# VachaLab/gorder

Measured on AMD Instinct MI355X. Metric: trajectory frames/sec, higher is better.
Workload: dtype f32

## Files before the change

gorder_amd/abi.py:

```python
from __future__ import annotations

import ctypes as C
import os
from dataclasses import dataclass, field
from typing import List, Optional, Sequence

import numpy as np

_HERE = os.path.dirname(os.path.abspath(__file__))
LIB_PATH = os.environ.get("GORDER_HIP_LIB") or os.path.join(_HERE, "libgorder_hip.so")

OK = 0
ERR_UNDEFINED_BOX = 1
ERR_NOT_ORTHOGONAL_BOX = 2
ERR_ZERO_BOX = 3
ERR_UNDEFINED_POSITION = 4
ERR_INVALID_GLOBAL_MEMBRANE_CENTER = 5
ERR_INVALID_LOCAL_MEMBRANE_CENTER = 6
ERR_DYNAMIC_NORMAL = 7
ERR_MANUAL_LEAFLET_FRAME = 8
ERR_MANUAL_NORMAL_FRAME = 9
ERR_INVALID_ARGUMENT = 100
ERR_DEVICE = 101
ERR_NO_DEVICE = 102
# ... 126 lines not shown
    flip: bool = False
    radius: float = 0.0
    membrane: Optional[np.ndarray] = None


@dataclass
class OrderMap:
    enabled: bool = False
    plane: int = 0
    span_x: Sequence[float] = (0.0, 0.0)
    span_y: Sequence[float] = (0.0, 0.0)
    bin: Sequence[float] = (0.1, 0.1)


GEOM_NONE, GEOM_CUBOID, GEOM_CYLINDER, GEOM_SPHERE = range(4)
GEOMREF_POINT, GEOMREF_BOX_CENTER, GEOMREF_GROUP = range(3)
_INF = float("inf")


@dataclass
class Geometry:
    kind: int = GEOM_NONE
    invert: bool = False
    reference: int = GEOMREF_POINT
    point: Sequence[float] = (0.0, 0.0, 0.0)
    group: Optional[np.ndarray] = None
    xdim: Sequence[float] = (-_INF, _INF)
    ydim: Sequence[float] = (-_INF, _INF)
    zdim: Sequence[float] = (-_INF, _INF)
    radius: float = 0.0
    span: Sequence[float] = (-_INF, _INF)
    orientation: int = 2
    structure_box: Sequence[float] = (0.0, 0.0, 0.0)


@dataclass
class DynamicNormal:
    enabled: bool = False
    radius: float = 2.0
    cloud: Optional[np.ndarray] = None


@dataclass
class Tables:
    n_atoms: int
    molecule_types: List[MolType]
    handle_pbc: bool = True
    normal: Sequence[float] = (0.0, 0.0, 1.0)
    leaflets: Leaflets = field(default_factory=Leaflets)
    ordermap: OrderMap = field(default_factory=OrderMap)
    timewise: bool = False
    device: int = 0
    flags: int = 0
    geometry: Geometry = field(default_factory=Geometry)
    dynamic_normal: DynamicNormal = field(default_factory=DynamicNormal)

    @property
    def n_acc(self) -> int:
        return sum(m.n_slots for m in self.molecule_types)

    @property
    def n_molecules_total(self) -> int:
        return sum(m.n_molecules for m in self.molecule_types)

    @property
    def n_samples_per_frame(self) -> int:
        return sum(m.n_slots * m.n_molecules for m in self.molecule_types)

    def as_ctypes(self):
        keep = []
        mts = (CMolType * max(1, len(self.molecule_types)))()
        for k, m in enumerate(self.molecule_types):
            c = mts[k]
            c.n_molecules = m.n_molecules
            b = _u32(m.bonds, (-1, m.n_molecules, 2)) if m.bonds is not None else None
            c.n_bond_types = 0 if b is None else b.shape[0]
            c.bonds = _ptr(b)
            ua = (CUaAtom * max(1, len(m.ua_atoms)))()
            for q, (kind, idx) in enumerate(m.ua_atoms):
                ia = _u32(idx, (m.n_molecules, 4))
                ua[q].kind = int(kind)
                ua[q].indices = _ptr(ia)
                keep.append(ia)
            c.n_ua_atoms = len(m.ua_atoms)
            c.ua_atoms = C.cast(ua, C.POINTER(CUaAtom))
            h = _u32(m.heads, (m.n_molecules,)) if m.heads is not None else None
            c.heads = _ptr(h)
            me = _u32(m.methyls, (m.n_molecules, -1)) if m.methyls is not None else None
            c.n_methyls = 0 if me is None else me.shape[1]
            c.methyls = _ptr(me)
            nh = _u32(m.normal_heads, (m.n_molecules,)) if m.normal_heads is not None else None
            c.normal_heads = _ptr(nh)
            keep += [b, ua, h, me, nh]
        t = CTables()
        t.n_atoms = self.n_atoms
        t.n_molecule_types = len(self.molecule_types)
        t.molecule_types = C.cast(mts, C.POINTER(CMolType))
        t.handle_pbc = 1 if self.handle_pbc else 0
        t.normal[:] = [float(x) for x in self.normal]
        lf = self.leaflets
        mem = _u32(lf.membrane) if lf.membrane is not None else None
        t.leaflets.method = lf.method
        t.leaflets.normal_dim = lf.normal_dim
        t.leaflets.frequency = lf.frequency
        t.leaflets.flip = 1 if lf.flip else 0
        t.leaflets.radius = lf.radius
        t.leaflets.n_membrane = 0 if mem is None else mem.size
        t.leaflets.membrane = _ptr(mem)
        om = self.ordermap
        t.ordermap.enabled = 1 if om.enabled else 0
        t.ordermap.plane = om.plane
        t.ordermap.span_x[:] = [float(x) for x in om.span_x]
        t.ordermap.span_y[:] = [float(x) for x in om.span_y]
        t.ordermap.bin[:] = [float(x) for x in om.bin]
        t.timewise = 1 if self.timewise else 0
        t.device = self.device
        t.flags = self.flags
        ge = self.geometry
        grp = _u32(ge.group) if ge.group is not None else None
        t.geometry.kind = ge.kind
        t.geometry.invert = 1 if ge.invert else 0
        t.geometry.reference = ge.reference
        t.geometry.point[:] = [float(x) for x in ge.point]
        t.geometry.n_group = 0 if grp is None else grp.size
        t.geometry.group = _ptr(grp)
        t.geometry.xdim[:] = [float(x) for x in ge.xdim]
        t.geometry.ydim[:] = [float(x) for x in ge.ydim]
        t.geometry.zdim[:] = [float(x) for x in ge.zdim]
        t.geometry.radius = ge.radius
        t.geometry.span[:] = [float(x) for x in ge.span]
        t.geometry.orientation = ge.orientation
        t.geometry.structure_box[:] = [float(x) for x in ge.structure_box]
        dn = self.dynamic_normal
        cloud = _u32(dn.cloud) if dn.cloud is not None else None
        t.dynamic_normal.enabled = 1 if dn.enabled else 0
        t.dynamic_normal.radius = dn.radius
        t.dynamic_normal.n_cloud = 0 if cloud is None else cloud.size
        t.dynamic_normal.cloud = _ptr(cloud)
        keep += [mts, mem, grp, cloud]
        return t, keep


_EXPORTS = [
    "gorder_hip_create", "gorder_hip_destroy", "gorder_hip_n_accumulators", "gorder_hip_ordermap_dims",
    "gorder_hip_set_stream", "gorder_hip_submit_device", "gorder_hip_submit_host",
    "gorder_hip_prime_leaflets", "gorder_hip_set_manual_leaflets", "gorder_hip_synchronize",
    "gorder_hip_finish", "gorder_hip_timewise", "gorder_hip_leaflets", "gorder_hip_leaflet_distances",
    "gorder_hip_normals", "gorder_hip_export_maps", "gorder_hip_set_normals",
    "gorder_hip_accumulators_device", "gorder_hip_bind_accumulators", "gorder_hip_last_error_index", "gorder_hip_last_error_frame", "gorder_hip_kernel_time_names",
    "gorder_hip_last_error_message", "gorder_hip_strerror", "gorder_hip_kernel_time", "gorder_hip_kernel_time_group", "gorder_hip_plan",
    "gorder_hip_plan_tables", "gorder_hip_selftest_arithmetic", "gorder_hip_selftest_trig", "gorder_hip_selftest_wave_ops", "gorder_hip_run_trajectory",
    "gorder_hip_comm_unique_id", "gorder_hip_comm_create", "gorder_hip_comm_destroy", "gorder_hip_allreduce",
    "gorder_hip_reset", "gorder_hip_xtc_decode", "gorder_hip_release_staging", "gorder_hip_speculation_stats", "gorder_hip_local_decide_stats",
    "gorder_hip_spherical_stats", "gorder_hip_clustering_stats",
    "gorder_hip_set_collect", "gorder_hip_collected_counts", "gorder_hip_collected_leaflets", "gorder_hip_collected_normals",
    "gorder_hip_set_manual_leaflet_table", "gorder_hip_set_manual_normal_table",
    "gorder_hip_timewise_chunk_frames", "gorder_hip_timewise_rows", "gorder_hip_timewise_blocks", "gorder_hip_error_estimate",
    "gorder_hip_convergence", "gorder_hip_ordermaps",
]

_lib = None


class GorderHipError(RuntimeError):
    def __init__(self, status: int, message: str = "", index: int = 0, frame: int = 0):
        self.status = status
        self.index = index
        self.frame = frame
        super().__init__(f"gorder_hip status {status}: {message}")


def load_library() -> C.CDLL:
    global _lib
    if _lib is not None:
        return _lib
    if not os.path.exists(LIB_PATH):
        raise GorderHipError(ERR_NO_DEVICE, f"{LIB_PATH} is missing: run `python -c 'import __graft_entry__ as g; "
                                            "g.build()'` (there is no CPU fallback)")
    try:
        import torch
        _rt = os.path.join(os.path.dirname(torch.__file__), "lib", "libamdhip64.so")
        if os.path.exists(_rt):
            C.CDLL(_rt, mode=C.RTLD_GLOBAL)
    except ImportError:
        pass
    lib = C.CDLL(LIB_PATH)
    vp, u32, u64, i32 = C.c_void_p, C.c_uint32, C.c_uint64, C.c_int
    lib.gorder_hip_create.argtypes = [C.POINTER(CTables), C.POINTER(vp)]
    lib.gorder_hip_destroy.argtypes = [vp]
    lib.gorder_hip_destroy.restype = None
    lib.gorder_hip_n_accumulators.argtypes = [vp]
    lib.gorder_hip_n_accumulators.restype = u32
    lib.gorder_hip_ordermap_dims.argtypes = [vp, C.POINTER(u32), C.POINTER(u32)]
    lib.gorder_hip_ordermap_dims.restype = u32
    lib.gorder_hip_set_stream.argtypes = [vp, vp]
    lib.gorder_hip_submit_device.argtypes = [vp, vp, vp, vp, u32]
    lib.gorder_hip_submit_host.argtypes = [vp, vp, vp, vp, u32]
    lib.gorder_hip_prime_leaflets.argtypes = [vp, vp, vp, u64]
    lib.gorder_hip_set_manual_leaflets.argtypes = [vp, vp, u64]
    lib.gorder_hip_synchronize.argtypes = [vp]
    lib.gorder_hip_finish.argtypes = [vp, vp, vp, vp, vp, C.POINTER(u64)]
    lib.gorder_hip_timewise.argtypes = [vp, vp, vp, u64]
    lib.gorder_hip_leaflets.argtypes = [vp, vp, C.POINTER(u64)]
    lib.gorder_hip_leaflet_distances.argtypes = [vp, vp]
    lib.gorder_hip_normals.argtypes = [vp, vp, vp]
    lib.gorder_hip_export_maps.argtypes = [vp, vp, vp, u64]
    lib.gorder_hip_set_normals.argtypes = [vp, vp, u32]
    lib.gorder_hip_accumulators_device.argtypes = [vp, C.POINTER(vp), C.POINTER(u64)]
    lib.gorder_hip_bind_accumulators.argtypes = [vp, vp, u64]
    lib.gorder_hip_last_error_index.argtypes = [vp]
    lib.gorder_hip_last_error_index.restype = u64
    lib.gorder_hip_kernel_time_names.argtypes = [vp]
    lib.gorder_hip_kernel_time_names.restype = C.c_char_p
    lib.gorder_hip_last_error_frame.argtypes = [vp]
    lib.gorder_hip_last_error_frame.restype = u64
    lib.gorder_hip_last_error_message.argtypes = [vp]
    lib.gorder_hip_last_error_message.restype = C.c_char_p
    lib.gorder_hip_strerror.argtypes = [i32]
    lib.gorder_hip_strerror.restype = C.c_char_p
    lib.gorder_hip_kernel_time.argtypes = [vp, C.POINTER(C.c_double), C.POINTER(u64), i32]
    lib.gorder_hip_kernel_time_group.argtypes = [vp, C.c_uint32, C.POINTER(C.c_char_p), C.POINTER(C.c_double), C.POINTER(u64)]
    lib.gorder_hip_plan.argtypes = [vp, C.POINTER(CPlan)]
    lib.gorder_hip_speculation_stats.argtypes = [vp, C.POINTER(C.c_uint64)]
    lib.gorder_hip_local_decide_stats.argtypes = [vp, C.POINTER(C.c_uint64)]
    lib.gorder_hip_spherical_stats.argtypes = [vp, C.POINTER(C.c_float)]
    lib.gorder_hip_clustering_stats.argtypes = [vp, C.POINTER(C.c_float)]
    lib.gorder_hip_plan_tables.argtypes = [C.POINTER(CTables), C.POINTER(CPlan), C.POINTER(i32)]
    lib.gorder_hip_selftest_arithmetic.argtypes = [i32, C.c_uint64, C.c_uint64, C.POINTER(C.c_uint64)]
    lib.gorder_hip_selftest_trig.argtypes = [i32, i32, C.c_uint32, C.c_uint32, C.c_uint32, C.c_void_p]
    lib.gorder_hip_selftest_wave_ops.argtypes = [i32, u32, vp, vp, vp, i32, vp, vp, vp, vp]
    lib.gorder_hip_run_trajectory.argtypes = [vp, C.POINTER(CTrajectory), C.POINTER(CTrajectoryStats)]
    lib.gorder_hip_comm_unique_id.argtypes = [vp]
    lib.gorder_hip_comm_create.argtypes = [vp, vp, i32, i32, C.POINTER(vp)]
    lib.gorder_hip_comm_destroy.argtypes = [vp]
    lib.gorder_hip_comm_destroy.restype = None
    lib.gorder_hip_allreduce.argtypes = [vp, vp]
    lib.gorder_hip_reset.argtypes = [vp]
    lib.gorder_hip_xtc_decode.argtypes = [vp, vp, u64, vp, u32, u32, vp, u32, vp, u32]
    lib.gorder_hip_release_staging.argtypes = [vp]
    lib.gorder_hip_release_staging.restype = None
    lib.gorder_hip_set_collect.argtypes = [vp, u32]
    lib.gorder_hip_collected_counts.argtypes = [vp, C.POINTER(u64), C.POINTER(u64)]
    lib.gorder_hip_collected_leaflets.argtypes = [vp, vp, vp, u64, C.POINTER(u64)]
    lib.gorder_hip_collected_normals.argtypes = [vp, vp, vp, u64, C.POINTER(u64)]
    lib.gorder_hip_set_manual_leaflet_table.argtypes = [vp, vp, u64, u64]
    lib.gorder_hip_set_manual_normal_table.argtypes = [vp, vp, u32, u64, u64]
    lib.gorder_hip_timewise_chunk_frames.argtypes = []
    lib.gorder_hip_timewise_chunk_frames.restype = u32
    lib.gorder_hip_timewise_rows.argtypes = [vp]
    lib.gorder_hip_timewise_rows.restype = u64
    lib.gorder_hip_timewise_blocks.argtypes = [vp, u32, u64, u64, vp, vp, C.POINTER(u64)]
    lib.gorder_hip_error_estimate.argtypes = [vp, u32, vp, vp, u32, vp, vp, vp]
    lib.gorder_hip_convergence.argtypes = [vp, vp, vp, u32, vp, vp, vp, vp, vp]
    lib.gorder_hip_ordermaps.argtypes = [vp, vp, vp, u32, u32, u32, vp, vp, u64, vp]
    _lib = lib
    return lib


def timewise_chunk_frames() -> int:
    return int(load_library().gorder_hip_timewise_chunk_frames())


def _pack_groups(groups):
    begin = np.zeros(len(groups) + 1, dtype=np.uint32)
    begin[1:] = np.cumsum([len(g) for g in groups])
    flat = [int(k) for g in groups for k in g]
    slots = np.array(flat if flat else [0], dtype=np.uint32)
    return begin, slots


def selftest_trig(fn: str, first_bits: int, stride: int, n: int, device: int = 0) -> np.ndarray:
    lib = load_library()
    out = np.empty(n, dtype=np.float32)
    st = lib.gorder_hip_selftest_trig(device, {"acos": 0, "acos_cores": 1, "cos": 2, "sin": 3}[fn], first_bits, stride, n, out.ctypes.data)
    if st != 0:
        raise GorderHipError(st, "gorder_hip_selftest_trig")
    return out


WAVE_OPS_ROWS = (10, 16, 9, 9)


def selftest_wave_ops(f64, f32, u32, finfo_empty: bool = False, device: int = 0):
    lib = load_library()
    f64 = np.ascontiguousarray(f64, dtype=np.float64)
    f32 = np.ascontiguousarray(f32, dtype=np.float32)
    u32 = np.ascontiguousarray(u32, dtype=np.uint32)
    n = len(f64)
    if len(f32) != n or len(u32) != n:
        raise ValueError("one value of each type per thread")
    o64 = np.empty((WAVE_OPS_ROWS[0], n), dtype=np.float64)
    o32 = np.empty((WAVE_OPS_ROWS[1], n), dtype=np.float32)
    ou = np.empty((WAVE_OPS_ROWS[2], n), dtype=np.uint32)
    fi = np.empty(WAVE_OPS_ROWS[3], dtype=np.uint32)
    st = lib.gorder_hip_selftest_wave_ops(device, n, f64.ctypes.data, f32.ctypes.data, u32.ctypes.data, int(finfo_empty),
                                          o64.ctypes.data, o32.ctypes.data, ou.ctypes.data, fi.ctypes.data)
    if st != 0:
        raise GorderHipError(st, lib.gorder_hip_strerror(st).decode())
    return o64, o32, ou, fi


def selftest_arithmetic(n: int = 1 << 26, seed: int = 1, device: int = 0):
    lib = load_library()
    out = (C.c_uint64 * 2)()
    st = lib.gorder_hip_selftest_arithmetic(device, n, seed, out)
    if st != 0:
        raise GorderHipError(st, lib.gorder_hip_strerror(st).decode())
    return int(out[0]), int(out[1])


def plan_tables(tables: Tables) -> dict:
    lib = load_library()
    ct, keep = tables.as_ctypes()
    plan, check = CPlan(), C.c_int(-1)
    st = lib.gorder_hip_plan_tables(C.byref(ct), C.byref(plan), C.byref(check))
    if st != OK:
        raise GorderHipError(st, lib.gorder_hip_strerror(st).decode())
    d = {name: getattr(plan, name) for name, _ in CPlan._fields_}
    d["selfcheck"] = check.value
    return d


@dataclass
class Results:
    sums: np.ndarray
    counts: np.ndarray
    n_frames: int
    map_sums: Optional[np.ndarray] = None
    map_counts: Optional[np.ndarray] = None

    def order_ticks(self, min_samples: int = 1) -> np.ndarray:
        n = self.counts.astype(np.int64)
        ok = n >= max(1, min_samples)
        q = np.full(self.sums.shape, np.iinfo(np.int64).min, dtype=np.int64)
        q[ok] = (np.abs(self.sums[ok]) // n[ok]) * np.sign(self.sums[ok])
        return q

    def order(self, min_samples: int = 1) -> np.ndarray:
        out = np.full(self.sums.shape, np.nan, dtype=np.float32)
        n = self.counts.astype(np.int64)
        ok = n >= max(1, min_samples)
        q = (np.abs(self.sums[ok]) // n[ok]) * np.sign(self.sums[ok])
        out[ok] = (q.astype(np.float64) / 1e6).astype(np.float32)
        return out


class HipEngine:

    def __init__(self, tables: Tables):
        self.lib = load_library()
        self.tables = tables
        ct, keep = tables.as_ctypes()
        self._h = C.c_void_p()
        st = self.lib.gorder_hip_create(C.byref(ct), C.byref(self._h))
        if st != OK:
            msg = self.lib.gorder_hip_strerror(st).decode()
            if self._h:
                msg += ": " + self.lib.gorder_hip_last_error_message(self._h).decode()
                self.lib.gorder_hip_destroy(self._h)
                self._h = C.c_void_p()
            raise GorderHipError(st, msg)
        self.n_acc = self.lib.gorder_hip_n_accumulators(self._h)
        self._keep = []

    def close(self):
        if getattr(self, "_h", None):
            self.lib.gorder_hip_destroy(self._h)
            self._h = C.c_void_p()

    def __del__(self):
        try:
            self.close()
        except Exception:
            pass

    def _check(self, st: int):
        if st != OK:
# ... 161 lines not shown
        self._check(self.lib.gorder_hip_timewise_blocks(self._h, n_blocks, total_frames, first_position, s.ctypes.data_as(C.c_void_p),
                                                        c.ctypes.data_as(C.c_void_p), C.byref(bs)))
        return s, c, int(bs.value)

    def error_estimate(self, groups, n_blocks: int = 5, blocks=None) -> np.ndarray:
        begin, slots = _pack_groups(groups)
        out = np.zeros((len(groups), 3), dtype=np.float32)
        bs = bc = None
        if blocks is not None:
            bs = np.ascontiguousarray(blocks[0], dtype=np.int64)
            bc = np.ascontiguousarray(blocks[1], dtype=np.uint64)
            assert bs.shape == bc.shape == (n_blocks, 3, self.n_acc)
        self._check(self.lib.gorder_hip_error_estimate(self._h, n_blocks, begin.ctypes.data_as(C.c_void_p), slots.ctypes.data_as(C.c_void_p),
                                                       len(groups), None if bs is None else bs.ctypes.data_as(C.c_void_p),
                                                       None if bc is None else bc.ctypes.data_as(C.c_void_p), out.ctypes.data_as(C.c_void_p)))
        return out

    def convergence(self, groups, carry=None):
        begin, slots = _pack_groups(groups)
        n = len(groups)
        prefix = np.zeros((self.timewise_rows(), 3, n), dtype=np.float32)
        es, ec = np.zeros((3, n), dtype=np.int64), np.zeros((3, n), dtype=np.uint64)
        cs = cc = None
        if carry is not None:
            cs = np.ascontiguousarray(carry[0], dtype=np.int64)
            cc = np.ascontiguousarray(carry[1], dtype=np.uint64)
            assert cs.shape == cc.shape == (3, n)
        self._check(self.lib.gorder_hip_convergence(self._h, begin.ctypes.data_as(C.c_void_p), slots.ctypes.data_as(C.c_void_p), n,
                                                    None if cs is None else cs.ctypes.data_as(C.c_void_p),
                                                    None if cc is None else cc.ctypes.data_as(C.c_void_p),
                                                    prefix.ctypes.data_as(C.c_void_p), es.ctypes.data_as(C.c_void_p),
                                                    ec.ctypes.data_as(C.c_void_p)))
        return prefix, (es, ec)

    def ordermaps(self, groups, min_samples: int = 1, negate: bool = True, device_maps=None) -> np.ndarray:
        begin, slots = _pack_groups(groups)
        nx, ny = self.ordermap_dims()
        out = np.zeros((len(groups), 3, nx, ny), dtype=np.float32)
        buf = out if out.size else np.zeros(1, dtype=np.float32)
        ds = dc = None
        n_u64 = 0
        if device_maps is not None:
            import torch
            ds, dc = device_maps
            for t in (ds, dc):
                assert t.is_cuda and t.is_contiguous() and t.element_size() == 8
            assert ds.numel() == dc.numel()
            n_u64 = ds.numel()
            torch.cuda.synchronize(ds.device)
        self._check(self.lib.gorder_hip_ordermaps(self._h, begin.ctypes.data_as(C.c_void_p), slots.ctypes.data_as(C.c_void_p), len(groups),
                                                  int(min_samples), 1 if negate else 0,
                                                  None if ds is None else C.c_void_p(ds.data_ptr()),
                                                  None if dc is None else C.c_void_p(dc.data_ptr()), n_u64,
                                                  buf.ctypes.data_as(C.c_void_p)))
        return out

    def leaflets(self):
        flags = np.zeros(self.tables.n_molecules_total, dtype=np.uint8)
        fr = C.c_uint64()
        self._check(self.lib.gorder_hip_leaflets(self._h, flags.ctypes.data_as(C.c_void_p), C.byref(fr)))
        return flags, int(fr.value)

    def set_collect(self, what: int):
        self._check(self.lib.gorder_hip_set_collect(self._h, what))

    def collected_counts(self):
        a, b = C.c_uint64(), C.c_uint64()
        self._check(self.lib.gorder_hip_collected_counts(self._h, C.byref(a), C.byref(b)))
        return int(a.value), int(b.value)

    def collected_leaflets(self):
        rows = self.collected_counts()[0]
        flags = np.zeros((rows, self.tables.n_molecules_total), dtype=np.uint8)
        frames = np.zeros(rows, dtype=np.uint64)
        n = C.c_uint64()
        self._check(self.lib.gorder_hip_collected_leaflets(self._h, flags.ctypes.data_as(C.c_void_p),
                                                           frames.ctypes.data_as(C.c_void_p), rows, C.byref(n)))
        assert n.value == rows
        return flags, frames

    def collected_normals(self):
        rows = self.collected_counts()[1]
        normals = np.zeros((rows, self.tables.n_molecules_total, 3), dtype=np.float32)
        frames = np.zeros(rows, dtype=np.uint64)
        n = C.c_uint64()
        self._check(self.lib.gorder_hip_collected_normals(self._h, normals.ctypes.data_as(C.c_void_p),
                                                          frames.ctypes.data_as(C.c_void_p), rows, C.byref(n)))
        assert n.value == rows
        return normals, frames

    def leaflet_distances(self) -> np.ndarray:
        d = np.zeros(self.tables.n_molecules_total, dtype=np.float32)
        self._check(self.lib.gorder_hip_leaflet_distances(self._h, d.ctypes.data_as(C.c_void_p)))
        return d

    def set_normals(self, normals: np.ndarray):
        n = np.ascontiguousarray(normals, dtype=np.float32)
        assert n.ndim == 3 and n.shape[1:] == (self.tables.n_molecules_total, 3)
        self._check(self.lib.gorder_hip_set_normals(self._h, n.ctypes.data_as(C.c_void_p), n.shape[0]))

    def normals(self):
        n = np.zeros((self.tables.n_molecules_total, 3), dtype=np.float32)
        k = np.zeros(self.tables.n_molecules_total, dtype=np.uint32)
        self._check(self.lib.gorder_hip_normals(self._h, n.ctypes.data_as(C.c_void_p), k.ctypes.data_as(C.c_void_p)))
        return n, k

    def accumulator_words(self) -> int:
        p, n = C.c_void_p(), C.c_uint64()
        self._check(self.lib.gorder_hip_accumulators_device(self._h, C.byref(p), C.byref(n)))
        return int(n.value)

    def flush(self):
        self.accumulator_words()

    def bind_accumulators(self, tensor):
        assert tensor.is_cuda and tensor.is_contiguous() and tensor.element_size() == 8
        self._keep.append(tensor)
        self._check(self.lib.gorder_hip_bind_accumulators(self._h, C.c_void_p(tensor.data_ptr()), tensor.numel()))

    def export_maps(self, sums, counts):
        for t in (sums, counts):
            assert t.is_cuda and t.is_contiguous() and t.element_size() == 8
        assert sums.numel() == counts.numel()
        self._check(self.lib.gorder_hip_export_maps(self._h, C.c_void_p(sums.data_ptr()), C.c_void_p(counts.data_ptr()),
                                                     sums.numel()))

    def kernel_time(self, reset: bool = False):
        ms, n = C.c_double(), C.c_uint64()
        self._check(self.lib.gorder_hip_kernel_time(self._h, C.byref(ms), C.byref(n), 1 if reset else 0))
        return ms.value, int(n.value)

    def kernel_names(self) -> str:
        return self.lib.gorder_hip_kernel_time_names(self._h).decode()

    def kernel_groups(self):
        out, k = [], 0
        while True:
            name, ms, n = C.c_char_p(), C.c_double(), C.c_uint64()
            if self.lib.gorder_hip_kernel_time_group(self._h, k, C.byref(name), C.byref(ms), C.byref(n)) != 0:
                return out
            out.append((name.value.decode(), ms.value, int(n.value)))
            k += 1

    def speculation_stats(self) -> dict:
        out = (C.c_uint64 * 4)()
        self._check(self.lib.gorder_hip_speculation_stats(self._h, out))
        return {"batches": int(out[0]), "moved": int(out[1]), "exact_frames": int(out[2]), "enabled": bool(out[3])}

    def local_decide_stats(self) -> dict:
        out = (C.c_uint64 * 4)()
        self._check(self.lib.gorder_hip_local_decide_stats(self._h, out))
        return {"submits": int(out[0]), "paused": int(out[1]), "open_frames": int(out[2]), "frames": int(out[3])}

    def spherical_stats(self) -> dict:
        out = (C.c_float * 12)()
        self._check(self.lib.gorder_hip_spherical_stats(self._h, out))
        v = np.array(out[:], dtype=np.float32)
        return {"centre": v[0:3].copy(), "weight_a": v[3], "mean_a": v[4], "var_a": v[5], "mean_b": v[6], "var_b": v[7],
                "avg_log_likelihood": v[8], "iterations": int(v[9]), "n_outer": int(v[10])}

    def clustering_stats(self) -> dict:
        out = (C.c_float * 12)()
        self._check(self.lib.gorder_hip_clustering_stats(self._h, out))
        v = np.array(out[:], dtype=np.float32)
        return {"eigenvalues": v[0:3].copy(), "steps": int(v[3]), "rounds": int(v[4]), "n_cluster": (int(v[5]), int(v[6])),
                "n_upper": int(v[7]), "n_lower": int(v[8]), "o_up": v[9], "o_lo": v[10]}

    def plan(self) -> dict:
        p = CPlan()
        self._check(self.lib.gorder_hip_plan(self._h, C.byref(p)))
        return {name: getattr(p, name) for name, _ in CPlan._fields_}
```

gorder_amd/csrc/gorder_hip.hip:

```cpp
#include <hip/hip_runtime.h>

#include <dlfcn.h>

#include <cmath>
#include <cstdio>
#include <cstdlib>
#include <cstring>
#include <mutex>
#include <new>
#include <string>
#include <deque>
#include <vector>

#include "../../include/gorder_hip.h"
#include "gm_math.h"
#include "plan.h"
#include "collect_store.h"
#include "replay_rows.h"
#include "timewise_blocks.h"
#include "ordermap_final.h"

#pragma clang fp contract(off)

using gorder::DirectItem;
using gorder::Item;
using gorder::kBlock;
using gorder::Plan;
using gorder::Tile;

#include "kernels_common.h"
#include "kernels_bonds.h"
#include "kernels_extras.h"
#include "kernels_leaflets.h"
#include "kernels_cluster.h"
#include "kernels_cluster_cutoff.h"
#include "kernels_normals.h"
#include "kernels_xtc.h"
#include "kernels_trr.h"
#include "kernels_collect.h"
#include "kernels_replay.h"
#include "kernels_timewise.h"
#include "kernels_ordermap.h"


struct gorder_hip_handle {
    void *traj_cache = nullptr;
    void (*traj_cache_free)(gorder_hip_handle *) = nullptr;
    Plan plan;
    gorder_tables_t tables{};
    int device = 0;
    hipStream_t own_stream = nullptr;
    hipStream_t stream = nullptr;
    Tile *d_tiles = nullptr;
    Item *d_items = nullptr;
    uint32_t *d_tile_slots = nullptr;
    DirectItem *d_direct = nullptr;
    Tile *d_ua_tiles = nullptr;
    gorder::UaItem *d_ua_items = nullptr;
    uint32_t *d_ua_tile_slots = nullptr;
    uint32_t map_nx = 0, map_ny = 0;
    unsigned long long *d_map_sums = nullptr, *d_map_cnts = nullptr;
    unsigned long long *d_map_packed = nullptr;
    unsigned long long *d_map_rec = nullptr;
    size_t map_rec_cap = 0;
    gorder::MapRun *d_ua_runs = nullptr, *d_runs = nullptr;
    uint32_t *d_ua_run_begin = nullptr, *d_run_begin = nullptr;
    Item *d_items_by_slot = nullptr;
    uint32_t *d_ua_item_run = nullptr, *d_item_run = nullptr;
    uint4 *d_lgrid = nullptr;
    LocalRowPre *d_lrowpre = nullptr;
    LocalEdge *d_ledge = nullptr;
    float4 *d_lfinfo = nullptr;
    static constexpr uint32_t kDecidePause = 16;
    uint32_t *d_lsummary = nullptr, *h_lsummary = nullptr;
    hipEvent_t lsummary_written = nullptr;
    bool lsummary_pending = false;
    uint32_t decide_pause = 0;
    uint64_t decide_submits = 0, decide_paused_submits = 0;
    uint32_t *d_lneed = nullptr;
    uint2 *d_ltodo = nullptr;
    size_t map_lds_bytes = 0;
    bool map_staged = false;
    uint64_t map_pending = 0;
    uint64_t map_fold_limit = kMapFoldLimit;
    uint32_t map_max_mol = 1;
    unsigned long long *d_tw_sums = nullptr, *d_tw_cnts = nullptr;
    uint64_t tw_cap = 0;
    unsigned long long *d_twx_blocks = nullptr, *d_twx_rows = nullptr, *d_twx_totals = nullptr, *d_twx_edge = nullptr;
    uint32_t *d_twx_groups = nullptr;
    float *d_twx_out = nullptr;
    size_t twx_blocks_cap = 0, twx_rows_cap = 0, twx_totals_cap = 0, twx_edge_cap = 0, twx_groups_cap = 0, twx_out_cap = 0;
    uint32_t *d_omx_groups = nullptr;
    float *d_omx_out = nullptr;
    size_t omx_groups_cap = 0, omx_out_cap = 0;
    ExtraArgs extra{};
    uint32_t *d_geom_group = nullptr;
    float *d_shapes = nullptr;
    float *d_inv_box = nullptr;
    size_t inv_box_cap = 0;
    uint32_t dyn_slab = 4, local_slab = 4;
    bool local_halo = false;
    size_t local_rec_stride = 0;
    XtcCheckpoint *d_xtc_cp = nullptr;
    size_t xtc_cp_cap = 0;
    bool dyn = false;
    uint32_t *d_dyn_cloud = nullptr, *d_dyn_heads = nullptr;
    uint32_t *d_dyn_cell_of = nullptr, *d_dyn_count = nullptr;
    float *d_dyn_rec = nullptr;
    float4 *d_dyn_normals = nullptr;
    DynCov *d_dyn_cov = nullptr;
    size_t dyn_normals_cap = 0;
    std::vector<float> last_normals;
    std::vector<float> manual_normals;
    uint32_t manual_frames = 0;
    bool manual_active = false;
    size_t shapes_cap = 0;
    uint32_t *d_err = nullptr;
    unsigned long long *d_acc = nullptr;
    unsigned long long *d_rep = nullptr;
    uint32_t n_rep = 32;
    bool rep_dirty = false;
    bool acc_external = false;
    size_t acc_words = 0;
    uint32_t *d_heads = nullptr, *d_membrane = nullptr, *d_methyl_begin = nullptr, *d_methyl_atoms = nullptr;
    uint8_t *d_aflags = nullptr;
    size_t aflags_rows = 0;
    float *d_adist = nullptr;
    float *d_sph_spill = nullptr, *d_sph_stats = nullptr;
    uint32_t sph_spill = 0, sph_slab = 1u << 20, sph_threads = 1024;
    void *d_cl_scratch = nullptr;
    uint32_t *d_cl_head_slot = nullptr;
    uint8_t *d_cl_carry = nullptr, *d_cl_is0 = nullptr;
    float *d_cl_stats = nullptr;
    uint32_t cl_slab = 1, cl_m_max = 0;
    bool cl_stored_w = false;
    bool cl_have_carry = false;
    bool cl_cut = false;
    uint32_t cl_tiles = 0, cl_sort = 0;
    std::vector<uint8_t> cl_is0;
    uint32_t *d_lcell_of = nullptr, *d_lcell_count = nullptr, *d_lcell_fill = nullptr;
    float *d_ltrig = nullptr;
    uint32_t *d_arow = nullptr, *d_aframes = nullptr;
    std::vector<uint32_t> up_arow, up_aframes;
    const uint32_t *up_arow_at = nullptr, *up_aframes_at = nullptr;
    size_t arow_cap = 0, aframes_cap = 0;
    bool have_assignment = false;
    uint64_t assignment_frame = 0;
    bool spec_enabled = false;
    bool spec_now = false;
    uint2 *d_own = nullptr;
    float4 *d_mom = nullptr;
    size_t mom_cap = 0;
    float *d_head_z = nullptr;
    size_t head_z_cap = 0;
    uint32_t *d_own_head_begin = nullptr;
    uint2 *d_own_heads = nullptr;
    float *d_spec_center = nullptr;
    uint8_t *d_spec_ok = nullptr;
    size_t spec_frames_cap = 0;
    uint32_t *d_spec_counters = nullptr;
    static constexpr uint32_t kSpecRing = 8;
    uint32_t *h_spec_counters = nullptr;
    hipEvent_t spec_counters_copied[kSpecRing] = {};
    uint64_t spec_ring_frames[kSpecRing] = {};
    uint32_t *d_spec_mol_begin = nullptr;
    SpecSample *d_spec_samples = nullptr;
    uint64_t spec_batches = 0, spec_fixed = 0, spec_exact_frames = 0;
    float *d_stage_xyz[2] = {nullptr, nullptr}, *d_stage_box[2] = {nullptr, nullptr};
    size_t stage_xyz_cap[2] = {0, 0}, stage_box_cap[2] = {0, 0};
    hipEvent_t stage_copied[2] = {nullptr, nullptr}, stage_computed[2] = {nullptr, nullptr};
    bool stage_used[2] = {false, false};
    int stage_next = 0;
    hipStream_t copy_stream = nullptr;
    float n2 = 1.0f, n2sq = 1.0f;
    int axis = -1;
    int frames_per_stage = kFramesPerStage;
    bool membrane_is_frame = false;
    bool use_gather = false;
    uint32_t wg_capacity = 256u * 6u;
    uint32_t wg_target = 0;
    uint32_t lw = 0;
    size_t lds_bytes = 0;
    uint64_t n_frames = 0;
    uint64_t err_index = 0;
    std::string err_msg;
    static constexpr uint32_t kTimingEvents = 1024;
    struct TimingSeg { uint32_t label, ev_a, ev_b; };
    bool timing_on = false;
    hipEvent_t timing_ev[kTimingEvents] = {};
    uint32_t timing_next_ev = 0;
    int timing_open_label = -1;
    uint32_t timing_open_ev = 0;
    std::deque<TimingSeg> timing_pending;
    std::vector<std::string> timing_labels;
    std::vector<double> timing_label_ms;
    std::vector<uint64_t> timing_label_n;
    uint64_t timing_launches = 0;
    std::string timed_kernels;
    std::vector<uint32_t> host_heads, host_dyn_heads;
    uint32_t *d_mol_slot0 = nullptr;
    uint64_t err_frame = 0;
    struct BatchLog { uint64_t ordinal, first, stride; std::vector<uint64_t> list; };
    static constexpr size_t kBatchLog = 4096;
    std::deque<BatchLog> batch_log;
    uint64_t n_submits = 0;
    const unsigned long long *decoder_key = nullptr;
    uint32_t collect = 0;
    bool collect_locked = false;
    gorder::CollectStore collect_flags;
    gorder::CollectStore collect_normals;
    unsigned long long *d_collect_words = nullptr;
    CollectVec3 *d_collect_vec = nullptr;
    uint8_t *d_touched = nullptr;
    size_t collect_words_cap = 0, collect_vec_cap = 0, touched_cap = 0;
    unsigned long long *d_ltable = nullptr;
    gorder::ReplayWindow ltable_win;
    bool replay_have_carry = false;
    uint64_t replay_carry_index = 0;
    ReplayVec3 *d_ntable = nullptr;
    gorder::ReplayWindow ntable_win;
    uint32_t ntable_step = 1;
    uint32_t *d_nrow = nullptr;
    size_t nrow_cap = 0;
};

namespace {

int fail(gorder_hip_handle *h, int status, const std::string &msg) {
    if (h) h->err_msg = msg;
    return status;
}

#define HIP_TRY(h, expr)                                                                    \
    do {                                                                                    \
        hipError_t e_ = (expr);                                                             \
        if (e_ != hipSuccess)                                                               \
            return fail(h, GORDER_ERR_DEVICE, std::string(#expr) + ": " + hipGetErrorString(e_)); \
    } while (0)

template <typename T>
int upload(gorder_hip_handle *h, T **dst, const std::vector<T> &src) {
    *dst = nullptr;
    if (src.empty()) return GORDER_OK;
    HIP_TRY(h, hipMalloc((void **)dst, src.size() * sizeof(T)));
    HIP_TRY(h, hipMemcpy(*dst, src.data(), src.size() * sizeof(T), hipMemcpyHostToDevice));
    return GORDER_OK;
}

template <typename T>
int ensure(gorder_hip_handle *h, T **buf, size_t *cap, size_t need) {
    if (need <= *cap) return GORDER_OK;
    if (*buf) HIP_TRY(h, hipFree(*buf));
    *buf = nullptr;
    *cap = 0;
// ... 10 lines not shown
uint32_t sample_atom(const Plan &p, uint32_t slot, uint32_t mol, uint32_t which) {
    for (const Tile &t : p.tiles)
        for (uint32_t q = 0; q < t.n_items; q++) {
            const Item &it = p.items[t.item0 + q];
            if (it.mol == mol && p.tile_slots[t.slot0 + it.lslot] == slot) return t.atom0 + (which ? it.lj : it.li);
        }
    for (const DirectItem &d : p.direct)
        if (d.mol == mol && d.slot == slot) return which ? d.j : d.i;
    for (const Tile &t : p.ua_tiles)
        for (uint32_t q = 0; q < t.n_items; q++) {
            const gorder::UaItem &it = p.ua_items[t.item0 + q];
            if (it.mol == mol && p.ua_tile_slots[t.slot0 + it.lslot0] == slot) return t.atom0 + it.l[which & 3u];
        }
    return 0;
}

int check_device_error(gorder_hip_handle *h) {
    unsigned long long rec[3] = {kErrNone, kErrNone, 0};
    HIP_TRY(h, hipMemcpy(rec, h->d_err, sizeof(rec), hipMemcpyDeviceToHost));
    const bool latched = rec[1] != kErrNone;
    const unsigned long long key = latched ? rec[1] : rec[0];
    if (key == kErrNone) { h->batch_log.clear(); return GORDER_OK; }
    const uint32_t code = (uint32_t)(key & 15u), detail = (uint32_t)(key >> 4) & 3u, mol = (uint32_t)(key >> 6) & 0x1ffffu;
    const uint32_t sample = (uint32_t)(key >> 23) & 1u, slot = (uint32_t)(key >> 24) & 0x3fffu;
    const uint32_t stage = (uint32_t)(key >> 38) & 3u, frame = (uint32_t)(key >> 40) & 0x7fffffu;
    const int status = code == 8u ? (int)GORDER_ERR_BOX_RANGE : (code == 9u ? (int)GORDER_ERR_TRAJECTORY_FORMAT :
                       (code == 10u ? (int)GORDER_ERR_CLUSTERING : (code == 11u ? (int)GORDER_ERR_CLUSTER_MATCH : (int)code)));
    h->err_frame = frame;
    char where[96];
    snprintf(where, sizeof(where), "frame %u of a batch", frame);
    if (latched)
        for (const auto &b : h->batch_log)
            if (b.ordinal == rec[2]) {
                if (b.list.empty()) h->err_frame = b.first + (uint64_t)frame * b.stride;
                else if (frame < b.list.size()) h->err_frame = b.list[frame];
                snprintf(where, sizeof(where), "frame %llu of the trajectory (frame %u of batch %llu)",
                         (unsigned long long)h->err_frame, frame, (unsigned long long)rec[2]);
                break;
            }
    h->err_index = 0;
    if (status == GORDER_ERR_UNDEFINED_POSITION) {
        if (stage == kStageTypes && sample) h->err_index = sample_atom(h->plan, slot, mol, detail);
        else if (mol < h->host_dyn_heads.size()) h->err_index = h->host_dyn_heads[mol];
    } else if (status == GORDER_ERR_INVALID_LOCAL_MEMBRANE_CENTER) {
        if (mol < h->host_heads.size()) h->err_index = h->host_heads[mol];
    } else if (status == GORDER_ERR_DYNAMIC_NORMAL) {
        h->err_index = detail;
    } else if (status == GORDER_ERR_CLUSTERING || status == GORDER_ERR_CLUSTER_MATCH) {
        h->err_index = h->err_frame;
    }
    char buf[200];
    snprintf(buf, sizeof(buf), "device raised %s (payload %llu) in %s", gorder_hip_strerror(status),
             (unsigned long long)h->err_index, where);
    h->err_msg = buf;
    return status;
}

int timing_drain_oldest(gorder_hip_handle *h) {
    const gorder_hip_handle::TimingSeg sg = h->timing_pending.front();
    float t = 0.0f;
    HIP_TRY(h, hipEventSynchronize(h->timing_ev[sg.ev_b]));
    HIP_TRY(h, hipEventElapsedTime(&t, h->timing_ev[sg.ev_a], h->timing_ev[sg.ev_b]));
    h->timing_label_ms[sg.label] += t;
    h->timing_label_n[sg.label] += 1;
    h->timing_pending.pop_front();
    return GORDER_OK;
}
int timing_mark(gorder_hip_handle *h, const char *label) {
    if (!h->timing_on) return GORDER_OK;
    if (!label && h->timing_open_label < 0) return GORDER_OK;
    while (h->timing_pending.size() >= gorder_hip_handle::kTimingEvents / 2u - 2u) {
        const int st = timing_drain_oldest(h);
        if (st != GORDER_OK) return st;
    }
    const uint32_t ev = h->timing_next_ev;
    h->timing_next_ev = (ev + 1u) % gorder_hip_handle::kTimingEvents;
    if (!h->timing_ev[ev]) HIP_TRY(h, hipEventCreate(&h->timing_ev[ev]));
    HIP_TRY(h, hipEventRecord(h->timing_ev[ev], h->stream));
    if (h->timing_open_label >= 0) h->timing_pending.push_back({(uint32_t)h->timing_open_label, h->timing_open_ev, ev});
    h->timing_open_label = -1;
    if (label) {
        size_t k = 0;
        while (k < h->timing_labels.size() && h->timing_labels[k] != label) k++;
        if (k == h->timing_labels.size()) {
            h->timing_labels.push_back(label);
            h->timing_label_ms.push_back(0.0);
            h->timing_label_n.push_back(0);
            if (!h->timed_kernels.empty()) h->timed_kernels += " + ";
            h->timed_kernels += label;
        }
        h->timing_open_label = (int)k;
        h->timing_open_ev = ev;
    }
    return GORDER_OK;
}
#define TIMING_MARK(h, label)                                   \
    do {                                                        \
        const int tm_ = timing_mark(h, label);                  \
        if (tm_ != GORDER_OK) return tm_;                       \
    } while (0)

bool env_flag(const char *name) {
    const char *v = getenv(name);
    return v && *v && strcmp(v, "0") != 0;
}

int fold_replicas(gorder_hip_handle *h) {
    if (!h->rep_dirty || !h->d_rep) return GORDER_OK;
    const uint32_t n = 4u * h->plan.n_acc;
    hipLaunchKernelGGL(k_fold_replicas, dim3((n + 255) / 256), dim3(256), 0, h->stream, h->d_acc, h->d_rep, h->n_rep, n);
    HIP_TRY(h, hipGetLastError());
    h->rep_dirty = false;
    return GORDER_OK;
}

int fold_maps(gorder_hip_handle *h) {
    if (!h->extra.maps || !h->map_pending) return GORDER_OK;
    const size_t n = (size_t)h->plan.n_acc * h->map_nx * h->map_ny;
    const uint32_t blocks = (uint32_t)std::min<size_t>((n + 255) / 256, 256 * 16);
    hipLaunchKernelGGL(k_fold_maps, dim3(blocks), dim3(256), 0, h->stream, h->d_map_packed, h->d_map_sums, h->d_map_cnts,
                       n, h->tables.leaflets.method != GORDER_LEAFLETS_NONE ? 1 : 0);
    HIP_TRY(h, hipGetLastError());
    h->map_pending = 0;
    return GORDER_OK;
}

int launch_cell_list(gorder_hip_handle *h, const LocalArgs &lo, uint32_t ns, uint32_t n_list, void *counts, size_t count_bytes) {
    const bool three = env_flag("GORDER_HIP_LOCAL_THREE_KERNELS");
    TIMING_MARK(h, n_list <= kLocalBuildMax && !three ? "k_local_build" : "k_local_bin + k_local_scan + k_local_scatter");
    if (n_list <= kLocalBuildMax && !three) {
        if (n_list <= 2u * 8192u) hipLaunchKernelGGL(k_local_build<2>, dim3(ns), dim3(1024), kLocalBuildLds, h->stream, lo);
        else if (n_list <= 5u * 8192u) hipLaunchKernelGGL(k_local_build<5>, dim3(ns), dim3(1024), kLocalBuildLds, h->stream, lo);
        else hipLaunchKernelGGL(k_local_build<kLocalBuildTrips>, dim3(ns), dim3(1024), kLocalBuildLds, h->stream, lo);
        return GORDER_OK;
    }
    HIP_TRY(h, hipMemsetAsync(counts, 0, count_bytes, h->stream));
    const dim3 ga((n_list + 255) / 256, ns);
    hipLaunchKernelGGL(k_local_bin, ga, dim3(256), 0, h->stream, lo);
    hipLaunchKernelGGL(k_local_scan, dim3(ns), dim3(1024), 0, h->stream, lo);
    hipLaunchKernelGGL(k_local_scatter, ga, dim3(256), 0, h->stream, lo);
    return GORDER_OK;
}

int run_dynamic_normals(gorder_hip_handle *h, const FrameArgs &a) {
    int st;
    const uint32_t n_mol = h->plan.n_mol_total;
    if ((st = ensure(h, &h->d_dyn_normals, &h->dyn_normals_cap, (size_t)a.n_frames * n_mol)) != GORDER_OK) return st;
    const gorder_dynamic_normal_t &dn = h->tables.dynamic_normal;
    const size_t ncell = (size_t)kLocalMaxCells1D * kLocalMaxCells1D;
    LocalArgs lo{};
    lo.xyz = a.xyz; lo.box9 = a.box9; lo.n_atoms = a.n_atoms;
    lo.n_mol_total = n_mol; lo.heads = h->d_dyn_heads; lo.membrane = h->d_dyn_cloud; lo.n_membrane = dn.n_cloud;
    lo.dim = 2; lo.pbc = a.pbc; lo.radius = dn.radius; lo.radius_thr = local_radius_threshold(dn.radius);
    lo.halo = 0; lo.rec_stride = dn.n_cloud;
    lo.cell_of = h->d_dyn_cell_of; lo.trig = h->d_dyn_rec;
    lo.cell_count = h->d_dyn_count; lo.cell_fill = h->d_dyn_count + h->dyn_slab * (ncell + 1);
    lo.err = h->d_err; lo.aframes = nullptr; lo.write_dist_frame = -1;
    for (uint32_t done = 0; done < a.n_frames; done += h->dyn_slab) {
        const uint32_t ns = std::min(a.n_frames - done, h->dyn_slab);
        lo.frame0 = done;
        lo.n_slab = ns;
        if ((st = launch_cell_list(h, lo, ns, dn.n_cloud, h->d_dyn_count,
                                   (size_t)h->dyn_slab * (2 * ncell + 1) * sizeof(uint32_t))) != GORDER_OK) return st;
        TIMING_MARK(h, "k_dyn_cov + k_dyn_eigen");
        hipLaunchKernelGGL(k_dyn_cov, dim3((n_mol + 15) / 16, ns), dim3(256), 0, h->stream, lo, h->d_dyn_cov);
        hipLaunchKernelGGL(k_dyn_eigen, dim3((uint32_t)(((size_t)ns * n_mol + 255) / 256)), dim3(256), 0, h->stream, lo, h->d_dyn_cov,
                           h->d_dyn_normals);
    }
    HIP_TRY(h, hipGetLastError());
    h->last_normals.resize(4 * (size_t)n_mol);
    HIP_TRY(h, hipMemcpyAsync(h->last_normals.data(), h->d_dyn_normals + (size_t)(a.n_frames - 1) * n_mol,
                              4 * sizeof(float) * (size_t)n_mol, hipMemcpyDeviceToHost, h->stream));
    return GORDER_OK;
}

int launch_orders(gorder_hip_handle *h, FrameArgs &a) {
    const Plan &p = h->plan;
    const uint32_t n_tiles = (uint32_t)p.tiles.size();
    const bool extras = h->extra.maps || h->extra.tw || h->extra.geom_kind || h->dyn || h->manual_active;
#define name(k) TIMING_MARK(h, k)
    if (h->dyn && !h->manual_active) {
        const int st2 = run_dynamic_normals(h, a);
        if (st2 != GORDER_OK) return st2;
    }
    if (h->extra.geom_kind) {
        int st2;
        if ((st2 = ensure(h, &h->d_shapes, &h->shapes_cap, (size_t)a.n_frames * 8)) != GORDER_OK) return st2;
        const gorder_geometry_t &ge = h->tables.geometry;
        GeomArgs ga{};
        ga.xyz = a.xyz; ga.box9 = a.box9; ga.n_atoms = a.n_atoms; ga.pbc = a.pbc;
        ga.kind = ge.kind; ga.reference = ge.reference; ga.orientation = ge.orientation;
        for (int d = 0; d < 3; d++) { ga.point[d] = ge.point[d]; ga.structure_box[d] = ge.structure_box[d]; }
        for (int d = 0; d < 2; d++) { ga.xdim[d] = ge.xdim[d]; ga.ydim[d] = ge.ydim[d]; ga.zdim[d] = ge.zdim[d]; ga.span[d] = ge.span[d]; }
        ga.radius = ge.radius; ga.group = h->d_geom_group; ga.n_group = ge.n_group;
        ga.shapes = h->d_shapes; ga.err = h->d_err;
        name("k_geom_shapes");
        hipLaunchKernelGGL(k_geom_shapes, dim3(a.n_frames), dim3(256), 0, h->stream, ga);
        HIP_TRY(h, hipGetLastError());
    }
    if (n_tiles && !extras) {
        const uint32_t G = (uint32_t)h->frames_per_stage;
        const uint32_t n_stages = (a.n_frames + G - 1) / G;
        uint32_t target = h->wg_target ? h->wg_target : h->wg_capacity;
        if (!h->wg_target) target = 12u * h->wg_capacity;
        uint32_t n_chunks = std::max(1u, target / n_tiles);
        n_chunks = std::min(n_chunks, std::max(1u, n_stages / 4u));
        uint32_t fpc = ((n_stages + n_chunks - 1) / n_chunks) * G;
        n_chunks = (a.n_frames + fpc - 1) / fpc;
        a.frames_per_chunk = fpc;
        const uint64_t grid = (uint64_t)n_tiles * n_chunks;
        if (grid > 0x7fffffffull) return fail(h, GORDER_ERR_INVALID_ARGUMENT, "batch too large");
        const bool ac = (h->tables.flags & GORDER_FLAG_TRIG_ACOS_COS) != 0;
        const dim3 g((uint32_t)grid), b(kBlock);
#define GORDER_LAUNCH_TILED_A(G_, NPF_, AC_, PBC_, LF_, AX_)                                               \
        do {                                                                                                \
            if (LF_ && h->spec_now)                                                                         \
                hipLaunchKernelGGL((k_bonds_tiled<G_, NPF_, AC_, PBC_, LF_, AX_, LF_>), g, b, h->lds_bytes, h->stream, a, \
                                   a.xyz, a.box9, a.aflags, a.arow, h->d_tiles, h->d_items, h->d_tile_slots, n_tiles, h->lw); \
            else                                                                                            \
                hipLaunchKernelGGL((k_bonds_tiled<G_, NPF_, AC_, PBC_, LF_, AX_>), g, b, h->lds_bytes, h->stream, a,     \
                                   a.xyz, a.box9, a.aflags, a.arow, h->d_tiles, h->d_items, h->d_tile_slots, n_tiles,   \
                                   h->lw);                                                                  \
        } while (0)
#define GORDER_LAUNCH_TILED_V(G_, NPF_, AC_, PBC_, LF_)                                                    \
        do {                                                                                                \
            if (h->axis == 2) GORDER_LAUNCH_TILED_A(G_, NPF_, AC_, PBC_, LF_, 2);                           \
            else if (h->axis == 1) GORDER_LAUNCH_TILED_A(G_, NPF_, AC_, PBC_, LF_, 1);                      \
            else if (h->axis == 0) GORDER_LAUNCH_TILED_A(G_, NPF_, AC_, PBC_, LF_, 0);                      \
            else GORDER_LAUNCH_TILED_A(G_, NPF_, AC_, PBC_, LF_, -1);                                       \
        } while (0)
#define GORDER_LAUNCH_TILED(G_, NPF_)                                                                       \
        do {                                                                                                \
            const int v_ = (ac ? 4 : 0) | (a.pbc ? 2 : 0) | (a.leaflets ? 1 : 0);                           \
            switch (v_) {                                                                                   \
                case 0: GORDER_LAUNCH_TILED_V(G_, NPF_, false, false, false); break;                        \
                case 1: GORDER_LAUNCH_TILED_V(G_, NPF_, false, false, true); break;                         \
                case 2: GORDER_LAUNCH_TILED_V(G_, NPF_, false, true, false); break;                         \
                case 3: GORDER_LAUNCH_TILED_V(G_, NPF_, false, true, true); break;                          \
                case 4: GORDER_LAUNCH_TILED_V(G_, NPF_, true, false, false); break;                         \
                case 5: GORDER_LAUNCH_TILED_V(G_, NPF_, true, false, true); break;                          \
                case 6: GORDER_LAUNCH_TILED_V(G_, NPF_, true, true, false); break;                          \
                default: GORDER_LAUNCH_TILED_V(G_, NPF_, true, true, true); break;                          \
            }                                                                                               \
        } while (0)
#define GORDER_LAUNCH_GATHER_V(G_, AC_, PBC_, LF_)                                                         \
        hipLaunchKernelGGL((k_bonds_gather<G_, AC_, PBC_, LF_>), g, b, 0, h->stream, a, a.xyz, a.box9, a.aflags, \
                           a.arow, h->d_tiles, h->d_items, h->d_tile_slots, n_tiles)
#define GORDER_LAUNCH_GATHER(G_)                                                                            \
        do {                                                                                                \
            const int v_ = (ac ? 4 : 0) | (a.pbc ? 2 : 0) | (a.leaflets ? 1 : 0);                           \
            switch (v_) {                                                                                   \
                case 0: GORDER_LAUNCH_GATHER_V(G_, false, false, false); break;                             \
                case 1: GORDER_LAUNCH_GATHER_V(G_, false, false, true); break;                              \
                case 2: GORDER_LAUNCH_GATHER_V(G_, false, true, false); break;                              \
                case 3: GORDER_LAUNCH_GATHER_V(G_, false, true, true); break;                               \
                case 4: GORDER_LAUNCH_GATHER_V(G_, true, false, false); break;                              \
                case 5: GORDER_LAUNCH_GATHER_V(G_, true, false, true); break;                               \
                case 6: GORDER_LAUNCH_GATHER_V(G_, true, true, false); break;                               \
                default: GORDER_LAUNCH_GATHER_V(G_, true, true, true); break;                               \
            }                                                                                               \
        } while (0)
        name(h->use_gather ? "k_bonds_gather" : "k_bonds_tiled");
        if (h->use_gather) {
            GORDER_LAUNCH_GATHER(4);
        } else {
            if ((3u * p.max_window + 6u) / 4u <= 4u * 64u && !env_flag("GORDER_HIP_NPF5")) GORDER_LAUNCH_TILED(4, 4);
            else GORDER_LAUNCH_TILED(4, 5);
        }
#undef GORDER_LAUNCH_GATHER
#undef GORDER_LAUNCH_GATHER_V
#undef GORDER_LAUNCH_TILED_A
#undef GORDER_LAUNCH_TILED_V
#undef GORDER_LAUNCH_TILED
        HIP_TRY(h, hipGetLastError());
    }
    if (extras || !p.ua_tiles.empty()) {
        ExtraArgs e = h->extra;
        e.tw_sums = h->d_tw_sums; e.tw_cnts = h->d_tw_cnts; e.tw_row0 = h->n_frames;
        e.shapes = h->d_shapes;
        const bool ua_fast = (h->tables.flags & GORDER_FLAG_UA_FAST_NORMALISE) != 0 && !p.ua_tiles.empty();
        e.inv_box = nullptr;
        if (ua_fast && a.pbc) {
            int st3;
            if ((st3 = ensure(h, &h->d_inv_box, &h->inv_box_cap, (size_t)a.n_frames * 8)) != GORDER_OK) return st3;
            hipLaunchKernelGGL(k_inv_box, dim3((4u * a.n_frames + 255u) / 256u), dim3(256), 0, h->stream, a.box9, a.n_frames, h->d_inv_box);
            e.inv_box = h->d_inv_box;
        }
        e.dyn = (h->dyn || h->manual_active) ? h->d_dyn_normals : nullptr;
        const bool ac = (h->tables.flags & GORDER_FLAG_TRIG_ACOS_COS) != 0;
        uint32_t sub = e.maps ? (uint32_t)std::max<uint64_t>(1, (h->map_fold_limit - 1) / h->map_max_mol) : a.n_frames;
        const bool staged = e.maps && h->map_staged;
        const size_t rec_per_frame = std::max(p.ua_tiles.size() * 3u, extras ? p.tiles.size() : (size_t)0) * kBlock;
        if (staged) {
            sub = std::min<uint32_t>(sub, (uint32_t)std::max<size_t>(1, ((size_t)1 << 27) / rec_per_frame));
            sub = std::min(sub, a.n_frames);
            const int st2 = ensure(h, &h->d_map_rec, &h->map_rec_cap, rec_per_frame * (((size_t)sub + 15) / 16 * 16));
            if (st2 != GORDER_OK) return st2;
        }
        for (uint32_t lo = 0; lo < a.n_frames; lo += sub) {
            const uint32_t hi = std::min(a.n_frames, lo + sub), nf = hi - lo;
            if (e.maps) {
                const uint64_t cost = (uint64_t)nf * h->map_max_mol;
                if (h->map_pending + cost >= h->map_fold_limit) {
                    const int st = fold_maps(h);
                    if (st != GORDER_OK) return st;
                }
                h->map_pending += cost;
// ... 646 lines not shown
            if (!mt.normal_heads) return fail(h, GORDER_ERR_INVALID_ARGUMENT, "dynamic normals need normal_heads[] per molecule type");
            for (uint32_t k = 0; k < mt.n_molecules; k++) {
                if (mt.normal_heads[k] >= t->n_atoms) return fail(h, GORDER_ERR_INVALID_ARGUMENT, "normal head index out of range");
                nheads.push_back(mt.normal_heads[k]);
            }
        }
        if ((st = upload(h, &h->d_dyn_cloud, cloud)) != GORDER_OK) return st;
        if ((st = upload(h, &h->d_dyn_heads, nheads)) != GORDER_OK) return st;
        h->host_dyn_heads = nheads;
        const size_t nm = dn.n_cloud, ncell = (size_t)kLocalMaxCells1D * kLocalMaxCells1D;
        const size_t sl = h->dyn_slab = local_slab_frames(nm);
        for (const void *fn : {reinterpret_cast<const void *>(k_local_build<2>), reinterpret_cast<const void *>(k_local_build<5>),
                               reinterpret_cast<const void *>(k_local_build<kLocalBuildTrips>)})
            HIP_TRY(h, hipFuncSetAttribute(fn, hipFuncAttributeMaxDynamicSharedMemorySize, (int)kLocalBuildLds));
        HIP_TRY(h, hipMalloc((void **)&h->d_dyn_cell_of, sl * nm * sizeof(uint32_t)));
        HIP_TRY(h, hipMalloc((void **)&h->d_dyn_rec, sl * nm * 4 * sizeof(float)));
        HIP_TRY(h, hipMalloc((void **)&h->d_dyn_count, sl * (2 * ncell + 1) * sizeof(uint32_t)));
        HIP_TRY(h, hipMalloc((void **)&h->d_dyn_cov, sl * (size_t)(p.n_mol_total ? p.n_mol_total : 1) * sizeof(DynCov)));
        h->dyn = true;
    }

    const gorder_leaflets_t &lf = t->leaflets;
    if (lf.method != GORDER_LEAFLETS_NONE) {
        if (lf.method > GORDER_LEAFLETS_CLUSTERING) return fail(h, GORDER_ERR_INVALID_ARGUMENT, "leaflets.method");
        if (lf.method != GORDER_LEAFLETS_SPHERICAL && lf.method != GORDER_LEAFLETS_CLUSTERING && lf.normal_dim > 2) return fail(h, GORDER_ERR_INVALID_ARGUMENT, "leaflets.normal_dim");
        std::vector<uint32_t> heads, mb(1, 0), ma;
        for (uint32_t m = 0; m < t->n_molecule_types; m++) {
            const gorder_moltype_t &mt = t->molecule_types[m];
            if (lf.method != GORDER_LEAFLETS_MANUAL && !mt.heads)
                return fail(h, GORDER_ERR_INVALID_ARGUMENT, "leaflets need heads[] per molecule type");
            if (lf.method == GORDER_LEAFLETS_INDIVIDUAL && (!mt.methyls || mt.n_methyls == 0))
                return fail(h, GORDER_ERR_INVALID_ARGUMENT, "individual leaflets need methyls[]");
            for (uint32_t k = 0; k < mt.n_molecules; k++) {
                const uint32_t hd = mt.heads ? mt.heads[k] : 0;
                if (hd >= t->n_atoms) return fail(h, GORDER_ERR_INVALID_ARGUMENT, "head index out of range");
                heads.push_back(hd);
                if (lf.method == GORDER_LEAFLETS_INDIVIDUAL)
                    for (uint32_t q = 0; q < mt.n_methyls; q++) {
                        const uint32_t a = mt.methyls[(size_t)k * mt.n_methyls + q];
                        if (a >= t->n_atoms) return fail(h, GORDER_ERR_INVALID_ARGUMENT, "methyl index out of range");
                        ma.push_back(a);
                    }
                mb.push_back((uint32_t)ma.size());
            }
        }
        if ((st = upload(h, &h->d_heads, heads)) != GORDER_OK) return st;
        h->host_heads = heads;
        if (lf.method == GORDER_LEAFLETS_LOCAL) {
            std::vector<uint32_t> ms;
            for (uint32_t m = 0; m < t->n_molecule_types; m++) ms.insert(ms.end(), t->molecule_types[m].n_molecules, p.slot0[m]);
            if ((st = upload(h, &h->d_mol_slot0, ms)) != GORDER_OK) return st;
        }
        if ((st = upload(h, &h->d_methyl_begin, mb)) != GORDER_OK) return st;
        if ((st = upload(h, &h->d_methyl_atoms, ma)) != GORDER_OK) return st;
        if (lf.method == GORDER_LEAFLETS_LOCAL && !(lf.radius > 0.0f))
            return fail(h, GORDER_ERR_INVALID_ARGUMENT, "local leaflets need a positive radius");
        if (lf.method == GORDER_LEAFLETS_GLOBAL || lf.method == GORDER_LEAFLETS_LOCAL) {
            if (!lf.membrane || lf.n_membrane == 0)
                return fail(h, GORDER_ERR_INVALID_ARGUMENT, "global/local leaflets need the membrane group");
            std::vector<uint32_t> mem(lf.membrane, lf.membrane + lf.n_membrane);
            for (uint32_t a : mem)
                if (a >= t->n_atoms) return fail(h, GORDER_ERR_INVALID_ARGUMENT, "membrane index out of range");
            if ((st = upload(h, &h->d_membrane, mem)) != GORDER_OK) return st;
            h->membrane_is_frame = lf.n_membrane == t->n_atoms && !env_flag("GORDER_HIP_LEAFLETS_GENERIC");
            for (uint32_t i = 0; i < lf.n_membrane && h->membrane_is_frame; i++) h->membrane_is_frame = mem[i] == i;
        }
        if (lf.method == GORDER_LEAFLETS_SPHERICAL) {
            if (!lf.membrane || lf.n_membrane < 2)
                return fail(h, GORDER_ERR_INVALID_ARGUMENT, "leaflets.n_membrane: spherical clustering needs at least two group atoms");
            std::vector<uint32_t> grp(lf.membrane, lf.membrane + lf.n_membrane);
            std::vector<int32_t> slot_of(t->n_atoms, -1);
            for (uint32_t i = 0; i < lf.n_membrane; i++) {
                if (grp[i] >= t->n_atoms) return fail(h, GORDER_ERR_INVALID_ARGUMENT, "leaflets.membrane: index out of range");
                if (slot_of[grp[i]] < 0) slot_of[grp[i]] = (int32_t)i;
            }
            for (uint32_t hd : heads)
                if (slot_of[hd] < 0)
                    return fail(h, GORDER_ERR_INVALID_ARGUMENT, "molecule_types[].heads: a head is not a member of leaflets.membrane");
            if ((st = upload(h, &h->d_membrane, grp)) != GORDER_OK) return st;
            h->sph_threads = lf.n_membrane <= 256u * (uint32_t)kSphKeep ? 256u : 1024u;
            const uint32_t resident = h->sph_threads * (uint32_t)kSphKeep;
            h->sph_spill = lf.n_membrane > resident ? lf.n_membrane - resident : 0u;
            if (h->sph_spill) {
                h->sph_slab = (uint32_t)std::min<size_t>(std::max<size_t>(((size_t)64 << 20) / (h->sph_spill * sizeof(float)), 1), 4096);
                HIP_TRY(h, hipMalloc((void **)&h->d_sph_spill, (size_t)h->sph_slab * h->sph_spill * sizeof(float)));
            }
            HIP_TRY(h, hipMalloc((void **)&h->d_sph_stats, 12 * sizeof(float)));
            HIP_TRY(h, hipMemset(h->d_sph_stats, 0, 12 * sizeof(float)));
        }
        if (lf.method == GORDER_LEAFLETS_CLUSTERING) {
            if (!lf.membrane || lf.n_membrane < kClMinGroup)
                return fail(h, GORDER_ERR_INVALID_ARGUMENT, "leaflets.n_membrane: clustering needs at least two group atoms");
            h->cl_cut = (t->flags & GORDER_FLAG_CLUSTER_CUTOFF) != 0;
            if (!h->cl_cut && lf.n_membrane > kClMaxGroup)
                return fail(h, GORDER_ERR_INVALID_ARGUMENT, "leaflets.n_membrane: clustering takes at most 8192 group atoms");
            if (h->cl_cut && lf.n_membrane > kClCutMaxGroup)
                return fail(h, GORDER_ERR_INVALID_ARGUMENT, "leaflets.n_membrane: clustering with GORDER_FLAG_CLUSTER_CUTOFF takes at most 131072 group atoms");
            std::vector<uint32_t> grp(lf.membrane, lf.membrane + lf.n_membrane);
            std::vector<int32_t> slot_of(t->n_atoms, -1);
            for (uint32_t i = 0; i < lf.n_membrane; i++) {
                if (grp[i] >= t->n_atoms) return fail(h, GORDER_ERR_INVALID_ARGUMENT, "leaflets.membrane: index out of range");
                if (i && grp[i] <= grp[i - 1]) return fail(h, GORDER_ERR_INVALID_ARGUMENT, "leaflets.membrane: clustering needs ascending, distinct atoms");
                slot_of[grp[i]] = (int32_t)i;
            }
            std::vector<uint32_t> head_slot;
            for (uint32_t hd : heads) {
                if (slot_of[hd] < 0)
                    return fail(h, GORDER_ERR_INVALID_ARGUMENT, "molecule_types[].heads: a head is not a member of leaflets.membrane");
                head_slot.push_back((uint32_t)slot_of[hd]);
            }
            if ((st = upload(h, &h->d_membrane, grp)) != GORDER_OK) return st;
            if ((st = upload(h, &h->d_cl_head_slot, head_slot)) != GORDER_OK) return st;
            const uint32_t n = lf.n_membrane;
            h->cl_m_max = std::min<uint32_t>(n - 1u, (uint32_t)kClMaxSteps);
            h->cl_stored_w = env_flag("GORDER_HIP_CLUSTER_STORED_W");
            h->cl_tiles = (n + kClCutTile - 1u) / kClCutTile;
            h->cl_sort = (n + kClCutSort - 1u) / kClCutSort;
            const size_t per_frame = h->cl_cut ? clcut_frame_bytes(n, h->cl_m_max)
                                               : cl_frame_bytes(n, h->cl_m_max) + (h->cl_stored_w ? (size_t)n * n * 4 : 0);
            h->cl_slab = (uint32_t)std::min<size_t>(std::max<size_t>(((size_t)512 << 20) / per_frame, 1), 1024);
            HIP_TRY(h, hipMalloc(&h->d_cl_scratch, (size_t)h->cl_slab * per_frame));
            HIP_TRY(h, hipMalloc((void **)&h->d_cl_carry, n));
            HIP_TRY(h, hipMalloc((void **)&h->d_cl_is0, h->cl_slab));
            HIP_TRY(h, hipMalloc((void **)&h->d_cl_stats, 12 * sizeof(float)));
            HIP_TRY(h, hipMemset(h->d_cl_stats, 0, 12 * sizeof(float)));
        }
        if (lf.method == GORDER_LEAFLETS_GLOBAL && p.spec_ok && !env_flag("GORDER_HIP_NO_SPECULATE")) {
            std::vector<uint2> own(p.tiles.size());
            for (size_t i = 0; i < own.size(); i++) own[i] = make_uint2(p.own[2 * i], p.own[2 * i + 1]);
            if ((st = upload(h, &h->d_own, own)) != GORDER_OK) return st;
            std::vector<std::vector<SpecSample>> per_mol(p.n_mol_total);
            for (const Tile &tile : p.tiles)
                for (uint32_t q = 0; q < tile.n_items; q++) {
                    const Item &it = p.items[tile.item0 + q];
                    per_mol[it.mol].push_back({tile.atom0 + it.li, tile.atom0 + it.lj, p.tile_slots[tile.slot0 + it.lslot]});
                }
            std::vector<uint32_t> mbeg(1, 0);
            std::vector<SpecSample> all;
            for (const auto &v : per_mol) { all.insert(all.end(), v.begin(), v.end()); mbeg.push_back((uint32_t)all.size()); }
            if ((st = upload(h, &h->d_spec_mol_begin, mbeg)) != GORDER_OK) return st;
            if ((st = upload(h, &h->d_spec_samples, all)) != GORDER_OK) return st;
            std::vector<uint2> oh(p.own_heads.size() / 2);
            for (size_t i = 0; i < oh.size(); i++) oh[i] = make_uint2(p.own_heads[2 * i], p.own_heads[2 * i + 1]);
            if ((st = upload(h, &h->d_own_head_begin, p.own_head_begin)) != GORDER_OK) return st;
            if ((st = upload(h, &h->d_own_heads, oh)) != GORDER_OK) return st;
            HIP_TRY(h, hipMalloc((void **)&h->d_spec_counters, 4 * sizeof(uint32_t)));
            HIP_TRY(h, hipMemset(h->d_spec_counters, 0, 4 * sizeof(uint32_t)));
            HIP_TRY(h, hipHostMalloc((void **)&h->h_spec_counters, 2 * gorder_hip_handle::kSpecRing * sizeof(uint32_t)));
            for (hipEvent_t &ev : h->spec_counters_copied) HIP_TRY(h, hipEventCreateWithFlags(&ev, hipEventDisableTiming));
            h->spec_enabled = true;
        }
        if (lf.method == GORDER_LEAFLETS_LOCAL) {
            const size_t nm = lf.n_membrane, ncell = (size_t)kLocalMaxCells1D * kLocalMaxCells1D;
            const size_t sl = h->local_slab = local_slab_frames(nm);
            for (const void *fn : {reinterpret_cast<const void *>(k_local_build<2>), reinterpret_cast<const void *>(k_local_build<5>),
                                   reinterpret_cast<const void *>(k_local_build<kLocalBuildTrips>)})
                HIP_TRY(h, hipFuncSetAttribute(fn, hipFuncAttributeMaxDynamicSharedMemorySize, (int)kLocalBuildLds));
            h->local_halo = t->handle_pbc && !env_flag("GORDER_HIP_LOCAL_ATOMS_ONLY");
            h->local_rec_stride = (h->local_halo ? 2u : 1u) * nm;
            HIP_TRY(h, hipMalloc((void **)&h->d_lcell_of, sl * nm * sizeof(uint32_t)));
            HIP_TRY(h, hipMalloc((void **)&h->d_ltrig, sl * h->local_rec_stride * sizeof(LocalRec)));
            HIP_TRY(h, hipMalloc((void **)&h->d_lcell_count, sl * (ncell + 1) * sizeof(uint32_t)));
            HIP_TRY(h, hipMalloc((void **)&h->d_lcell_fill, sl * ncell * sizeof(uint32_t)));
            HIP_TRY(h, hipMalloc((void **)&h->d_lgrid, sl * sizeof(uint4)));
            if (h->local_halo) {
                HIP_TRY(h, hipMalloc((void **)&h->d_lrowpre, sl * (size_t)kLocalMaxCells1D * (kLocalMaxCells1D + 1u) * sizeof(LocalRowPre)));
                HIP_TRY(h, hipMalloc((void **)&h->d_ledge, sl * (size_t)kLocalMaxCells1D * (kLocalMaxCells1D + 1u) * sizeof(LocalEdge)));
                HIP_TRY(h, hipMalloc((void **)&h->d_lfinfo, sl * sizeof(float4)));
                HIP_TRY(h, hipMalloc((void **)&h->d_lneed, (sl + 1) * sizeof(uint32_t)));
                HIP_TRY(h, hipMalloc((void **)&h->d_lsummary, 2 * sizeof(uint32_t)));
                HIP_TRY(h, hipMemset(h->d_lsummary, 0, 2 * sizeof(uint32_t)));
                HIP_TRY(h, hipHostMalloc((void **)&h->h_lsummary, 2 * sizeof(uint32_t)));
                h->h_lsummary[0] = h->h_lsummary[1] = 0u;
                HIP_TRY(h, hipEventCreateWithFlags(&h->lsummary_written, hipEventDisableTiming));
                HIP_TRY(h, hipFuncSetAttribute(reinterpret_cast<const void *>(k_local_decide), hipFuncAttributeMaxDynamicSharedMemorySize,
                                               (int)kDecideLds));
                HIP_TRY(h, hipFuncSetAttribute(reinterpret_cast<const void *>(k_local_sums), hipFuncAttributeMaxDynamicSharedMemorySize,
                                               (int)kSumsLds));
                HIP_TRY(h, hipMalloc((void **)&h->d_ltodo, (1 + sl * (size_t)(p.n_mol_total ? p.n_mol_total : 1)) * sizeof(uint2)));
            }
        }
        HIP_TRY(h, hipMalloc((void **)&h->d_adist, sizeof(float) * (p.n_mol_total ? p.n_mol_total : 1)));
    }
    HIP_TRY(h, hipDeviceSynchronize());
    return GORDER_OK;
}

void gorder_hip_destroy(gorder_hip_handle *h) {
    if (!h) return;
    (void)hipSetDevice(h->device);
    if (h->stream) (void)hipStreamSynchronize(h->stream);
    if (h->traj_cache_free) h->traj_cache_free(h);
    for (hipEvent_t ev : h->timing_ev)
        if (ev) (void)hipEventDestroy(ev);
    (void)hipFree(h->d_mol_slot0);
    (void)hipFree(h->d_tiles); (void)hipFree(h->d_items); (void)hipFree(h->d_tile_slots);
    (void)hipFree(h->d_direct); (void)hipFree(h->d_err); (void)hipFree(h->d_xtc_cp);
    (void)hipFree(h->d_ua_tiles); (void)hipFree(h->d_ua_items); (void)hipFree(h->d_ua_tile_slots);
    (void)hipFree(h->d_map_sums); (void)hipFree(h->d_map_cnts); (void)hipFree(h->d_map_packed); (void)hipFree(h->d_tw_sums); (void)hipFree(h->d_tw_cnts);
    (void)hipFree(h->d_twx_blocks); (void)hipFree(h->d_twx_rows); (void)hipFree(h->d_twx_totals); (void)hipFree(h->d_twx_edge); (void)hipFree(h->d_twx_groups); (void)hipFree(h->d_twx_out);
    (void)hipFree(h->d_omx_groups); (void)hipFree(h->d_omx_out);
    (void)hipFree(h->d_geom_group); (void)hipFree(h->d_shapes); (void)hipFree(h->d_inv_box);
    (void)hipFree(h->d_map_rec); (void)hipFree(h->d_ua_runs); (void)hipFree(h->d_ua_run_begin);
    (void)hipFree(h->d_runs); (void)hipFree(h->d_run_begin); (void)hipFree(h->d_items_by_slot);
    (void)hipFree(h->d_ua_item_run); (void)hipFree(h->d_item_run); (void)hipFree(h->d_lgrid); (void)hipFree(h->d_lrowpre); (void)hipFree(h->d_ledge);
    (void)hipFree(h->d_own); (void)hipFree(h->d_mom); (void)hipFree(h->d_head_z); (void)hipFree(h->d_own_head_begin); (void)hipFree(h->d_own_heads); (void)hipFree(h->d_spec_center); (void)hipFree(h->d_spec_ok);
    (void)hipFree(h->d_spec_counters); (void)hipFree(h->d_spec_mol_begin); (void)hipFree(h->d_spec_samples);
    if (h->h_spec_counters) (void)hipHostFree(h->h_spec_counters);
    for (hipEvent_t ev : h->spec_counters_copied) if (ev) (void)hipEventDestroy(ev); (void)hipFree(h->d_lfinfo); (void)hipFree(h->d_ltodo); (void)hipFree(h->d_lneed);
    (void)hipFree(h->d_lsummary); if (h->h_lsummary) (void)hipHostFree(h->h_lsummary); if (h->lsummary_written) (void)hipEventDestroy(h->lsummary_written);
    (void)hipFree(h->d_dyn_cloud); (void)hipFree(h->d_dyn_heads); (void)hipFree(h->d_dyn_cell_of); (void)hipFree(h->d_dyn_count);
    (void)hipFree(h->d_dyn_rec); (void)hipFree(h->d_dyn_normals); (void)hipFree(h->d_dyn_cov);
    if (!h->acc_external) (void)hipFree(h->d_acc);
    (void)hipFree(h->d_rep);
    (void)hipFree(h->d_heads); (void)hipFree(h->d_membrane); (void)hipFree(h->d_methyl_begin);
    (void)hipFree(h->d_methyl_atoms); (void)hipFree(h->d_aflags); (void)hipFree(h->d_adist);
    (void)hipFree(h->d_sph_spill); (void)hipFree(h->d_sph_stats);
    (void)hipFree(h->d_cl_scratch); (void)hipFree(h->d_cl_head_slot); (void)hipFree(h->d_cl_carry); (void)hipFree(h->d_cl_is0);
    (void)hipFree(h->d_cl_stats);
    (void)hipFree(h->d_arow); (void)hipFree(h->d_aframes);
    (void)hipFree(h->d_collect_words); (void)hipFree(h->d_collect_vec); (void)hipFree(h->d_touched);
    (void)hipFree(h->d_ltable); (void)hipFree(h->d_ntable); (void)hipFree(h->d_nrow);
    h->collect_flags.release(); h->collect_normals.release();
    (void)hipFree(h->d_lcell_of); (void)hipFree(h->d_lcell_count); (void)hipFree(h->d_lcell_fill);
    (void)hipFree(h->d_ltrig);
    for (int k = 0; k < 2; k++) {
        (void)hipFree(h->d_stage_xyz[k]); (void)hipFree(h->d_stage_box[k]);
        if (h->stage_copied[k]) (void)hipEventDestroy(h->stage_copied[k]);
        if (h->stage_computed[k]) (void)hipEventDestroy(h->stage_computed[k]);
    }
    if (h->copy_stream) (void)hipStreamDestroy(h->copy_stream);
    if (h->own_stream) (void)hipStreamDestroy(h->own_stream);
    delete h;
}

uint32_t gorder_hip_n_accumulators(const gorder_hip_handle *h) { return h ? h->plan.n_acc : 0; }
uint32_t gorder_hip_ordermap_dims(const gorder_hip_handle *h, uint32_t *nx, uint32_t *ny) {
    if (nx) *nx = h ? h->map_nx : 0;
    if (ny) *ny = h ? h->map_ny : 0;
    return h ? h->map_nx * h->map_ny : 0;
}

int gorder_hip_set_stream(gorder_hip_handle *h, void *hip_stream) {
    if (!h) return GORDER_ERR_INVALID_ARGUMENT;
    HIP_TRY(h, hipSetDevice(h->device));
    HIP_TRY(h, hipStreamSynchronize(h->stream));
    h->stream = hip_stream ? (hipStream_t)hip_stream : h->own_stream;
    return GORDER_OK;
}

static void spec_poll(gorder_hip_handle *h, bool wait);
int gorder_hip_speculation_stats(gorder_hip_handle *h, uint64_t out[4]) {
    if (!h || !out) return GORDER_ERR_INVALID_ARGUMENT;
    HIP_TRY(h, hipSetDevice(h->device));
    HIP_TRY(h, hipStreamSynchronize(h->stream));
    spec_poll(h, true);
    out[0] = h->spec_batches; out[1] = h->spec_fixed; out[2] = h->spec_exact_frames; out[3] = h->spec_enabled ? 1 : 0;
    return GORDER_OK;
}

int gorder_hip_local_decide_stats(gorder_hip_handle *h, uint64_t out[4]) {
    if (!h || !out) return GORDER_ERR_INVALID_ARGUMENT;
    HIP_TRY(h, hipSetDevice(h->device));
    HIP_TRY(h, hipStreamSynchronize(h->stream));
    out[0] = h->decide_submits; out[1] = h->decide_paused_submits;
    out[2] = h->h_lsummary ? h->h_lsummary[0] : 0; out[3] = h->h_lsummary ? h->h_lsummary[1] : 0;
    return GORDER_OK;
}

int gorder_hip_plan(const gorder_hip_handle *h, gorder_hip_plan_t *plan) {
    if (!h || !plan) return GORDER_ERR_INVALID_ARGUMENT;
    plan->n_tiles = (uint32_t)h->plan.tiles.size();
    plan->block_threads = kBlock;
    plan->max_window_atoms = h->plan.max_window;
    plan->n_direct_items = (uint32_t)h->plan.direct.size();
    plan->frames_per_stage = (uint32_t)h->frames_per_stage;
    plan->lds_bytes = (uint32_t)h->lds_bytes;
    plan->map_staged = h->map_staged ? 1u : 0u;
    plan->map_lds_bytes = (uint32_t)h->map_lds_bytes;
    plan->leaflets_one_read = h->plan.spec_ok ? 1u : 0u;
    return GORDER_OK;
}

static void spec_poll(gorder_hip_handle *h, bool wait) {
    for (uint32_t i = 0; i < gorder_hip_handle::kSpecRing; i++) {
        if (!h->spec_ring_frames[i]) continue;
        if (wait) (void)hipEventSynchronize(h->spec_counters_copied[i]);
        else if (hipEventQuery(h->spec_counters_copied[i]) != hipSuccess) continue;
        const uint32_t moved = h->h_spec_counters[2 * i], exact = h->h_spec_counters[2 * i + 1];
        h->spec_fixed += moved;
        h->spec_exact_frames += exact;
        if ((uint64_t)exact * 8u > h->spec_ring_frames[i] ||
            (uint64_t)moved * 16u > h->spec_ring_frames[i] * h->plan.n_mol_total)
            h->spec_enabled = false;
        h->spec_ring_frames[i] = 0;
    }
}

static size_t cl_round(size_t b) { return (b + 15u) & ~(size_t)15u; }
static size_t cl_frame_bytes(uint32_t n, uint32_t m_max) {
    return cl_round(3 * (size_t)n * 4) + 3 * cl_round((size_t)n * 4) + cl_round((size_t)(m_max + 1u) * n * 4) +
           cl_round(kClSol * 8) + cl_round(n) + cl_round(kClMeta * 4) + 16;
}
static void clcut_sizes(uint32_t n, uint32_t m_max, size_t (&b)[22]) {
    const size_t tiles = (n + kClCutTile - 1u) / kClCutTile, sort = (n + kClCutSort - 1u) / kClCutSort, nf = cl_round((size_t)n * 4);
    const size_t v[22] = {cl_round(kClSol * 8), cl_round((size_t)tiles * kClLd * 8), cl_round(kClLd * 8), cl_round(2 * kClLd * 8),
                          cl_round(kClCutScal * 8), cl_round(sizeof(ClCutGrid)), cl_round(sort * kClCutMaxCells * 4),
                          cl_round((kClCutMaxCells + 1u) * 4), nf , nf , cl_round(3 * (size_t)n * 4), nf ,
                          nf , nf , nf , nf , cl_round((size_t)(m_max + 1u) * n * 4),
                          cl_round(kClMeta * 4), 16 , 16 , cl_round(n) , 0};
    for (int k = 0; k < 22; k++) b[k] = v[k];
}
static size_t clcut_frame_bytes(uint32_t n, uint32_t m_max) {
    size_t b[22], sum = 0;
    clcut_sizes(n, m_max, b);
    for (size_t v : b) sum += v;
    return sum;
}
static int run_clustering_cutoff(gorder_hip_handle *h, const float *d_xyz, const float *d_box, size_t n_assign, uint32_t row0) {
    const gorder_leaflets_t &lf = h->tables.leaflets;
    const uint32_t n = lf.n_membrane, slab = h->cl_slab, tiles = h->cl_tiles, sort = h->cl_sort;
    size_t bytes[22];
    clcut_sizes(n, h->cl_m_max, bytes);
    ClCutArgs ca{};
    ca.c.xyz = d_xyz; ca.c.box9 = d_box; ca.c.n_atoms = h->plan.n_atoms; ca.c.group = h->d_membrane; ca.c.n = n;
    ca.c.pbc = h->tables.handle_pbc ? 1 : 0; ca.c.m_max = h->cl_m_max; ca.c.err = h->d_err; ca.c.W = nullptr;
    ca.n_tiles = tiles; ca.n_sort = sort;
    char *base = (char *)h->d_cl_scratch;
    int at = 0;
    auto carve = [&]() { char *p = base; base += bytes[at++] * slab; return p; };
    ca.c.sol = (double *)carve(); ca.part = (double *)carve(); ca.coef = (double *)carve(); ca.albe = (double *)carve();
    ca.scal = (double *)carve(); ca.grid = (ClCutGrid *)carve(); ca.cnt = (uint32_t *)carve(); ca.cell_start = (uint32_t *)carve();
    ca.cell_of = (uint32_t *)carve(); ca.perm = (uint32_t *)carve(); ca.c.pos = (float *)carve(); ca.c.s = (float *)carve();
    ca.c.q = (float *)carve(); ca.c.emb = (float *)carve(); ca.e0 = (float *)carve(); ca.e1 = (float *)carve();
    ca.c.V = (float *)carve(); ca.c.meta = (float *)carve(); ca.c.fail = (uint32_t *)carve(); ca.done = (uint32_t *)carve();
    ca.c.lab = (uint8_t *)carve();
    ClOrientArgs oa{};
    oa.n = n; oa.lab = ca.c.lab; oa.emb = ca.c.emb; oa.meta = ca.c.meta; oa.fail = ca.c.fail; oa.carry = h->d_cl_carry;
    oa.aflags = h->d_aflags; oa.n_mol_total = h->plan.n_mol_total; oa.head_slot = h->d_cl_head_slot;
    oa.flip = lf.flip ? 1 : 0; oa.err = h->d_err; oa.is_frame0 = h->d_cl_is0;
    for (size_t done = 0; done < n_assign; done += slab) {
        const uint32_t ns = (uint32_t)std::min<size_t>(n_assign - done, slab);
        const bool last = done + ns == n_assign;
        ca.c.aframes = h->d_aframes + done; ca.c.n_assign = ns;
        oa.aframes = ca.c.aframes; oa.n_assign = ns; oa.row0 = row0 + (uint32_t)done;
        oa.adist = last ? h->d_adist : nullptr;
        oa.stats = last ? h->d_cl_stats : nullptr;
        const dim3 rows(tiles, ns), blocks(sort, ns);
        HIP_TRY(h, hipMemsetAsync(ca.c.fail, 0, (size_t)ns * sizeof(uint32_t), h->stream));
        HIP_TRY(h, hipMemsetAsync(ca.done, 0, (size_t)ns * sizeof(uint32_t), h->stream));
        HIP_TRY(h, hipMemcpyAsync(h->d_cl_is0, h->cl_is0.data() + done, ns, hipMemcpyHostToDevice, h->stream));
        TIMING_MARK(h, "k_clcut_cells");
        hipLaunchKernelGGL(k_clcut_grid, dim3(ns), dim3(256), 0, h->stream, ca);
        hipLaunchKernelGGL(k_clcut_count, blocks, dim3(1024), 0, h->stream, ca);
        hipLaunchKernelGGL(k_clcut_scan, dim3(ns), dim3(1024), 0, h->stream, ca);
        hipLaunchKernelGGL(k_clcut_scatter, blocks, dim3(1024), 0, h->stream, ca);
        TIMING_MARK(h, "k_clcut_lanczos");
        hipLaunchKernelGGL(k_clcut_degrees, rows, dim3(kClCutTile), 0, h->stream, ca);
        hipLaunchKernelGGL(k_clcut_start, dim3(ns), dim3(1024), 0, h->stream, ca);
        for (int j = 0; j < (int)h->cl_m_max; j++) {
            hipLaunchKernelGGL(k_clcut_spmv, rows, dim3(kClCutTile), 0, h->stream, ca, j);
            hipLaunchKernelGGL(k_clcut_coef, dim3(ns), dim3(512), 0, h->stream, ca, j, 0);
            hipLaunchKernelGGL(k_clcut_update, rows, dim3(kClCutTile), 0, h->stream, ca, j, 0);
            hipLaunchKernelGGL(k_clcut_dots, rows, dim3(kClCutTile), 0, h->stream, ca, j);
            hipLaunchKernelGGL(k_clcut_coef, dim3(ns), dim3(512), 0, h->stream, ca, j, 1);
            hipLaunchKernelGGL(k_clcut_update, rows, dim3(kClCutTile), 0, h->stream, ca, j, 1);
            hipLaunchKernelGGL(k_clcut_small, dim3(ns), dim3(1024), 0, h->stream, ca, j);
            hipLaunchKernelGGL(k_clcut_scale, rows, dim3(kClCutTile), 0, h->stream, ca, j);
        }
        TIMING_MARK(h, "k_clcut_embed");
        hipLaunchKernelGGL(k_clcut_ritz, rows, dim3(kClCutTile), 0, h->stream, ca);
        hipLaunchKernelGGL(k_clcut_embed, dim3(ns), dim3(1024), 0, h->stream, ca);
        TIMING_MARK(h, "k_cluster_orient");
        hipLaunchKernelGGL(k_cluster_orient, dim3(1), dim3(1024), 0, h->stream, oa);
        HIP_TRY(h, hipGetLastError());
    }
    h->cl_have_carry = true;
    return GORDER_OK;
}

static int run_clustering(gorder_hip_handle *h, const float *d_xyz, const float *d_box, size_t n_assign, uint32_t row0) {
    if (h->cl_cut) return run_clustering_cutoff(h, d_xyz, d_box, n_assign, row0);
    const gorder_leaflets_t &lf = h->tables.leaflets;
    const uint32_t n = lf.n_membrane, slab = h->cl_slab;
    ClArgs ca{};
    ca.xyz = d_xyz; ca.box9 = d_box; ca.n_atoms = h->plan.n_atoms; ca.group = h->d_membrane; ca.n = n;
    ca.pbc = h->tables.handle_pbc ? 1 : 0; ca.m_max = h->cl_m_max; ca.err = h->d_err;
    char *base = (char *)h->d_cl_scratch;
    auto carve = [&](size_t per_frame) { char *at = base; base += per_frame * slab; return at; };
    ca.sol = (double *)carve(cl_round(kClSol * 8));
    ca.pos = (float *)carve(cl_round(3 * (size_t)n * 4));
    ca.s = (float *)carve(cl_round((size_t)n * 4));
    ca.q = (float *)carve(cl_round((size_t)n * 4));
    ca.emb = (float *)carve(cl_round((size_t)n * 4));
    ca.V = (float *)carve(cl_round((size_t)(h->cl_m_max + 1u) * n * 4));
    ca.meta = (float *)carve(cl_round(kClMeta * 4));
    ca.fail = (uint32_t *)carve(16);
    ca.lab = (uint8_t *)carve(cl_round(n));
    ca.W = h->cl_stored_w ? (float *)carve((size_t)n * n * 4) : nullptr;
    ClOrientArgs oa{};
    oa.n = n; oa.lab = ca.lab; oa.emb = ca.emb; oa.meta = ca.meta; oa.fail = ca.fail; oa.carry = h->d_cl_carry;
    oa.aflags = h->d_aflags; oa.n_mol_total = h->plan.n_mol_total; oa.head_slot = h->d_cl_head_slot;
    oa.flip = lf.flip ? 1 : 0; oa.err = h->d_err; oa.is_frame0 = h->d_cl_is0;
    for (size_t done = 0; done < n_assign; done += slab) {
        const uint32_t ns = (uint32_t)std::min<size_t>(n_assign - done, slab);
        const bool last = done + ns == n_assign;
        ca.aframes = h->d_aframes + done; ca.n_assign = ns;
        oa.aframes = ca.aframes; oa.n_assign = ns; oa.row0 = row0 + (uint32_t)done;
        oa.adist = last ? h->d_adist : nullptr;
        oa.stats = last ? h->d_cl_stats : nullptr;
        HIP_TRY(h, hipMemsetAsync(ca.fail, 0, (size_t)ns * sizeof(uint32_t), h->stream));
        HIP_TRY(h, hipMemcpyAsync(h->d_cl_is0, h->cl_is0.data() + done, ns, hipMemcpyHostToDevice, h->stream));
        TIMING_MARK(h, "k_cluster_degrees");
        hipLaunchKernelGGL(k_cluster_degrees, dim3((n + 255u) / 256u, ns), dim3(256), 0, h->stream, ca);
        TIMING_MARK(h, "k_cluster_lanczos");
        hipLaunchKernelGGL(k_cluster_lanczos, dim3(ns), dim3(1024), 0, h->stream, ca);
        TIMING_MARK(h, "k_cluster_embed");
        hipLaunchKernelGGL(k_cluster_embed, dim3(ns), dim3(1024), 0, h->stream, ca);
        TIMING_MARK(h, "k_cluster_orient");
        hipLaunchKernelGGL(k_cluster_orient, dim3(1), dim3(1024), 0, h->stream, oa);
    }
    h->cl_have_carry = true;
    return GORDER_OK;
}

static int run_leaflets(gorder_hip_handle *h, const float *d_xyz, const float *d_box,
                        const std::vector<uint32_t> &aframes, uint32_t row0, const uint8_t *skip = nullptr) {
    if (aframes.empty()) return GORDER_OK;
    int st;
    const size_t cap_before = h->aframes_cap;
    if ((st = ensure(h, &h->d_aframes, &h->aframes_cap, aframes.size())) != GORDER_OK) return st;
    if (h->aframes_cap != cap_before) h->up_aframes_at = nullptr;
    if (h->up_aframes_at != h->d_aframes || h->up_aframes != aframes) {
        HIP_TRY(h, hipMemcpyAsync(h->d_aframes, aframes.data(), aframes.size() * sizeof(uint32_t),
                                  hipMemcpyHostToDevice, h->stream));
        h->up_aframes = aframes;
        h->up_aframes_at = h->d_aframes;
    }
    const gorder_leaflets_t &lf = h->tables.leaflets;
    LeafletArgs la{};
    la.xyz = d_xyz; la.box9 = d_box; la.n_atoms = h->plan.n_atoms;
    la.aframes = h->d_aframes; la.row0 = row0; la.aflags = h->d_aflags; la.adist = h->d_adist;
    la.n_mol_total = h->plan.n_mol_total; la.heads = h->d_heads;
    la.membrane = h->d_membrane; la.n_membrane = lf.n_membrane;
    la.methyl_begin = h->d_methyl_begin; la.methyl_atoms = h->d_methyl_atoms;
    la.dim = lf.normal_dim; la.flip = lf.flip ? 1 : 0; la.pbc = h->tables.handle_pbc ? 1 : 0;
    la.err = h->d_err;
    la.skip = skip;
    la.n_assign = (uint32_t)aframes.size();
    if (lf.method == GORDER_LEAFLETS_GLOBAL) {
        const dim3 g(skip ? std::min<uint32_t>((uint32_t)aframes.size(), 512u) : (uint32_t)aframes.size()), b(1024);
        TIMING_MARK(h, h->membrane_is_frame ? "k_leaflets_global_contig" : "k_leaflets_global");
        if (h->membrane_is_frame) {
            if (skip) hipLaunchKernelGGL(k_leaflets_global_contig<true>, g, dim3(256), 0, h->stream, la);
            else hipLaunchKernelGGL(k_leaflets_global_contig<false>, g, dim3(256), 0, h->stream, la);
        } else {
            if (skip) hipLaunchKernelGGL(k_leaflets_global<true>, g, b, 0, h->stream, la);
            else hipLaunchKernelGGL(k_leaflets_global<false>, g, b, 0, h->stream, la);
        }
    } else if (lf.method == GORDER_LEAFLETS_INDIVIDUAL) {
        TIMING_MARK(h, "k_leaflets_individual");
        size_t done = 0;
        while (done < aframes.size()) {
            const uint32_t ny = (uint32_t)std::min<size_t>(aframes.size() - done, 65535);
            LeafletArgs lb = la;
            lb.aframes = h->d_aframes + done;
            lb.row0 = row0 + (uint32_t)done;
            if (done + ny < aframes.size()) lb.adist = nullptr;
            hipLaunchKernelGGL(k_leaflets_individual, dim3((la.n_mol_total + 255) / 256, ny), dim3(256), 0,
                               h->stream, lb);
            done += ny;
        }
    } else if (lf.method == GORDER_LEAFLETS_SPHERICAL) {
        TIMING_MARK(h, "k_leaflets_spherical");
        SphArgs sa{};
        sa.xyz = d_xyz; sa.box9 = d_box; sa.n_atoms = h->plan.n_atoms;
        sa.aflags = h->d_aflags; sa.n_mol_total = h->plan.n_mol_total; sa.heads = h->d_heads;
        sa.group = h->d_membrane; sa.n_group = lf.n_membrane;
        sa.flip = lf.flip ? 1 : 0; sa.pbc = h->tables.handle_pbc ? 1 : 0;
        sa.spill = h->d_sph_spill; sa.n_spill = h->sph_spill; sa.err = h->d_err;
        for (size_t done = 0; done < aframes.size(); done += h->sph_slab) {
            const uint32_t ns = (uint32_t)std::min<size_t>(aframes.size() - done, h->sph_slab);
            const bool last = done + ns == aframes.size();
            sa.aframes = h->d_aframes + done;
            sa.row0 = row0 + (uint32_t)done;
            sa.n_assign = ns;
            sa.adist = last ? h->d_adist : nullptr;
            sa.stats = last ? h->d_sph_stats : nullptr;
            if (h->sph_threads == 256u) hipLaunchKernelGGL(k_leaflets_spherical<256>, dim3(ns), dim3(256), 0, h->stream, sa);
            else hipLaunchKernelGGL(k_leaflets_spherical<1024>, dim3(ns), dim3(1024), 0, h->stream, sa);
        }
    } else if (lf.method == GORDER_LEAFLETS_CLUSTERING) {
        if ((st = run_clustering(h, d_xyz, d_box, aframes.size(), row0)) != GORDER_OK) return st;
    } else if (lf.method == GORDER_LEAFLETS_LOCAL) {
        const size_t ncell = (size_t)kLocalMaxCells1D * kLocalMaxCells1D;
        LocalArgs lo{};
        lo.xyz = d_xyz; lo.box9 = d_box; lo.n_atoms = h->plan.n_atoms;
        lo.aflags = h->d_aflags; lo.adist = h->d_adist; lo.n_mol_total = h->plan.n_mol_total;
        lo.heads = h->d_heads; lo.mol_slot0 = h->d_mol_slot0; lo.n_membrane = lf.n_membrane;
        lo.membrane = h->membrane_is_frame ? nullptr : h->d_membrane;
        lo.dim = lf.normal_dim; lo.flip = lf.flip ? 1 : 0; lo.pbc = h->tables.handle_pbc ? 1 : 0;
        lo.radius = lf.radius;
        lo.radius_thr = local_radius_threshold(lf.radius);
        lo.cell_of = h->d_lcell_of; lo.trig = h->d_ltrig; lo.cell_count = h->d_lcell_count;
        lo.cell_fill = h->d_lcell_fill; lo.err = h->d_err;
        lo.grid = h->d_lgrid;
        lo.halo = h->local_halo ? 1 : 0;
        lo.prune = env_flag("GORDER_HIP_LOCAL_NO_PRUNE") ? 0 : (env_flag("GORDER_HIP_LOCAL_DECIDE_NOTHING") ? 2 : 1);
        lo.rec_stride = (uint32_t)h->local_rec_stride;
        lo.rowpre = h->d_lrowpre;
        lo.edge = h->d_ledge;
        lo.finfo = h->d_lfinfo;
        lo.todo = h->d_ltodo;
        bool decide = lo.halo && lo.prune && lo.n_mol_total && !env_flag("GORDER_HIP_LOCAL_NO_DECIDE");
        if (decide) {
            if (h->lsummary_pending) {
                if (hipEventQuery(h->lsummary_written) == hipSuccess) {
                    h->lsummary_pending = false;
                    if (2u * h->h_lsummary[0] > h->h_lsummary[1]) h->decide_pause = gorder_hip_handle::kDecidePause;
                } else {
                    (void)hipGetLastError();
                }
            }
            if (h->decide_pause) { h->decide_pause--; h->decide_paused_submits++; decide = false; }
            else h->decide_submits++;
        }
        lo.need = decide ? h->d_lneed : nullptr;
        lo.sums = decide && lf.n_membrane <= kLocalBuildMax && !env_flag("GORDER_HIP_LOCAL_THREE_KERNELS") &&
                  !env_flag("GORDER_HIP_LOCAL_NO_SUMS") ? 1 : 0;
        const bool report = decide && !h->lsummary_pending;
        lo.summary = report ? h->d_lsummary : nullptr;
        for (size_t done = 0; done < aframes.size(); done += h->local_slab) {
            const uint32_t ns = (uint32_t)std::min<size_t>(aframes.size() - done, h->local_slab);
            lo.aframes = h->d_aframes + done;
            lo.n_slab = ns;
            lo.row0 = row0 + (uint32_t)done;
            lo.write_dist_frame = (done + ns == aframes.size()) ? (int)ns - 1 : -1;
            lo.summary_host = report && done + ns == aframes.size() ? h->h_lsummary : nullptr;
            if (lf.n_membrane > kLocalBuildMax || env_flag("GORDER_HIP_LOCAL_THREE_KERNELS"))
                HIP_TRY(h, hipMemsetAsync(h->d_lcell_fill, 0, ns * ncell * sizeof(uint32_t), h->stream));
            if (lo.sums) {
                HIP_TRY(h, hipMemsetAsync(h->d_lneed, 0, (ns + 1) * sizeof(uint32_t), h->stream));
                TIMING_MARK(h, "k_local_sums");
                hipLaunchKernelGGL(k_local_sums, dim3(ns), dim3(1024), kSumsLds, h->stream, lo);
                TIMING_MARK(h, "k_local_decide");
                hipLaunchKernelGGL(k_local_decide, dim3(ns), dim3(1024), kDecideLds, h->stream, lo);
            }
            const int cst = launch_cell_list(h, lo, ns, lf.n_membrane, h->d_lcell_count, ns * (ncell + 1) * sizeof(uint32_t));
            if (cst != GORDER_OK) return cst;
            if (lo.halo) {
                TIMING_MARK(h, "k_local_rowprefix");
                hipLaunchKernelGGL(k_local_rowprefix, dim3(kLocalMaxCells1D / 4u, ns), dim3(256), 0, h->stream, lo);
                lo.rows_groups = (lo.n_mol_total + 15u) / 16u;
                if (lo.need && !lo.sums) {
                    TIMING_MARK(h, "k_local_decide");
                    hipLaunchKernelGGL(k_local_decide, dim3(ns), dim3(1024), kDecideLds, h->stream, lo);
                }
                TIMING_MARK(h, "k_local_flags_rows");
                if (lo.need) hipLaunchKernelGGL(k_local_flags_rows_open, dim3(lo.rows_groups * 8u * kRowsSlots), dim3(256), 0, h->stream, lo);
                else hipLaunchKernelGGL(k_local_flags_rows, dim3(lo.rows_groups * ((ns + 7u) / 8u * 8u)), dim3(256), 0, h->stream, lo);
                TIMING_MARK(h, "k_local_flags_todo");
                hipLaunchKernelGGL(k_local_flags_todo, dim3(512), dim3(256), 0, h->stream, lo);
            } else {
                TIMING_MARK(h, "k_local_flags");
                hipLaunchKernelGGL(k_local_flags, dim3((lo.n_mol_total + 3) / 4, ns), dim3(256), 0, h->stream, lo);
            }
        }
        if (report && !aframes.empty()) {
            HIP_TRY(h, hipEventRecord(h->lsummary_written, h->stream));
            h->lsummary_pending = true;
        }
    }
    HIP_TRY(h, hipGetLastError());
    return GORDER_OK;
}

int gorder_hip_submit_device(gorder_hip_handle *h, const float *d_xyz, const float *d_box,
                             const uint64_t *frame_index, uint32_t n_frames) {
    if (!h || !d_xyz || !frame_index) return GORDER_ERR_INVALID_ARGUMENT;
    const bool pbc = h->tables.handle_pbc != 0;
    if (pbc && !d_box) return fail(h, GORDER_ERR_INVALID_ARGUMENT, "box required when handle_pbc = 1");
    if (((uintptr_t)d_xyz & 15u) != 0) return fail(h, GORDER_ERR_INVALID_ARGUMENT, "d_xyz must be 16-byte aligned");
    if (n_frames == 0) return GORDER_OK;
    HIP_TRY(h, hipSetDevice(h->device));
    h->collect_locked = true;
    const Plan &p = h->plan;
    const gorder_leaflets_t &lf = h->tables.leaflets;
    int st;
    if ((h->n_frames + n_frames) > (uint64_t)(9223372036854775807ll / 1000000ll) / h->map_max_mol)
        return fail(h, GORDER_ERR_OVERFLOW, "order accumulators could overflow i64 (frames x molecules >= 2^63 / 1e6)");

    const bool leaflets = lf.method != GORDER_LEAFLETS_NONE;
    size_t n_new_rows = 0;
    bool spec = false;
    std::vector<uint32_t> spec_aframes;
    std::vector<uint64_t> collect_frames;
    if (h->manual_frames) {
        if (h->manual_frames != n_frames) return fail(h, GORDER_ERR_INVALID_ARGUMENT, "gorder_hip_set_normals: frame count differs from the batch");
        if (!p.direct.empty()) return fail(h, GORDER_ERR_INVALID_ARGUMENT, "manual normals: a bond spans more than the LDS window");
    }
    const bool ltable = lf.method == GORDER_LEAFLETS_MANUAL && h->d_ltable;
    gorder::ReplayLeafletBatch replay;
    std::vector<uint32_t> normal_rows;
    if (ltable) {
        uint64_t bad = 0;
        if (gorder::replay_plan_leaflets(lf.frequency, h->ltable_win, h->replay_have_carry, h->replay_carry_index, frame_index, n_frames,
                                         replay, &bad) != gorder::kReplayOk) {
            h->err_frame = bad;
            return fail(h, GORDER_ERR_MANUAL_LEAFLET_FRAME, "manual leaflet table: no row for frame " + std::to_string(bad));
        }
    }
    if (h->d_ntable) {
        uint64_t bad = 0;
        const gorder::ReplayStatus rs = gorder::replay_plan_normals(h->ntable_step, h->ntable_win, frame_index, n_frames, normal_rows, &bad);
        if (rs != gorder::kReplayOk) {
            h->err_frame = bad;
            if (rs == gorder::kReplayBadStep)
                return fail(h, GORDER_ERR_INVALID_ARGUMENT, "manual normal table: frame " + std::to_string(bad) + " is no multiple of the step");
            return fail(h, GORDER_ERR_MANUAL_NORMAL_FRAME, "manual normal table: no row for frame " + std::to_string(bad));
        }
    }
    auto abort_batch = [&](int status) {
        hipLaunchKernelGGL(k_batch_abort, dim3(1), dim3(1), 0, h->stream, h->d_err);
        (void)hipGetLastError();
        (void)timing_mark(h, nullptr);
        return status;
    };
    if (leaflets) {
        std::vector<uint32_t> arow(n_frames), aframes;
        uint32_t cur = 0;
        bool have = h->have_assignment;
        uint64_t last_assign_frame = h->assignment_frame;
        if (ltable) {
            arow = replay.arow;
            last_assign_frame = replay.carry_index * lf.frequency;
        } else for (uint32_t f = 0; f < n_frames; f++) {
            if (lf.method != GORDER_LEAFLETS_MANUAL && should_assign(lf.frequency, frame_index[f])) {
                if (lf.method == GORDER_LEAFLETS_CLUSTERING) {
                    if (aframes.empty()) h->cl_is0.clear();
                    if (aframes.empty() && frame_index[f] != 0 && !h->cl_have_carry)
                        return fail(h, GORDER_ERR_LEAFLETS_NOT_PRIMED, "clustering: no clusters of an earlier assignment frame to match against");
                    h->cl_is0.push_back(frame_index[f] == 0 ? 1 : 0);
                }
                aframes.push_back(f);
                cur = (uint32_t)aframes.size();
                have = true;
                last_assign_frame = frame_index[f];
            }
            if (!have) return fail(h, GORDER_ERR_LEAFLETS_NOT_PRIMED, "no leaflet assignment for the first frame");
            arow[f] = cur;
        }
        const bool tw_tiled = h->extra.tw && !(h->tables.flags & GORDER_FLAG_TRIG_ACOS_COS) && h->d_item_run &&
                              h->frames_per_stage == (int)kRecFrames && !env_flag("GORDER_HIP_TW_GATHER");
        spec = h->spec_enabled && lf.method == GORDER_LEAFLETS_GLOBAL && h->have_assignment && aframes.size() == n_frames &&
               !h->extra.maps && (!h->extra.tw || tw_tiled) && !h->extra.geom_kind && !h->dyn && !h->manual_frames && !h->d_ntable &&
               !h->use_gather && !p.tiles.empty();
        if (spec) {
            spec_poll(h, false);
            const uint32_t slot = (uint32_t)(h->spec_batches % gorder_hip_handle::kSpecRing);
            if (h->spec_ring_frames[slot]) (void)hipEventSynchronize(h->spec_counters_copied[slot]), spec_poll(h, false);
            spec = h->spec_enabled;
        }
        if (spec) std::fill(arow.begin(), arow.end(), 0u);
        const size_t rows = (ltable ? replay.expand.size() : aframes.size()) + 1;
        if (rows > h->aflags_rows) {
            uint8_t *nb = nullptr;
            const size_t nrows = rows + rows / 4;
            HIP_TRY(h, hipMalloc((void **)&nb, nrows * (size_t)p.n_mol_total));
            if (h->d_aflags) {
                HIP_TRY(h, hipMemcpyAsync(nb, h->d_aflags, p.n_mol_total, hipMemcpyDeviceToDevice, h->stream));
                HIP_TRY(h, hipStreamSynchronize(h->stream));
                HIP_TRY(h, hipFree(h->d_aflags));
            }
            h->d_aflags = nb;
            h->aflags_rows = nrows;
        }
        const size_t cap_before = h->arow_cap;
        if ((st = ensure(h, &h->d_arow, &h->arow_cap, n_frames)) != GORDER_OK) return st;
        if (h->arow_cap != cap_before) h->up_arow_at = nullptr;
        if (h->up_arow_at != h->d_arow || h->up_arow != arow) {
            HIP_TRY(h, hipMemcpyAsync(h->d_arow, arow.data(), n_frames * sizeof(uint32_t), hipMemcpyHostToDevice,
                                      h->stream));
            h->up_arow = arow;
            h->up_arow_at = h->d_arow;
        }
        if (h->collect & GORDER_COLLECT_LEAFLETS)
            for (uint32_t f : aframes) collect_frames.push_back(frame_index[f]);
        if (spec) spec_aframes = aframes;
        else if (ltable) { if ((st = replay_flag_rows(h, replay)) != GORDER_OK) return abort_batch(st); }
        else if ((st = run_leaflets(h, d_xyz, d_box, aframes, 1)) != GORDER_OK) return abort_batch(st);
        h->have_assignment = true;
        h->assignment_frame = last_assign_frame;
        n_new_rows = spec ? 0 : (ltable ? replay.expand.size() : aframes.size());
    }
    if (h->extra.tw && h->n_frames + n_frames > h->tw_cap) {
        const size_t row = 3 * (size_t)p.n_acc;
        const uint64_t ncap = (h->n_frames + n_frames) * 2;
        unsigned long long *ns = nullptr, *nc = nullptr;
        HIP_TRY(h, hipMalloc((void **)&ns, ncap * row * sizeof(unsigned long long)));
        HIP_TRY(h, hipMalloc((void **)&nc, ncap * row * sizeof(unsigned long long)));
        HIP_TRY(h, hipMemsetAsync(ns, 0, ncap * row * sizeof(unsigned long long), h->stream));
        HIP_TRY(h, hipMemsetAsync(nc, 0, ncap * row * sizeof(unsigned long long), h->stream));
        if (h->d_tw_sums) {
            HIP_TRY(h, hipMemcpyAsync(ns, h->d_tw_sums, h->n_frames * row * sizeof(unsigned long long), hipMemcpyDeviceToDevice, h->stream));
            HIP_TRY(h, hipMemcpyAsync(nc, h->d_tw_cnts, h->n_frames * row * sizeof(unsigned long long), hipMemcpyDeviceToDevice, h->stream));
            HIP_TRY(h, hipStreamSynchronize(h->stream));
            HIP_TRY(h, hipFree(h->d_tw_sums));
            HIP_TRY(h, hipFree(h->d_tw_cnts));
        }
// ... 898 lines not shown
```

gorder_amd/csrc/kernels_leaflets.h:

```cpp
#pragma once

namespace {

struct LeafletArgs {
    const float *xyz;
    const float *box9;
    uint32_t n_atoms;
    const uint32_t *aframes;
    uint32_t row0;
    uint8_t *aflags;
    float *adist;
    uint32_t n_mol_total;
    const uint32_t *heads;
    const uint32_t *membrane;
    uint32_t n_membrane;
    const uint32_t *methyl_begin;
    const uint32_t *methyl_atoms;
    uint32_t dim;
    int flip, pbc;
    uint32_t *err;
    const uint8_t *skip;
    uint32_t n_assign;
};

// ... 344 lines not shown
        __syncthreads();
    }
}

struct SpecArgs {
    const float *xyz;
    const float *box9;
    uint32_t n_atoms, n_frames, n_tiles, n_mol_total, n_membrane;
    uint32_t dim;
    int flip, pbc;
    const float4 *mom;
    const float *head_z;
    float *center;
    uint8_t *ok;
    uint8_t *aflags;
    float *adist;
    uint32_t *counters;
    uint32_t *counters_next;
    uint32_t *host_counters;
    uint32_t *err;
};
__global__ __launch_bounds__(256) void k_spec_check(SpecArgs a) {
    __shared__ float s_center;
    __shared__ int s_ok;
    for (uint32_t f = blockIdx.x; f < a.n_frames; f += gridDim.x) {
        const float L = a.pbc ? a.box9[9 * (size_t)f + 4 * a.dim] : 0.0f;
        if (threadIdx.x < 64u) {
            double S = 0.0, Q = 0.0;
            float mn = 3.0e38f, mx = -3.0e38f;
            for (uint32_t t = threadIdx.x; t < a.n_tiles; t += 64u) {
                const float4 m = a.mom[(size_t)f * a.n_tiles + t];
                S += (double)m.x; Q += (double)m.y;
                mn = fminf(mn, m.z); mx = fmaxf(mx, m.w);
            }
            wave_sum2_minmax_bfly(S, Q, mn, mx);
            if (threadIdx.x == 0u) {
                const double n = (double)a.n_membrane, c = S / n;
                bool ok = (S - S == 0.0) && (Q - Q == 0.0) && mn <= mx;
                if (ok && a.pbc) {
                    const double k = 6.283185307179586 / (double)L;
                    const double var = fmax(Q - S * S / n, 0.0) + 1e-4 * Q + 1e-6 * n;
                    const double dmax = k * fmax((double)mx - c, c - (double)mn), S2 = k * k * var, den = n - 0.5 * S2;
                    ok = den > 0.0 && L > 0.0f;
                    if (ok) {
                        const double dist = (dmax * S2 / 6.0 / den) / k;
                        const double room = 0.5 * (double)L - 1e-4 * (double)L - dist;
                        ok = (double)mx - c < room && c - (double)mn < room;
                    }
                }
                a.center[f] = (float)c;
                a.ok[f] = ok ? 1 : 0;
                s_center = (float)c;
                s_ok = ok ? 1 : 0;
                if (!ok) atomicAdd(&a.counters[1], 1u);
            }
        }
        __syncthreads();
        if (s_ok) {
            const float c = s_center;
            const bool last = f + 1 == a.n_frames;
            int bad = 0;
            for (uint32_t m = threadIdx.x; m < a.n_mol_total; m += blockDim.x) {
                float d = a.head_z[(size_t)f * a.n_mol_total + m] - c;
                if (a.pbc) d = gm_min_image(d, L, bad);
                a.aflags[(size_t)(1u + f) * a.n_mol_total + m] = (uint8_t)((d >= 0.0f ? 0 : 1) ^ (a.flip ? 1 : 0));
                if (last && a.adist) a.adist[m] = d;
            }
            if (bad) raise_box_range(a.err, f);
        }
        __syncthreads();
    }
}
struct SpecSample { uint32_t i, j, slot; };
template <bool ACOS_COS, bool TW>
__global__ __launch_bounds__(64) void k_spec_fixup(FrameArgs a, SpecArgs sa, const uint32_t *__restrict__ mol_begin,
                                                   const SpecSample *__restrict__ samples, unsigned long long *tw_sums,
                                                   unsigned long long *tw_cnts, uint64_t tw_row0) {
    const uint64_t n_pairs = (uint64_t)sa.n_frames * sa.n_mol_total;
    uint32_t moved = 0;
    for (uint64_t p0 = (uint64_t)blockIdx.x * 64u; p0 < n_pairs; p0 += (uint64_t)gridDim.x * 64u) {
        const uint64_t pi = p0 + threadIdx.x;
        bool differs = false;
        uint32_t exact_l = 0;
        if (pi < n_pairs) {
            exact_l = sa.aflags[(size_t)sa.n_mol_total + pi];
            differs = exact_l != sa.aflags[pi % sa.n_mol_total];
        }
        unsigned long long todo = __ballot(differs);
        moved += (uint32_t)__popcll(todo);
        while (todo) {
            const int l = __ffsll((long long)todo) - 1;
            todo &= todo - 1ull;
            const uint64_t pj = p0 + (uint64_t)l;
            const uint32_t f = (uint32_t)(pj / sa.n_mol_total), m = (uint32_t)(pj - (uint64_t)f * sa.n_mol_total);
            const uint32_t exact = (uint32_t)__shfl((int)exact_l, l, 64);
            const float *x = a.xyz + (size_t)f * a.n_atoms * 3u;
            for (uint32_t q = mol_begin[m] + threadIdx.x; q < mol_begin[m + 1]; q += 64u) {
                const SpecSample sm = samples[q];
                SampleAcc acc;
                int bad = 0;
                const float *p1 = x + 3u * (size_t)sm.i, *p2 = x + 3u * (size_t)sm.j;
                bond_sample<ACOS_COS>(a, f, p1[0], p1[1], p1[2], p2[0], p2[1], p2[2], m, acc, bad);
                unsigned long long *rep = a.rep;
                if (exact == 0u) {
                    atomicAdd(&rep[(size_t)a.n_acc + sm.slot], (unsigned long long)acc.s_tot);
                    atomicAdd(&rep[3u * (size_t)a.n_acc + sm.slot], 1ull);
                } else {
                    atomicAdd(&rep[(size_t)a.n_acc + sm.slot], (unsigned long long)(-acc.s_tot));
                    atomicAdd(&rep[3u * (size_t)a.n_acc + sm.slot], ~0ull);
                }
                if (TW) {
                    const size_t up = (size_t)(tw_row0 + f) * 3u * a.n_acc + (size_t)a.n_acc + sm.slot;
                    atomicAdd(&tw_sums[up], (unsigned long long)(exact == 0u ? acc.s_tot : -acc.s_tot));
                    atomicAdd(&tw_cnts[up], exact == 0u ? 1ull : ~0ull);
                }
            }
        }
    }
    if (threadIdx.x == 0u && moved) atomicAdd(&sa.counters[0], moved);
}
__global__ __launch_bounds__(256) void k_spec_finish(SpecArgs sa) {
    for (uint32_t m = threadIdx.x; m < sa.n_mol_total; m += blockDim.x)
        sa.aflags[m] = sa.aflags[(size_t)sa.n_frames * sa.n_mol_total + m];
    if (threadIdx.x == 0u) {
        sa.host_counters[0] = sa.counters[0];
        sa.host_counters[1] = sa.counters[1];
        sa.counters_next[0] = 0u;
        sa.counters_next[1] = 0u;
    }
}

__global__ __launch_bounds__(256) void k_leaflets_individual(LeafletArgs a) {
    const uint32_t m = blockIdx.x * blockDim.x + threadIdx.x;
    if (m >= a.n_mol_total) return;
    const uint32_t f = a.aframes[blockIdx.y];
    const float *x = a.xyz + (size_t)f * a.n_atoms * 3u;
    float L = 1.0f;
    if (a.pbc) L = a.box9[9 * (size_t)f + 4 * a.dim];
    int bad = 0;
    const float hp = x[3u * (size_t)a.heads[m] + a.dim];
    float total = 0.0f;
    for (uint32_t k = a.methyl_begin[m]; k < a.methyl_begin[m + 1]; k++) {
        const float mp = x[3u * (size_t)a.methyl_atoms[k] + a.dim];
        const float d = hp - mp;
        total += a.pbc ? gm_min_image(d, L, bad) : d;
    }
    a.aflags[(size_t)(a.row0 + blockIdx.y) * a.n_mol_total + m] =
        (uint8_t)((total >= 0.0f ? 0 : 1) ^ (a.flip ? 1 : 0));
    if (blockIdx.y + 1 == gridDim.y && a.adist) a.adist[m] = total;
    if (bad) raise_box_range(a.err, f);
}

constexpr uint32_t kLocalMaxCells1D = 128;
constexpr uint32_t kLocalSlabMax = 2048;
inline uint32_t local_slab_frames(size_t n_membrane) {
    const size_t per_frame = n_membrane * (2u * 12u + 4u) + (size_t)(2 * 4u + 16u + 16u) * kLocalMaxCells1D * (kLocalMaxCells1D + 1u) + 32u;
    const size_t n = ((size_t)4096 << 20) / per_frame;
    uint32_t cap = kLocalSlabMax;
    if (const char *ev = getenv("GORDER_HIP_LOCAL_SLAB")) cap = (uint32_t)std::max(4, atoi(ev));
    return (uint32_t)(n < 4 ? 4 : (n > cap ? cap : n));
}

struct LocalRowPre { float sc, ss; double sz; };
struct alignas(16) LocalEdge { uint32_t q; float zm, sq; uint32_t cs; };
constexpr uint32_t kEdgeSpanMax = 2000;
__device__ __forceinline__ uint32_t local_edge_trig(float sc, float ss) {
    return ((uint32_t)(int)__builtin_rintf(sc * 16.0f) & 0xffffu) | ((uint32_t)(int)__builtin_rintf(ss * 16.0f) << 16);
}
__device__ __forceinline__ void local_edge_trig_diff(uint32_t hi, uint32_t lo, float &dc, float &ds) {
    dc = (float)(int16_t)((hi & 0xffffu) - (lo & 0xffffu)) * 0.0625f;
    ds = (float)(int16_t)((hi >> 16) - (lo >> 16)) * 0.0625f;
}
struct LocalRec { float x, y, z; };

struct LocalArgs {
    const float *xyz;
    const float *box9;
    uint32_t n_atoms;
    const uint32_t *aframes;
    uint32_t frame0;
    uint32_t n_slab;
    uint32_t row0;
    uint8_t *aflags;
    float *adist;
    int write_dist_frame;
    uint32_t n_mol_total;
    const uint32_t *heads;
    const uint32_t *mol_slot0;
    const uint32_t *membrane;
    uint32_t n_membrane;
    uint4 *grid;
    uint32_t dim;
    int flip, pbc;
    float radius;
    float radius_thr;
    uint32_t *cell_of;
    float *trig;
    uint32_t *cell_count;
    uint32_t *cell_fill;
    int halo;
    int prune;
    uint32_t rows_groups;
    uint32_t rec_stride;
    LocalEdge *edge;
    LocalRowPre *rowpre;
    float4 *finfo;
    uint2 *todo;
    int sums;
    uint32_t *summary;
    uint32_t *summary_host;
    uint32_t *need;
    uint32_t *err;
};

constexpr uint32_t kLocalFine = 4;
constexpr uint32_t kLocalFineRows = 7;
__device__ __forceinline__ void local_axis(float L, float radius, uint32_t &nc, uint32_t &k, uint32_t k_max = kLocalFine,
                                           uint32_t nc_max = kLocalMaxCells1D) {
    nc = 1; k = 0;
    for (uint32_t kk = k_max; kk >= 1u; kk--) {
        const float fine = floorf(L / (radius / (float)kk) * 0.9999f);
        if (fine >= (float)(2u * kk + 1u) && fine <= (float)nc_max) { nc = (uint32_t)fine; k = kk; return; }
    }
}
__device__ __forceinline__ void local_grid(const LocalArgs &a, const float *box, uint32_t &nca, uint32_t &ncb,
                                           int &da, int &db, uint32_t &ka, uint32_t &kb) {
    da = (int)((a.dim + 1u) % 3u);
    db = (int)((a.dim + 2u) % 3u);
    nca = ncb = 1;
    ka = kb = 0;
    if (a.pbc) {
        const uint32_t k_max = a.halo ? kLocalFineRows : kLocalFine;
        local_axis(box[da], a.radius, nca, ka, k_max);
        local_axis(box[db], a.radius, ncb, kb, k_max, a.halo ? kLocalMaxCells1D - 2u * kLocalFineRows : kLocalMaxCells1D);
    }
}
__device__ __forceinline__ uint32_t local_row_stride(const LocalArgs &a, uint32_t ncb, uint32_t kb) {
    return a.halo ? ncb + 2u * kb : ncb;
}
__device__ __forceinline__ void local_grid(const LocalArgs &a, const float *box, uint32_t &nca, uint32_t &ncb,
                                           int &da, int &db) {
    uint32_t ka, kb;
    local_grid(a, box, nca, ncb, da, db, ka, kb);
}

__device__ __forceinline__ void local_finfo_init(const LocalArgs &a, uint32_t s) {
    if (a.finfo) reinterpret_cast<uint4 *>(a.finfo)[s] = make_uint4(0xffffffffu, 0u, 0u, 0u);
}
__device__ __forceinline__ void frame_box(const LocalArgs &a, uint32_t f, float *box) {
    box[0] = box[1] = box[2] = 1.0f;
    if (a.pbc) {
        const float *b = a.box9 + 9 * (size_t)f;
        box[0] = b[0]; box[1] = b[4]; box[2] = b[8];
    }
}

__device__ __forceinline__ uint32_t local_cell_of(const LocalArgs &a, uint32_t s, uint32_t f, uint32_t i,
                                                  const float *box, uint32_t nca, uint32_t ncb, uint32_t ncs, int da, int db) {
    const float *p = a.xyz + ((size_t)f * a.n_atoms + (a.membrane ? a.membrane[i] : i)) * 3u;
    int bad = 0;
    uint32_t ca = 0, cb = 0;
    if (a.pbc) {
        const float wa = gm_wrap(p[da], box[da], bad), wb = gm_wrap(p[db], box[db], bad);
        ca = (uint32_t)fminf(fmaxf(floorf(wa / box[da] * (float)nca), 0.0f), (float)(nca - 1u));
        cb = (uint32_t)fminf(fmaxf(floorf(wb / box[db] * (float)ncb), 0.0f), (float)(ncb - 1u));
    }
    const uint32_t c = ca * ncs + cb;
    a.cell_of[(size_t)s * a.n_membrane + i] = c;
    if (bad) raise_box_range(a.err, f);
    return c;
}

constexpr uint32_t kLocalLdsCells = 4096;

__global__ __launch_bounds__(256) void k_local_bin(LocalArgs a) {
    __shared__ uint32_t hist[kLocalLdsCells];
    const uint32_t i = blockIdx.x * blockDim.x + threadIdx.x;
    const uint32_t s = blockIdx.y;
    const uint32_t f = a.aframes ? a.aframes[s] : a.frame0 + s;
    float box[3];
    frame_box(a, f, box);
    uint32_t nca, ncb, ka, kb;
    int da, db;
    local_grid(a, box, nca, ncb, da, db, ka, kb);
    const uint32_t ncs = local_row_stride(a, ncb, kb), ncell = nca * ncs;
    uint32_t *count = a.cell_count + (size_t)s * (kLocalMaxCells1D * kLocalMaxCells1D + 1u);
    const bool lds = ncell <= kLocalLdsCells;
    if (lds) {
        for (uint32_t k = threadIdx.x; k < ncell; k += blockDim.x) hist[k] = 0;
        __syncthreads();
    }
    if (i < a.n_membrane) {
        const uint32_t c = local_cell_of(a, s, f, i, box, nca, ncb, ncs, da, db);
        if (lds) atomicAdd(&hist[c], 1u);
        else atomicAdd(&count[c], 1u);
        if (a.halo && c % ncs < 2u * kb) {
            if (lds) atomicAdd(&hist[c + ncb], 1u);
            else atomicAdd(&count[c + ncb], 1u);
        }
    }
    if (lds) {
        __syncthreads();
        for (uint32_t k = threadIdx.x; k < ncell; k += blockDim.x)
            if (hist[k]) atomicAdd(&count[k], hist[k]);
    }
}

__global__ __launch_bounds__(1024) void k_local_scan(LocalArgs a) {
    __shared__ uint32_t part[1024];
    const uint32_t s = blockIdx.x;
    uint32_t *cnt = a.cell_count + (size_t)s * (kLocalMaxCells1D * kLocalMaxCells1D + 1u);
    constexpr uint32_t N = kLocalMaxCells1D * kLocalMaxCells1D, PER = N / 1024u;
    uint32_t local[PER];
    uint32_t sum = 0;
    for (uint32_t k = 0; k < PER; k++) {
        local[k] = cnt[threadIdx.x * PER + k];
        sum += local[k];
    }
    part[threadIdx.x] = sum;
    __syncthreads();
    for (uint32_t off = 1; off < 1024; off <<= 1) {
        uint32_t v = threadIdx.x >= off ? part[threadIdx.x - off] : 0;
        __syncthreads();
        part[threadIdx.x] += v;
        __syncthreads();
    }
    uint32_t run = part[threadIdx.x] - sum;
    for (uint32_t k = 0; k < PER; k++) {
        cnt[threadIdx.x * PER + k] = run;
        run += local[k];
    }
    if (threadIdx.x == 1023) cnt[N] = run;
    if (threadIdx.x == 0 && a.grid) {
        float box[3];
        frame_box(a, a.aframes ? a.aframes[s] : a.frame0 + s, box);
        uint32_t nca, ncb, ka, kb;
        int da, db;
        local_grid(a, box, nca, ncb, da, db, ka, kb);
        a.grid[s] = make_uint4(nca, ncb, ka, kb);
        local_finfo_init(a, s);
    }
}

__global__ __launch_bounds__(256) void k_local_scatter(LocalArgs a) {
    __shared__ uint32_t hist[kLocalLdsCells];
    const uint32_t i = blockIdx.x * blockDim.x + threadIdx.x;
    const uint32_t s = blockIdx.y;
    const uint32_t f = a.aframes ? a.aframes[s] : a.frame0 + s;
    float box[3];
    frame_box(a, f, box);
    uint32_t nca, ncb, ka, kb;
    int da, db;
    local_grid(a, box, nca, ncb, da, db, ka, kb);
    const uint32_t ncs = local_row_stride(a, ncb, kb), ncell = nca * ncs;
    const int dn = (int)a.dim;
    const bool lds = ncell <= kLocalLdsCells;
    uint32_t *fill = a.cell_fill + (size_t)s * (kLocalMaxCells1D * kLocalMaxCells1D);
    const bool valid = i < a.n_membrane;
    uint32_t c = 0, rank = 0;
    if (valid) c = a.cell_of[(size_t)s * a.n_membrane + i];
    if (lds) {
        for (uint32_t k = threadIdx.x; k < ncell; k += blockDim.x) hist[k] = 0;
        __syncthreads();
        if (valid) rank = atomicAdd(&hist[c], 1u);
        __syncthreads();
        for (uint32_t k = threadIdx.x; k < ncell; k += blockDim.x)
            if (hist[k]) hist[k] = atomicAdd(&fill[k], hist[k]);
        __syncthreads();
        if (valid) rank += hist[c];
    } else if (valid) {
        rank = atomicAdd(&fill[c], 1u);
    }
    if (!valid) return;
    const uint32_t start = a.cell_count[(size_t)s * (kLocalMaxCells1D * kLocalMaxCells1D + 1u) + c];
    const float *p = a.xyz + ((size_t)f * a.n_atoms + (a.membrane ? a.membrane[i] : i)) * 3u;
    const size_t q = (size_t)s * a.rec_stride + start + rank;
    reinterpret_cast<LocalRec *>(a.trig)[q] = LocalRec{p[da], p[db], p[dn]};
    if (a.halo && c % ncs < 2u * kb) {
        const uint32_t c2 = c + ncb;
        const size_t q2 = (size_t)s * a.rec_stride + a.cell_count[(size_t)s * (kLocalMaxCells1D * kLocalMaxCells1D + 1u) + c2] +
                          atomicAdd(&fill[c2], 1u);
        reinterpret_cast<LocalRec *>(a.trig)[q2] = LocalRec{p[da], p[db], p[dn]};
    }
}

template <uint32_t PIECE>
__device__ __forceinline__ void local_row_prefix(const uint32_t *__restrict__ cstart, const LocalRec *__restrict__ rec,
                                                 LocalRowPre *__restrict__ out, LocalEdge *__restrict__ out_edge, uint32_t ra,
                                                 uint32_t ncs, float inv_Ln,
                                                 float z_mid, float *pc, float *ps, double *pz, float *pq, float &zlo, float &zhi,
                                                 uint32_t &nf) {
    const uint32_t lane = threadIdx.x & 63u;
    constexpr uint32_t CQ = kLocalMaxCells1D / 64u + 1u;
    uint32_t cq[CQ];
#pragma unroll
    for (uint32_t i = 0; i < CQ; i++) cq[i] = lane + 64u * i <= ncs ? cstart[ra * ncs + lane + 64u * i] : 0xffffffffu;
    const uint32_t qa = (uint32_t)__builtin_amdgcn_readfirstlane((int)cq[0]);
    uint32_t qb = 0;
#pragma unroll
    for (uint32_t i = 0; i < CQ; i++)
        if ((ncs >> 6) == i) qb = (uint32_t)__builtin_amdgcn_readlane((int)cq[i], (int)(ncs & 63u));
    float carry_c = 0.0f, carry_s = 0.0f, carry_q = 0.0f;
    double carry_z = 0.0;
    static_assert(PIECE == 256u, "a lane takes four consecutive records of a piece");
    for (uint32_t base = qa; base < qb || base == qa; base += PIECE) {
        const uint32_t n_here = min(PIECE, qb - base);
        LocalRec r[4];
#pragma unroll
        for (uint32_t k = 0; k < 4u; k++) {
            const uint32_t q = base + 4u * lane + k;
            r[k] = rec[q < qb ? q : (qb ? qb - 1u : 0u)];
        }
        float vc[4], vs[4], vq[4];
        double vz[4];
#pragma unroll
        for (uint32_t k = 0; k < 4u; k++) {
            const bool valid = base + 4u * lane + k < qb;
            float sn_t, cs_t;
            local_trig(r[k].z, inv_Ln, &sn_t, &cs_t);
            vc[k] = valid ? cs_t : 0.0f;
            vs[k] = valid ? sn_t : 0.0f;
            vz[k] = valid ? (double)r[k].z : 0.0;
            const float dq = r[k].z - z_mid;
            vq[k] = valid ? dq * dq : 0.0f;
            if (valid) {
                zlo = fminf(zlo, r[k].z);
                zhi = fmaxf(zhi, r[k].z);
                nf |= ((r[k].x - r[k].x) + (r[k].y - r[k].y)) + (r[k].z - r[k].z) == 0.0f ? 0u : 1u;
            }
        }
        const float c1 = vc[0], c2 = c1 + vc[1], c3 = c2 + vc[2], tc = c3 + vc[3];
        const float s1 = vs[0], s2 = s1 + vs[1], s3 = s2 + vs[2], ts = s3 + vs[3];
        const float q1 = vq[0], q2 = q1 + vq[1], q3 = q2 + vq[2], tq = q3 + vq[3];
        const double z1 = vz[0], z2 = z1 + vz[1], z3 = z2 + vz[2], tz = z3 + vz[3];
        float ic = tc, is = ts, iq = tq;
        double iz = tz;
        row_sums(ic, is, iz, iq);
        float bc = 0.0f, bs = 0.0f, bq = 0.0f;
        double bz = 0.0;
#pragma unroll
        for (int r4 = 0; r4 < 3; r4++) {
            const float rc = lane_value(ic, 16 * r4 + 15), rs = lane_value(is, 16 * r4 + 15), rq = lane_value(iq, 16 * r4 + 15);
            const double rz = lane_value(iz, 16 * r4 + 15);
            if ((int)(lane >> 4) > r4) { bc += rc; bs += rs; bz += rz; bq += rq; }
        }
        ic += bc; is += bs; iz += bz; iq += bq;
        const float ec = carry_c + (ic - tc), es = carry_s + (is - ts), eq = carry_q + (iq - tq);
        const double ez = carry_z + (iz - tz);
        *reinterpret_cast<float4 *>(pc + 4u * lane) = make_float4(ec, ec + c1, ec + c2, ec + c3);
        *reinterpret_cast<float4 *>(ps + 4u * lane) = make_float4(es, es + s1, es + s2, es + s3);
        *reinterpret_cast<float4 *>(pq + 4u * lane) = make_float4(eq, eq + q1, eq + q2, eq + q3);
        *reinterpret_cast<double2 *>(pz + 4u * lane) = make_double2(ez, ez + z1);
        *reinterpret_cast<double2 *>(pz + 4u * lane + 2u) = make_double2(ez + z2, ez + z3);
        carry_c += lane_value(ic, 63);
        carry_s += lane_value(is, 63);
        carry_z += lane_value(iz, 63);
        carry_q += lane_value(iq, 63);
        if (lane == 0u) { pc[n_here] = carry_c; ps[n_here] = carry_s; pz[n_here] = carry_z; pq[n_here] = carry_q; }
        __builtin_amdgcn_fence(__ATOMIC_RELEASE, "wavefront");
        __builtin_amdgcn_wave_barrier();
        __builtin_amdgcn_fence(__ATOMIC_ACQUIRE, "wavefront");
        const bool last = base + n_here >= qb;
#pragma unroll
        for (uint32_t i = 0; i < CQ; i++) {
            const uint32_t j = lane + 64u * i, q0 = cq[i];
            if (j <= ncs && q0 >= base && (q0 < base + n_here || (last && q0 == qb))) {
                LocalRowPre o;
                o.sc = pc[q0 - base]; o.ss = ps[q0 - base]; o.sz = pz[q0 - base];
                out[j] = o;
                LocalEdge e;
                e.q = q0;
                e.zm = (float)(o.sz - (double)(q0 - qa) * (double)z_mid);
                e.sq = pq[q0 - base];
                e.cs = local_edge_trig(o.sc, o.ss);
                out_edge[j] = e;
            }
        }
        __builtin_amdgcn_fence(__ATOMIC_RELEASE, "wavefront");
        __builtin_amdgcn_wave_barrier();
        if (qb == qa) break;
    }
}
__device__ __forceinline__ void local_finfo_merge(const LocalArgs &a, uint32_t s, float zlo, float zhi, uint32_t nf) {
    wave_minmax_or_bfly(zlo, zhi, nf);
    if ((threadIdx.x & 63u) == 0u) {
        uint32_t *fi = reinterpret_cast<uint32_t *>(a.finfo + s);
        if (zlo <= zhi) {
            atomicMin(fi, local_float_key(zlo));
            atomicMax(fi + 1, local_float_key(zhi));
        }
        if (nf) atomicOr(fi + 2, 1u);
    }
}
constexpr uint32_t kRowPrefixPiece = 256;
__global__ __launch_bounds__(256) void k_local_rowprefix(LocalArgs a) {
    __shared__ alignas(16) float l_c[4][kRowPrefixPiece + 4], l_s[4][kRowPrefixPiece + 4], l_q[4][kRowPrefixPiece + 4];
    __shared__ alignas(16) double l_z[4][kRowPrefixPiece + 2];
    const uint32_t s = blockIdx.y, wave = threadIdx.x >> 6, ra = blockIdx.x * 4u + wave;
    const uint4 g = a.grid[s];
    const uint32_t nca = g.x, ncs = local_row_stride(a, g.y, g.w);
// ... 515 lines not shown
        const float B = __builtin_fmaxf((r_q - 2.0f * hm * r_z) + fr * hm * hm, 0.0f) * 1.02f + 1e-3f * fr;
        const float mid = T - 0.5f * A, rad = 0.5005f * __builtin_amdgcn_sqrtf(fr * B);
        const float slack = 0.1f + fn * (1e-3f + 1e-6f * fn * Ln);
        const float r_c = __builtin_amdgcn_sqrtf(c_c * c_c + c_s * c_s);
        const float est_c = (local_atan2_fast(-c_s, -c_c) + 3.1415927f) * (Ln * 0.15915494f);
        const float shift_c = gm_min_image(hn_pos - est_c, Ln, bad);
        const float xr = (fr + 1.0f) * __builtin_amdgcn_rcpf(r_c);
        const float emargin = 1e-4f * Ln + (xr + 0.5708f * xr * xr * xr) * (0.15916f * Ln);
        const bool same_image = fr + 1.0f < r_c && ulo_g + shift_c > -halfn + emargin && uhi_g + shift_c < halfn - emargin;
        const bool head_near = __builtin_fabsf(mid) + rad < (halfn - 1e-3f * Ln) * fi;
        const uint64_t wide = __ballot(!span_ok);
        const bool spans_ok = ((wide >> (16u * row)) & 0xffffull) == 0ull;
        const bool decided = !fail && !redo && spans_ok && c_n > r_n && same_image && head_near && (int)s != a.write_dist_frame &&
                             __builtin_fabsf(mid) > rad + slack;
        const uint64_t dm = __ballot(sub != 15u || decided || !head_ok);
        if (dm == ~0ull) {
            if (sub == 15u && head_ok)
                a.aflags[(size_t)(a.row0 + s) * a.n_mol_total + m] = (uint8_t)((mid > 0.0f ? 1 : 0) ^ (a.flip ? 1 : 0));
            if (bad) raise_box_range(a.err, f);
            return;
        }
    }
    if (try_prune && !fail && sub < n_rows && j_lo != j_hi) {
        const LocalRowPre p_lo = pre[row_e0 + j_lo], p_hi = pre[row_e0 + j_hi];
        sc += p_hi.sc - p_lo.sc;
        ss += p_hi.ss - p_lo.ss;
        inner_z = p_hi.sz - p_lo.sz;
    }
    {
        const uint32_t n_a = run_q1[0] - run_q0[0], n_b = run_q1[1] - run_q0[1];
        const uint32_t p_a = (n_a + 7u) >> 3, p_b = (n_b + 7u) >> 3, mine = p_a + p_b;
        const uint32_t incl = row_sum(mine);
        const uint32_t t0 = lane_value(incl, 15), t1 = lane_value(incl, 31), t2 = lane_value(incl, 47), t3 = lane_value(incl, 63);
        n_ring = row == 0u ? t0 : (row == 1u ? t1 : (row == 2u ? t2 : t3));
        constexpr uint32_t kRec = (uint32_t)sizeof(LocalRec);
        const uint32_t pos = incl - mine;
        const uint32_t a_from = run_q0[0] * kRec, a_to = run_q1[0] * kRec, b_from = run_q0[1] * kRec, b_to = run_q1[1] * kRec;
        for (uint32_t k = 0; k < mine; k++) {
            const bool second = k >= p_a;
            const uint32_t from = (second ? b_from - p_a * (8u * kRec) : a_from) + k * (8u * kRec), to = second ? b_to : a_to;
            if (pos + k < kRowRing) ring[pos + k] = make_uint2(from, min(to, from + 8u * kRec));
        }
    }
    redo |= n_ring > kRowRing;
    uint32_t n_max = max(max((uint32_t)__builtin_amdgcn_readlane((int)n_ring, 0), (uint32_t)__builtin_amdgcn_readlane((int)n_ring, 16)),
                         max((uint32_t)__builtin_amdgcn_readlane((int)n_ring, 32), (uint32_t)__builtin_amdgcn_readlane((int)n_ring, 48)));
    n_max = min(n_max, kRowRing);
    const uint32_t n_mine = min(n_ring, kRowRing), half = sub >> 3, lane_off = (sub & 7u) * (uint32_t)sizeof(LocalRec);
    const uint32_t n_end = (n_max + 2u * kRowFlight - 1u) / (2u * kRowFlight) * (2u * kRowFlight);
    for (uint32_t e = n_mine + sub; e < n_end; e += 16u) ring[e] = make_uint2(0u, 0u);
    __builtin_amdgcn_wave_barrier();
    const __amdgpu_buffer_rsrc_t rec_rsrc = __builtin_amdgcn_make_buffer_rsrc(const_cast<LocalRec *>(rec), 0, a.rec_stride * (uint32_t)sizeof(LocalRec), 0x00020000);
    typedef uint32_t u3 __attribute__((ext_vector_type(3)));
    typedef float f3 __attribute__((ext_vector_type(3)));
    float t_min = 0.0f;
    for (uint32_t t = 0; !fail && t < n_max; t += 2u * kRowFlight) {
        f3 r[kRowFlight];
        uint2 run[kRowFlight];
        bool v[kRowFlight];
#pragma unroll
        for (uint32_t u = 0; u < kRowFlight; u++) run[u] = ring[t + 2u * u + half];
#pragma unroll
        for (uint32_t u = 0; u < kRowFlight; u++) {
            const uint32_t q = run[u].x + lane_off;
            v[u] = q < run[u].y;
            r[u] = __builtin_bit_cast(f3, (u3)__builtin_amdgcn_raw_buffer_load_b96(rec_rsrc, (int)q, 0, 0));
        }
#pragma unroll
        for (uint32_t u = 0; u < kRowFlight; u++) {
            const float ea = __builtin_fabsf(r[u].x - ha_pos), eb = __builtin_fabsf(r[u].y - hb_pos);
            const float ta = La - ea, tb = Lb - eb;
            const float ma = __builtin_fminf(ea, ta), mb = __builtin_fminf(eb, tb);
            const bool in = v[u] & (ma * ma + mb * mb < thr);
            t_min = __builtin_fminf(t_min, __builtin_fminf(ta, tb));
            cnt += in ? 1u : 0u;
            su += in ? r[u].z : 0.0f;
        }
    }
    redo |= t_min < 0.0f;
    double tu = (double)su + inner_z;
    tu = row_sum(tu);
    row_sums(sc, ss, cnt, n_inner);
    const uint64_t redo_mask = __ballot(redo);
    const bool row_redo = ((redo_mask >> (16u * row)) & 0xffffull) != 0ull;
    bool general = fail || row_redo;
    if (sub == 15u && head_ok && !general) {
        if (cnt == 0u) {
            raise_error(a.err, GORDER_ERR_INVALID_LOCAL_MEMBRANE_CENTER, f, kStageTypes, a.mol_slot0 ? a.mol_slot0[m] : 0u, 0, m);
        } else {
            const float r_inner = __builtin_amdgcn_sqrtf(sc * sc + ss * ss), e_ring = (float)(cnt - n_inner) + 1.0f;
            const float est = (local_atan2_fast(-ss, -sc) + 3.1415927f) * (Ln * 0.15915494f);
            const float shift = gm_min_image(hn_pos - est, Ln, bad);
            const float margin = 1e-4f * Ln + e_ring * __builtin_amdgcn_rcpf(r_inner) * (0.2501f * Ln);
            if (e_ring < r_inner && ulo_g + shift > -halfn + margin && uhi_g + shift < halfn - margin) {
                const double dc = (double)cnt;
                double rc = __builtin_amdgcn_rcp(dc);
                rc = __builtin_fma(__builtin_fma(-dc, rc, 1.0), rc, rc);
                rc = __builtin_fma(__builtin_fma(-dc, rc, 1.0), rc, rc);
                const float center = gm_wrap((float)(tu * rc), Ln, bad);
                if (center != center) {
                    raise_error(a.err, GORDER_ERR_INVALID_LOCAL_MEMBRANE_CENTER, f, kStageTypes, a.mol_slot0 ? a.mol_slot0[m] : 0u, 0, m);
                } else {
                    const float d = gm_min_image(hn_pos - center, Ln, bad);
                    a.aflags[(size_t)(a.row0 + s) * a.n_mol_total + m] = (uint8_t)((d >= 0.0f ? 0 : 1) ^ (a.flip ? 1 : 0));
                    if ((int)s == a.write_dist_frame && a.adist) a.adist[m] = d;
                }
            } else {
                general = true;
            }
        }
    }
    if (bad) raise_box_range(a.err, f);
    if (general && head_ok && sub == 15u) {
        const uint32_t at = atomicAdd(&a.todo[0].x, 1u);
        a.todo[1u + at] = make_uint2(s, m);
    }
}
constexpr uint32_t kRowsSlots = 1;
__global__ __launch_bounds__(256) void k_local_flags_rows(LocalArgs a) {
    __shared__ LocalRingLists l_ring[16];
    const uint32_t n_groups = a.rows_groups, linear = blockIdx.x;
    const uint32_t xcd = linear & 7u, k = linear >> 3;
    const uint32_t s = (k / n_groups) * 8u + xcd, bx = k - (k / n_groups) * n_groups;
    if (s < a.n_slab) local_rows_group(a, s, bx, l_ring);
}
__global__ __launch_bounds__(256) void k_local_flags_rows_open(LocalArgs a) {
    __shared__ LocalRingLists l_ring[16];
    const uint32_t n_groups = a.rows_groups, linear = blockIdx.x;
    const uint32_t xcd = linear & 7u, k = linear >> 3;
    if (a.need[a.n_slab] == 0u) return;
    const uint32_t slot = k / n_groups, bx = k - slot * n_groups, lane = threadIdx.x & 63u;
    uint32_t seen = 0;
    for (uint32_t base = xcd; base < a.n_slab; base += 8u * 64u) {
        const uint32_t sl = base + 8u * lane;
        uint64_t open = __ballot(sl < a.n_slab && a.need[sl] != 0u);
        while (open != 0ull) {
            const uint32_t bit = (uint32_t)__builtin_ctzll(open);
            open &= open - 1ull;
            if (seen++ % kRowsSlots == slot) local_rows_group(a, (uint32_t)__builtin_amdgcn_readfirstlane((int)(base + 8u * bit)), bx, l_ring);
        }
    }
}

constexpr uint32_t kSumsCells = 9000;
constexpr uint32_t kSumsLds = kSumsCells * 2u * (uint32_t)sizeof(unsigned long long);
struct LocalWrapped { float a, b; int bad; };
__device__ __attribute__((noinline)) LocalWrapped local_wrap_far(float xa, float xb, float La, float Lb) {
    LocalWrapped w;
    w.bad = 0;
    w.a = gm_wrap(xa, La, w.bad);
    w.b = gm_wrap(xb, Lb, w.bad);
    return w;
}
__global__ __launch_bounds__(1024) void k_local_sums(LocalArgs a) {
    extern __shared__ unsigned long long l_sums[];
    __shared__ float l_zlo[16], l_zhi[16];
    __shared__ uint32_t l_flag[16];
    const uint32_t s = blockIdx.x, tid = threadIdx.x, lane = tid & 63u, wave = tid >> 6;
    const uint32_t f = a.aframes ? a.aframes[s] : a.frame0 + s;
    float box[3];
    frame_box(a, f, box);
    uint32_t nca, ncb, ka, kb;
    int da, db;
    local_grid(a, box, nca, ncb, da, db, ka, kb);
    const uint32_t ncs = local_row_stride(a, ncb, kb), n_base = nca * ncb;
    const int dn = (int)a.dim;
    if (tid == 0u) a.grid[s] = make_uint4(nca, ncb, ka, kb);
    if (!(a.pbc && ka >= 1u && kb >= 1u && n_base <= kSumsCells)) {
        if (tid == 0u) { local_finfo_init(a, s); a.need[s] = 1u; a.need[a.n_slab] = 1u; }
        return;
    }
    unsigned long long *l_a = l_sums, *l_b = l_sums + n_base;
    for (uint32_t k = tid; k < 2u * n_base; k += 1024u) l_sums[k] = 0ull;
    __syncthreads();
    const float *x = a.xyz + (size_t)f * a.n_atoms * 3u;
    const float La = box[da], Lb = box[db], Ln = box[dn];
    const float inv_a = (float)nca / La, inv_b = (float)ncb / Lb, inv_Ln = 1.0f / Ln, z_mid = 0.5f * Ln;
    int bad = 0;
    float zlo = 3.0e38f, zhi = -3.0e38f;
    uint32_t flag = 0;
    constexpr uint32_t U = 8;
    for (uint32_t i0 = tid; i0 < a.n_membrane; i0 += U * 1024u) {
        uint32_t at[U];
        float pa[U], pb[U], pn[U];
#pragma unroll
        for (uint32_t u = 0; u < U; u++) { const uint32_t i = min(i0 + u * 1024u, a.n_membrane - 1u); at[u] = a.membrane ? a.membrane[i] : i; }
#pragma unroll
        for (uint32_t u = 0; u < U; u++) {
            pa[u] = x[3u * (size_t)at[u] + da]; pb[u] = x[3u * (size_t)at[u] + db]; pn[u] = x[3u * (size_t)at[u] + dn];
        }
#pragma unroll
        for (uint32_t u = 0; u < U; u++) {
            if (i0 + u * 1024u >= a.n_membrane) continue;
            float wa = pa[u] > La ? pa[u] - La : pa[u], wb = pb[u] > Lb ? pb[u] - Lb : pb[u];
            wa = wa < 0.0f ? wa + La : wa;
            wb = wb < 0.0f ? wb + Lb : wb;
            if (__builtin_expect(!(wa >= 0.0f && wa <= La && wb >= 0.0f && wb <= Lb), 0)) {
                const LocalWrapped w = local_wrap_far(pa[u], pb[u], La, Lb);
                wa = w.a; wb = w.b; bad |= w.bad;
            }
            const uint32_t ca = (uint32_t)fminf(fmaxf(floorf(wa * inv_a), 0.0f), (float)(nca - 1u));
            const uint32_t cb = (uint32_t)fminf(fmaxf(floorf(wb * inv_b), 0.0f), (float)(ncb - 1u));
            const float z = pn[u], zm = z - z_mid;
            float sn, cs;
            local_trig(z, inv_Ln, &sn, &cs);
            const bool finite = ((pa[u] - pa[u]) + (pb[u] - pb[u])) + (z - z) == 0.0f;
            const bool room = zm > -8.0f && zm < 8.0f;
            flag |= (finite ? 0u : 1u) | (room ? 0u : 2u);
            zlo = fminf(zlo, z);
            zhi = fmaxf(zhi, z);
            if (finite && room) {
                const unsigned long long wa64 = ((unsigned long long)(uint32_t)__builtin_rintf((zm + 8.0f) * 32768.0f) << 32) |
                                                (unsigned long long)(uint32_t)__builtin_rintf(zm * zm * 8192.0f);
                const unsigned long long wb64 = (1ull << 42) | ((unsigned long long)(uint32_t)__builtin_rintf((cs + 1.0f) * 256.0f) << 21) |
                                                (unsigned long long)(uint32_t)__builtin_rintf((sn + 1.0f) * 256.0f);
                atomicAdd(&l_a[ca * ncb + cb], wa64);
                atomicAdd(&l_b[ca * ncb + cb], wb64);
            }
        }
    }
    if (bad) raise_box_range(a.err, f);
    __syncthreads();
    LocalEdge *out = a.edge + (size_t)s * (kLocalMaxCells1D * (kLocalMaxCells1D + 1u));
    for (uint32_t ra = wave; ra < nca; ra += 16u) {
        uint32_t c_n = 0, c_c = 0, c_s = 0;
        double c_z = 0.0, c_q = 0.0;
        for (uint32_t j0 = 0; j0 <= ncs; j0 += 64u) {
            const uint32_t j = j0 + lane, jb = j < ncb ? j : j - ncb;
            unsigned long long va = 0ull, vb = 0ull;
            if (j < ncs) { va = l_a[ra * ncb + jb]; vb = l_b[ra * ncb + jb]; }
            const uint32_t n = (uint32_t)(vb >> 42), ci = (uint32_t)(vb >> 21) & 0x1fffffu, si = (uint32_t)vb & 0x1fffffu;
            const double zi = (double)(uint32_t)(va >> 32), qi = (double)(uint32_t)va;
            flag |= n > 4095u ? 2u : 0u;
            const uint32_t i_n = wave_scan_rows(n, lane), i_c = wave_scan_rows(ci, lane), i_s = wave_scan_rows(si, lane);
            const double i_z = wave_scan_rows(zi, lane), i_q = wave_scan_rows(qi, lane);
            if (j <= ncs) {
                const uint32_t e_n = c_n + (i_n - n);
                const double e_z = c_z + (i_z - zi), e_q = c_q + (i_q - qi);
                const float e_c = (float)(c_c + (i_c - ci)) * (1.0f / 256.0f) - (float)e_n;
                const float e_s = (float)(c_s + (i_s - si)) * (1.0f / 256.0f) - (float)e_n;
                LocalEdge e;
                e.q = e_n;
                e.zm = (float)(e_z * (1.0 / 32768.0) - 8.0 * (double)e_n);
                e.sq = (float)(e_q * (1.0 / 8192.0));
                e.cs = local_edge_trig(e_c, e_s);
                out[(size_t)ra * (ncs + 1u) + j] = e;
            }
            c_n += lane_value(i_n, 63);
            c_c += lane_value(i_c, 63);
            c_s += lane_value(i_s, 63);
            c_z += lane_value(i_z, 63);
            c_q += lane_value(i_q, 63);
        }
    }
    block_finfo_record(zlo, zhi, flag, 1u, l_zlo, l_zhi, l_flag, reinterpret_cast<uint4 *>(a.finfo) + s);
    if (tid == 0u && flag) { a.need[s] = 1u; a.need[a.n_slab] = 1u; }
}

constexpr uint32_t kDecideEntries = 10000;
constexpr uint32_t kDecideLds = kDecideEntries * (uint32_t)sizeof(LocalEdge);
struct DecideFrame {
    uint32_t nca, ncb, ka, kb, ncs, n_rows;
    int da, db, dn;
    float La, Lb, Ln, z_min, z_max;
};
template <typename EdgePtr>
__device__ __forceinline__ bool local_decide_head(const LocalArgs &a, const DecideFrame &F, uint32_t f, uint32_t m, EdgePtr edge,
                                                  bool &centre_above, int &bad) {
    const uint32_t nca = F.nca, ncb = F.ncb, ka = F.ka, kb = F.kb, ncs = F.ncs, n_rows = F.n_rows;
    const float La = F.La, Lb = F.Lb, Ln = F.Ln;
    const float halfn = Ln / 2.0f, z_mid = 0.5f * Ln;
    const float thr = a.radius_thr;
    const float *hp = a.xyz + ((size_t)f * a.n_atoms + a.heads[m]) * 3u;
    const float ha_pos = hp[F.da], hb_pos = hp[F.db], hn_pos = hp[F.dn];
    const float wa = ha_pos < 0.0f ? ha_pos + La : (ha_pos > La ? ha_pos - La : ha_pos);
    const float wb = hb_pos < 0.0f ? hb_pos + Lb : (hb_pos > Lb ? hb_pos - Lb : hb_pos);
    const float ca = La * __builtin_amdgcn_rcpf((float)nca), cb = Lb * __builtin_amdgcn_rcpf((float)ncb);
    const uint32_t ha = (uint32_t)fminf(fmaxf(floorf(wa * __builtin_amdgcn_rcpf(ca)), 0.0f), (float)(nca - 1u));
    const uint32_t hb = (uint32_t)fminf(fmaxf(floorf(wb * __builtin_amdgcn_rcpf(cb)), 0.0f), (float)(ncb - 1u));
    const float fa = wa - (float)ha * ca, fb = wb - (float)hb * cb;
    uint32_t a0 = ha + nca - ka, b0 = hb + ncb - kb;
    a0 -= a0 >= nca ? nca : 0u;
    b0 -= b0 >= ncb ? ncb : 0u;
    const float ulo_g = F.z_min - hn_pos, uhi_g = F.z_max - hn_pos;
    const bool redo = !(fa >= -1e-4f * ca && fa <= ca * 1.0001f && fb >= -1e-4f * cb && fb <= cb * 1.0001f) ||
                      !(wa >= 0.0f && wa <= La && wb >= 0.0f && wb <= Lb);
    const float r_in = thr * (1.0f - 4e-4f), r_out = thr * (1.0f + 4e-4f);
    const float inv_cb = __builtin_amdgcn_rcpf(cb), t0 = fb * inv_cb + (float)kb, two_kb = (float)(2u * kb);
    uint32_t c_n = 0, r_n = 0;
    float c_z = 0.0f, r_z = 0.0f, r_q = 0.0f, c_c = 0.0f, c_s = 0.0f;
    bool spans_ok = true;
    for (uint32_t sub0 = 0; sub0 < n_rows; sub0 += 4u) {
        LocalEdge e_a[4], e_d[4], e_lo[4], e_hi[4];
#pragma unroll
        for (uint32_t u = 0; u < 4u; u++) {
            const uint32_t sub = sub0 + u;
            const float a_lo = ((float)sub - (float)ka) * ca - fa, a_hi = a_lo + ca;
            const float a_far = fmaxf(fabsf(a_lo), fabsf(a_hi));
            const float a_near = (a_lo <= 0.0f && a_hi >= 0.0f) ? 0.0f : fminf(fabsf(a_lo), fabsf(a_hi));
            const float w_out2 = r_out - a_near * a_near, w_in2 = r_in - a_far * a_far;
            const bool touch = sub < n_rows && w_out2 > 0.0f;
            const float w_out = __builtin_amdgcn_sqrtf(fmaxf(w_out2, 0.0f)) * inv_cb;
            const float jo_lo_f = floorf(t0 - w_out - 1e-3f), jo_hi_f = floorf(t0 + w_out + 1e-3f);
            const uint32_t jo_lo = (uint32_t)fminf(fmaxf(jo_lo_f, 0.0f), two_kb);
            const uint32_t jo_hi = (uint32_t)fminf(fmaxf(jo_hi_f, 0.0f), two_kb);
            const float w_in = __builtin_amdgcn_sqrtf(fmaxf(w_in2, 0.0f)) * inv_cb;
            const float lo_f = ceilf(t0 - w_in + 1e-3f), hi_f = floorf(t0 + w_in - 1e-3f) - 1.0f;
            const bool inner = w_in2 > 0.0f && hi_f >= lo_f;
            const uint32_t ji_lo = (uint32_t)fmaxf(lo_f, (float)jo_lo), ji_hi = (uint32_t)fmaxf(fminf(hi_f, (float)jo_hi), 0.0f);
            const bool has_inner = inner && ji_lo <= ji_hi;
            const uint32_t j_d = jo_hi + 1u;
            const uint32_t j_lo = has_inner ? ji_lo : j_d, j_hi = has_inner ? ji_hi + 1u : j_d;
            uint32_t ra = a0 + (sub < n_rows ? sub : 0u);
            ra -= ra >= nca ? nca : 0u;
            EdgePtr row_edge = edge + (ra * (ncs + 1u) + b0);
            e_a[u] = row_edge[touch ? jo_lo : 0u];
            e_d[u] = row_edge[touch ? j_d : 0u];
            e_lo[u] = row_edge[touch ? j_lo : 0u];
            e_hi[u] = row_edge[touch ? j_hi : 0u];
        }
#pragma unroll
        for (uint32_t u = 0; u < 4u; u++) {
            const uint32_t n_c = e_d[u].q - e_a[u].q;
            const float z_c = e_d[u].zm - e_a[u].zm;
            c_n += n_c;
            c_z += z_c;
            r_n += n_c - (e_hi[u].q - e_lo[u].q);
            r_z += z_c - (e_hi[u].zm - e_lo[u].zm);
            r_q += (e_d[u].sq - e_a[u].sq) - (e_hi[u].sq - e_lo[u].sq);
            float dc, ds;
            local_edge_trig_diff(e_d[u].cs, e_a[u].cs, dc, ds);
            c_c += dc;
            c_s += ds;
            spans_ok &= n_c < kEdgeSpanMax;
        }
    }
    const float hm = hn_pos - z_mid, fn = (float)c_n, fr = (float)r_n, fi = (float)(c_n - r_n);
    const float T = c_z - fn * hm, A = r_z - fr * hm;
    const float B = __builtin_fmaxf((r_q - 2.0f * hm * r_z) + fr * hm * hm, 0.0f) * 1.02f + 1e-3f * fr;
    const float mid = T - 0.5f * A, rad = 0.5005f * __builtin_amdgcn_sqrtf(fr * B);
    const float slack = 0.1f + fn * (1.05e-3f + 1e-6f * fn * Ln);
    const float r_c = __builtin_amdgcn_sqrtf(c_c * c_c + c_s * c_s);
    const float est_c = (local_atan2_fast(-c_s, -c_c) + 3.1415927f) * (Ln * 0.15915494f);
    const float shift_c = gm_min_image(hn_pos - est_c, Ln, bad);
    const float e_c = fr + 1.0f + 0.004f * fn;
    const float xr = e_c * __builtin_amdgcn_rcpf(r_c);
    const float emargin = 1e-4f * Ln + (xr + 0.5708f * xr * xr * xr) * (0.15916f * Ln);
    const bool same_image = e_c < r_c && ulo_g + shift_c > -halfn + emargin && uhi_g + shift_c < halfn - emargin;
    const bool head_near = __builtin_fabsf(mid) + rad < (halfn - 1e-3f * Ln) * fi;
    centre_above = mid > 0.0f;
    return !redo && spans_ok && c_n > r_n && same_image && head_near && a.prune != 2 &&
           __builtin_fabsf(mid) > rad + slack;
}
template <typename EdgePtr>
__device__ __forceinline__ void local_decide_frame(const LocalArgs &a, const DecideFrame &F, uint32_t s, uint32_t f, EdgePtr edge) {
    int bad = 0;
    uint32_t n_open = 0;
    for (uint32_t m0 = threadIdx.x & ~63u; m0 < a.n_mol_total; m0 += 1024u) {
        const uint32_t m_raw = m0 + (threadIdx.x & 63u);
        const bool head_ok = m_raw < a.n_mol_total;
        const uint32_t m = head_ok ? m_raw : a.n_mol_total - 1u;
        bool centre_above;
        const bool decided = local_decide_head(a, F, f, m, edge, centre_above, bad);
        if (decided && head_ok)
            a.aflags[(size_t)(a.row0 + s) * a.n_mol_total + m] = (uint8_t)((centre_above ? 1 : 0) ^ (a.flip ? 1 : 0));
        n_open += (uint32_t)__popcll(__ballot(!decided && head_ok));
    }
    if (n_open != 0u && (threadIdx.x & 63u) == 0u) { atomicAdd(&a.need[s], n_open); a.need[a.n_slab] = 1u; }
    if (bad) raise_box_range(a.err, f);
}
__global__ __launch_bounds__(1024) void k_local_decide(LocalArgs a) {
    extern __shared__ LocalEdge l_edge[];
    const uint32_t s = blockIdx.x;
    const uint32_t f = a.aframes ? a.aframes[s] : a.frame0 + s;
    float box[3];
    frame_box(a, f, box);
    const uint4 g = a.grid[s];
    const uint4 fk = reinterpret_cast<const uint4 *>(a.finfo)[s];
    DecideFrame F;
    F.nca = g.x; F.ncb = g.y; F.ka = g.z; F.kb = g.w; F.ncs = g.y + 2u * g.w; F.n_rows = 2u * g.z + 1u;
    F.da = (int)((a.dim + 1u) % 3u); F.db = (int)((a.dim + 2u) % 3u); F.dn = (int)a.dim;
    F.La = box[F.da]; F.Lb = box[F.db]; F.Ln = box[F.dn];
    F.z_min = local_key_float(fk.x); F.z_max = local_key_float(fk.y);
    const bool fail = !(F.ka >= 1u && F.kb >= 1u && F.n_rows <= 16u && fk.z == 0u && fk.x <= fk.y);
    if (a.sums && s == 0u && threadIdx.x == 0u) a.todo[0] = make_uint2(0u, 0u);
    if (fail || !(F.z_max - F.z_min < 0.75f * F.Ln) || (int)s == a.write_dist_frame || (a.sums && a.need[s] != 0u)) {
        if (threadIdx.x == 0u) { atomicAdd(&a.need[s], 1u); a.need[a.n_slab] = 1u; }
        return;
    }
    const LocalEdge *edge = a.edge + (size_t)s * (kLocalMaxCells1D * (kLocalMaxCells1D + 1u));
    const uint32_t n_entries = F.nca * (F.ncs + 1u);
    if (n_entries <= kDecideEntries) {
        const uint4 *src = reinterpret_cast<const uint4 *>(edge);
        uint4 *dst = reinterpret_cast<uint4 *>(l_edge);
        for (uint32_t i = threadIdx.x; i < n_entries; i += 1024u) dst[i] = src[i];
        __syncthreads();
        local_decide_frame<const LocalEdge *>(a, F, s, f, l_edge);
    } else {
        local_decide_frame<const LocalEdge *>(a, F, s, f, edge);
    }
}

__global__ __launch_bounds__(256) void k_local_flags_todo(LocalArgs a) {
    if (a.need && a.summary && blockIdx.x == 0u && threadIdx.x < 64u) {
        uint32_t c = 0;
        for (uint32_t s = threadIdx.x; s < a.n_slab; s += 64u) c += a.need[s] != 0u ? 1u : 0u;
        c = wave_sum_rows(c);
        if (threadIdx.x == 0u) {
            const uint32_t open = atomicAdd(&a.summary[0], c) + c, seen = atomicAdd(&a.summary[1], a.n_slab) + a.n_slab;
            if (a.summary_host) {
                a.summary_host[0] = open;
                a.summary_host[1] = seen;
                a.summary[0] = a.summary[1] = 0u;
            }
        }
    }
    const uint32_t n = a.todo[0].x;
    for (uint32_t i = blockIdx.x * 4u + (threadIdx.x >> 6); i < n; i += gridDim.x * 4u) {
        const uint2 e = a.todo[1u + i];
        local_flags_head(a, (uint32_t)__builtin_amdgcn_readfirstlane((int)e.x), (uint32_t)__builtin_amdgcn_readfirstlane((int)e.y));
    }
}

constexpr int kSphKeep = 16;
constexpr int kSphMaxIter = 50;
constexpr float kSphTolerance = 1e-4f;

struct SphArgs {
    const float *xyz;
    const float *box9;
    uint32_t n_atoms;
    const uint32_t *aframes;
    uint32_t row0;
    uint32_t n_assign;
    uint8_t *aflags;
    float *adist;
    float *stats;
    uint32_t n_mol_total;
    const uint32_t *heads;
    const uint32_t *group;
    uint32_t n_group;
    int flip, pbc;
    float *spill;
    uint32_t n_spill;
    uint32_t *err;
};

struct SphParams { float w, mean_a, var_a, mean_b, var_b; };

__device__ __forceinline__ float sph_distance(const float *p, const float (&c)[3], const float (&box)[3], int pbc, int &bad) {
    float v[3];
#pragma unroll
    for (int d = 0; d < 3; d++) {
        const float dx = p[d] - c[d];
        v[d] = pbc ? gm_min_image(dx, box[d], bad) : dx;
    }
    return __builtin_sqrtf((v[0] * v[0] + v[1] * v[1]) + v[2] * v[2]);
}

__device__ __forceinline__ float sph_log_gaussian(float x, float mean, float log_var, float var) {
    const float diff = x - mean;
    return -0.5f * ((1.8378770664093453f + log_var) + diff * diff / var);
}
struct SphEStep { float log_wa, log_wb, log_va, log_vb; };
__device__ __forceinline__ SphEStep sph_estep_setup(const SphParams &p) {
    return {logf(p.w), logf(1.0f - p.w), logf(p.var_a), logf(p.var_b)};
}
__device__ __forceinline__ float sph_responsibility(float x, const SphParams &p, const SphEStep &e, float &log_px) {
    const float ja = e.log_wa + sph_log_gaussian(x, p.mean_a, e.log_va, p.var_a);
    const float jb = e.log_wb + sph_log_gaussian(x, p.mean_b, e.log_vb, p.var_b);
    const float m = fmaxf(ja, jb);
    log_px = m + logf(expf(ja - m) + expf(jb - m));
    return expf(ja - log_px);
}

template <uint32_t THREADS>
__global__ __launch_bounds__(THREADS) void k_leaflets_spherical(SphArgs a) {
    __shared__ double scratch[6 * 16];
    __shared__ uint32_t hist[2][256];
    __shared__ uint32_t s_pref[2], s_rank[2];
    const uint32_t bi = blockIdx.x, tid = threadIdx.x, n = a.n_group;
    const uint32_t f = a.aframes[bi];
    const float *x = a.xyz + (size_t)f * a.n_atoms * 3u;
    float *spill = a.spill + (size_t)bi * a.n_spill;
    uint8_t *row = a.aflags + (size_t)(a.row0 + bi) * a.n_mol_total;
    const bool last = bi + 1u == a.n_assign;
    float box[3] = {1.0f, 1.0f, 1.0f};
    if (a.pbc) { const float *b = a.box9 + 9 * (size_t)f; box[0] = b[0]; box[1] = b[4]; box[2] = b[8]; }
    int bad = 0;

    float est[3] = {0.0f, 0.0f, 0.0f};
    if (a.pbc) {
        double cs[6] = {0, 0, 0, 0, 0, 0};
        float inv[3];
#pragma unroll
        for (int d = 0; d < 3; d++) inv[d] = 1.0f / box[d];
        for (uint32_t i = tid; i < n; i += THREADS) {
            const float *p = x + 3u * (size_t)a.group[i];
#pragma unroll
            for (int d = 0; d < 3; d++) {
                float sn, c;
                fast_sincos_rev(gm_wrap(p[d], box[d], bad) * inv[d], &sn, &c);
                cs[d] += (double)c;
                cs[3 + d] += (double)sn;
            }
        }
        block_sum_n<6>(cs, scratch);
#pragma unroll
        for (int d = 0; d < 3; d++) est[d] = (atan2f(-(float)cs[3 + d], -(float)cs[d]) + 3.1415927f) / (6.2831855f / box[d]);
    }
    float centre[3];
    {
        double acc[3] = {0, 0, 0};
        for (uint32_t i = tid; i < n; i += THREADS) {
            const float *p = x + 3u * (size_t)a.group[i];
#pragma unroll
            for (int d = 0; d < 3; d++) acc[d] += (double)(a.pbc ? gm_nearest_image(p[d], est[d], box[d], bad) : p[d]);
        }
        block_sum_n<3>(acc, scratch);
#pragma unroll
        for (int d = 0; d < 3; d++) {
            const float c = (float)(acc[d] / (double)n);
            centre[d] = a.pbc ? gm_wrap(c, box[d], bad) : c;
        }
    }

    float keep[kSphKeep];
    double chk[2] = {0.0, 0.0};
#pragma unroll
    for (int k = 0; k < kSphKeep; k++) {
        const uint32_t i = tid + (uint32_t)k * THREADS;
        keep[k] = 0.0f;
        if (i < n) {
            const float dd = sph_distance(x + 3u * (size_t)a.group[i], centre, box, a.pbc, bad);
            keep[k] = dd;
            chk[0] += (double)(dd - dd);
            chk[1] += (double)dd;
        }
    }
    for (uint32_t i = tid + (uint32_t)kSphKeep * THREADS; i < n; i += THREADS) {
        const float dd = sph_distance(x + 3u * (size_t)a.group[i], centre, box, a.pbc, bad);
        spill[i - (uint32_t)kSphKeep * THREADS] = dd;
        chk[0] += (double)(dd - dd);
        chk[1] += (double)dd;
    }
    auto for_each = [&](auto &&fn) {
#pragma unroll
        for (int k = 0; k < kSphKeep; k++)
            if (tid + (uint32_t)k * THREADS < n) fn(keep[k]);
        for (uint32_t i = tid + (uint32_t)kSphKeep * THREADS; i < n; i += THREADS) fn(spill[i - (uint32_t)kSphKeep * THREADS]);
    };
    block_sum_n<2>(chk, scratch);
// ... 122 lines not shown
```

include/gorder_hip.h:

```cpp
#ifndef GORDER_HIP_H
#define GORDER_HIP_H

#include <stddef.h>
#include <stdint.h>

#include "gorder_xtc.h"

#ifdef __cplusplus
extern "C" {
#endif

typedef enum {
    GORDER_OK = 0,
    GORDER_ERR_UNDEFINED_BOX = 1,
    GORDER_ERR_NOT_ORTHOGONAL_BOX = 2,
    GORDER_ERR_ZERO_BOX = 3,
    GORDER_ERR_UNDEFINED_POSITION = 4,
    GORDER_ERR_INVALID_GLOBAL_MEMBRANE_CENTER = 5,
    GORDER_ERR_INVALID_LOCAL_MEMBRANE_CENTER = 6,
    GORDER_ERR_DYNAMIC_NORMAL = 7,
    GORDER_ERR_MANUAL_LEAFLET_FRAME = 8,
    GORDER_ERR_MANUAL_NORMAL_FRAME = 9,
    GORDER_ERR_INVALID_ARGUMENT = 100,
    GORDER_ERR_DEVICE = 101,
// ... 101 lines not shown
    gorder_geometry_t geometry;
    gorder_dynamic_normal_t dynamic_normal;
} gorder_tables_t;


typedef struct gorder_hip_handle gorder_hip_handle;

int gorder_hip_create(const gorder_tables_t *tables, gorder_hip_handle **out);
void gorder_hip_destroy(gorder_hip_handle *h);

uint32_t gorder_hip_n_accumulators(const gorder_hip_handle *h);
uint32_t gorder_hip_ordermap_dims(const gorder_hip_handle *h, uint32_t *nx, uint32_t *ny);

int gorder_hip_set_stream(gorder_hip_handle *h, void *hip_stream);

int gorder_hip_submit_device(gorder_hip_handle *h, const float *d_xyz, const float *d_box,
                             const uint64_t *frame_index, uint32_t n_frames);

int gorder_hip_submit_host(gorder_hip_handle *h, const float *xyz, const float *box,
                           const uint64_t *frame_index, uint32_t n_frames);

typedef struct {
    const char *const *paths;
    uint32_t n_paths;
    const uint32_t *group;
    uint32_t n_group;
    float begin_ps, end_ps;
    uint32_t step;
    uint32_t n_threads;
    uint32_t batch_frames;
    uint64_t first_frame_index;
    uint32_t device_decode;
    uint32_t shard_index;
    uint32_t shard_count;
    uint32_t reserved;
} gorder_trajectory_t;

typedef struct {
    uint64_t n_frames;
    uint64_t n_batches;
    uint64_t bytes_h2d;
    double seconds_total;
    double seconds_decode;
    double seconds_reader_stalled;
    double seconds_gpu_starved;
    uint32_t batch_frames, decoder_threads;
    uint32_t device_decode;
    uint32_t frames_decoded_by_host;
    uint64_t shard_first, shard_frames_total;
    double seconds_setup;
} gorder_trajectory_stats_t;

int gorder_hip_run_trajectory(gorder_hip_handle *h, const gorder_trajectory_t *trajectory,
                              gorder_trajectory_stats_t *stats );
void gorder_hip_release_staging(gorder_hip_handle *h);

int gorder_hip_xtc_decode(gorder_hip_handle *h, const uint8_t *d_blob, uint64_t blob_bytes,
                          const gorder_xtc_frame_t *d_frames, uint32_t n_frames, uint32_t n_atoms_file,
                          const int32_t *d_slot_of, uint32_t n_stop, float *d_xyz, uint32_t n_atoms_out);

int gorder_hip_prime_leaflets(gorder_hip_handle *h, const float *d_xyz, const float *d_box,
                              uint64_t frame_index);

int gorder_hip_set_manual_leaflets(gorder_hip_handle *h, const uint8_t *flags, uint64_t frame_index);

int gorder_hip_set_manual_leaflet_table(gorder_hip_handle *h, const uint8_t *flags,
                                        uint64_t first_row, uint64_t n_rows);
int gorder_hip_set_manual_normal_table(gorder_hip_handle *h, const float *normals, uint32_t step,
                                       uint64_t first_row, uint64_t n_rows);

int gorder_hip_synchronize(gorder_hip_handle *h);

int gorder_hip_finish(gorder_hip_handle *h, int64_t *sums, uint64_t *counts, int64_t *map_sums,
                      uint64_t *map_counts, uint64_t *n_frames_analyzed);

int gorder_hip_timewise(gorder_hip_handle *h, int64_t *tw_sums, uint64_t *tw_counts,
                        uint64_t capacity_frames);

uint32_t gorder_hip_timewise_chunk_frames(void);
uint64_t gorder_hip_timewise_rows(const gorder_hip_handle *h);

int gorder_hip_timewise_blocks(gorder_hip_handle *h, uint32_t n_blocks, uint64_t total_frames,
                               uint64_t first_position, int64_t *block_sums, uint64_t *block_counts,
                               uint64_t *block_size);

int gorder_hip_error_estimate(gorder_hip_handle *h, uint32_t n_blocks, const uint32_t *group_begin,
                              const uint32_t *slots, uint32_t n_groups, const int64_t *block_sums,
                              const uint64_t *block_counts, float *errors);

int gorder_hip_convergence(gorder_hip_handle *h, const uint32_t *group_begin, const uint32_t *slots,
                           uint32_t n_groups, const int64_t *carry_sums, const uint64_t *carry_counts,
                           float *prefix, int64_t *end_sums, uint64_t *end_counts);

int gorder_hip_leaflets(gorder_hip_handle *h, uint8_t *flags, uint64_t *assignment_frame);
typedef enum { GORDER_COLLECT_LEAFLETS = 1u, GORDER_COLLECT_NORMALS = 2u } gorder_collect_t;
int gorder_hip_set_collect(gorder_hip_handle *h, uint32_t what);
int gorder_hip_collected_counts(gorder_hip_handle *h, uint64_t *n_leaflet_rows, uint64_t *n_normal_rows);
int gorder_hip_collected_leaflets(gorder_hip_handle *h, uint8_t *flags, uint64_t *frames,
                                  uint64_t capacity_rows, uint64_t *n_rows);
int gorder_hip_collected_normals(gorder_hip_handle *h, float *normals, uint64_t *frames,
                                 uint64_t capacity_rows, uint64_t *n_rows);

int gorder_hip_leaflet_distances(gorder_hip_handle *h, float *distances);
int gorder_hip_spherical_stats(gorder_hip_handle *h, float out[12]);
int gorder_hip_clustering_stats(gorder_hip_handle *h, float out[12]);

int gorder_hip_set_normals(gorder_hip_handle *h, const float *normals, uint32_t n_frames);

int gorder_hip_normals(gorder_hip_handle *h, float *normals, uint32_t *n_points);

int gorder_hip_accumulators_device(gorder_hip_handle *h, void **d_ptr, uint64_t *n_u64);

int gorder_hip_comm_unique_id(uint8_t id[128]);
int gorder_hip_comm_create(gorder_hip_handle *h, const uint8_t id[128], int n_ranks, int rank, void **comm_out);
void gorder_hip_comm_destroy(void *comm);
int gorder_hip_allreduce(gorder_hip_handle *h, void *nccl_comm);

int gorder_hip_reset(gorder_hip_handle *h);

int gorder_hip_export_maps(gorder_hip_handle *h, void *d_sums, void *d_counts, uint64_t n_u64);

int gorder_hip_ordermaps(gorder_hip_handle *h, const uint32_t *group_begin, const uint32_t *slots, uint32_t n_groups,
                         uint32_t min_samples, uint32_t negate, const void *d_sums, const void *d_counts,
                         uint64_t n_u64, float *maps);

int gorder_hip_bind_accumulators(gorder_hip_handle *h, void *d_ptr, uint64_t n_u64);

uint64_t gorder_hip_last_error_index(const gorder_hip_handle *h);
uint64_t gorder_hip_last_error_frame(const gorder_hip_handle *h);
const char *gorder_hip_last_error_message(const gorder_hip_handle *h);
const char *gorder_hip_strerror(int status);

int gorder_hip_kernel_time(gorder_hip_handle *h, double *ms, uint64_t *launches, int reset);
int gorder_hip_kernel_time_group(gorder_hip_handle *h, uint32_t index, const char **name, double *ms, uint64_t *segments);
const char *gorder_hip_kernel_time_names(const gorder_hip_handle *h);

typedef struct {
    uint32_t n_tiles;
    uint32_t block_threads;
    uint32_t max_window_atoms;
    uint32_t n_direct_items;
    uint32_t frames_per_stage;
    uint32_t lds_bytes;
    uint32_t map_staged;
    uint32_t map_lds_bytes;
    uint32_t leaflets_one_read;
} gorder_hip_plan_t;
int gorder_hip_plan(const gorder_hip_handle *h, gorder_hip_plan_t *plan);
int gorder_hip_plan_tables(const gorder_tables_t *tables, gorder_hip_plan_t *plan, int *selfcheck);

int gorder_hip_speculation_stats(gorder_hip_handle *h, uint64_t out[4]);

int gorder_hip_local_decide_stats(gorder_hip_handle *h, uint64_t out[4]);

int gorder_hip_selftest_arithmetic(int device, uint64_t n, uint64_t seed, uint64_t mismatches[2]);
int gorder_hip_selftest_trig(int device, int fn, uint32_t first_bits, uint32_t stride, uint32_t n, float *out);
#define GORDER_WAVE_OPS_F64_ROWS 10
#define GORDER_WAVE_OPS_F32_ROWS 16
#define GORDER_WAVE_OPS_U32_ROWS 9
#define GORDER_WAVE_OPS_FINFO_WORDS 9
int gorder_hip_selftest_wave_ops(int device, uint32_t block, const double *f64, const float *f32, const uint32_t *u32,
                                 int finfo_empty, double *out_f64, float *out_f32, uint32_t *out_u32, uint32_t *out_finfo);

#ifdef __cplusplus
}
#endif
#endif
```

Before: 20.41 million.

## Add fine-grid banded local sums and decide path for large membranes

For large membranes with PBC halo, adds a finer 512-cell edge table built by a banded k_local_sums kernel. The bands are spread across blocks in an XCD-interleaved order, and a multi-block k_local_decide<true> uses rounding-aware error bounds. Frames already decided then skip the cell-list count, scan and fill kernels through early returns on need flags. This aims to resolve most lipids cheaply and avoid full cell-list work on large systems. In exchange it costs extra memory, which shrinks slab size, adds more kernels, and relies on new float-rounding slack terms for correctness.

```diff
diff --git a/gorder_amd/abi.py b/gorder_amd/abi.py
--- a/gorder_amd/abi.py
+++ b/gorder_amd/abi.py
@@ -302,6 +302,7 @@
     "gorder_hip_plan_tables", "gorder_hip_selftest_arithmetic", "gorder_hip_selftest_trig", "gorder_hip_selftest_wave_ops", "gorder_hip_run_trajectory",
     "gorder_hip_comm_unique_id", "gorder_hip_comm_create", "gorder_hip_comm_destroy", "gorder_hip_allreduce",
     "gorder_hip_reset", "gorder_hip_xtc_decode", "gorder_hip_release_staging", "gorder_hip_speculation_stats", "gorder_hip_local_decide_stats",
+    "gorder_hip_debug_local_edges",
     "gorder_hip_spherical_stats", "gorder_hip_clustering_stats",
     "gorder_hip_set_collect", "gorder_hip_collected_counts", "gorder_hip_collected_leaflets", "gorder_hip_collected_normals",
     "gorder_hip_set_manual_leaflet_table", "gorder_hip_set_manual_normal_table",
@@ -373,6 +374,7 @@
     lib.gorder_hip_plan.argtypes = [vp, C.POINTER(CPlan)]
     lib.gorder_hip_speculation_stats.argtypes = [vp, C.POINTER(C.c_uint64)]
     lib.gorder_hip_local_decide_stats.argtypes = [vp, C.POINTER(C.c_uint64)]
+    lib.gorder_hip_debug_local_edges.argtypes = [vp, vp, C.c_uint32]
     lib.gorder_hip_spherical_stats.argtypes = [vp, C.POINTER(C.c_float)]
     lib.gorder_hip_clustering_stats.argtypes = [vp, C.POINTER(C.c_float)]
     lib.gorder_hip_plan_tables.argtypes = [C.POINTER(CTables), C.POINTER(CPlan), C.POINTER(i32)]
@@ -840,6 +842,11 @@
         self._check(self.lib.gorder_hip_local_decide_stats(self._h, out))
         return {"submits": int(out[0]), "paused": int(out[1]), "open_frames": int(out[2]), "frames": int(out[3])}
 
+    def debug_local_edges(self, n_entries: int) -> np.ndarray:
+        out = np.zeros((n_entries, 4), dtype=np.uint32)
+        self._check(self.lib.gorder_hip_debug_local_edges(self._h, out.ctypes.data_as(C.c_void_p), C.c_uint32(n_entries)))
+        return out
+
     def spherical_stats(self) -> dict:
         out = (C.c_float * 12)()
         self._check(self.lib.gorder_hip_spherical_stats(self._h, out))
diff --git a/gorder_amd/csrc/gorder_hip.hip b/gorder_amd/csrc/gorder_hip.hip
--- a/gorder_amd/csrc/gorder_hip.hip
+++ b/gorder_amd/csrc/gorder_hip.hip
@@ -71,6 +71,9 @@
     LocalRowPre *d_lrowpre = nullptr;
     LocalEdge *d_ledge = nullptr;
     float4 *d_lfinfo = nullptr;
+    uint4 *d_lgrid_fine = nullptr;
+    LocalEdge *d_ledge_fine = nullptr;
+    float4 *d_lfinfo_fine = nullptr;
     static constexpr uint32_t kDecidePause = 16;
     uint32_t *d_lsummary = nullptr, *h_lsummary = nullptr;
     hipEvent_t lsummary_written = nullptr;
@@ -100,6 +103,7 @@
     size_t inv_box_cap = 0;
     uint32_t dyn_slab = 4, local_slab = 4;
     bool local_halo = false;
+    bool local_fine = false;
     size_t local_rec_stride = 0;
     XtcCheckpoint *d_xtc_cp = nullptr;
     size_t xtc_cp_cap = 0;
@@ -416,7 +420,7 @@
     lo.xyz = a.xyz; lo.box9 = a.box9; lo.n_atoms = a.n_atoms;
     lo.n_mol_total = n_mol; lo.heads = h->d_dyn_heads; lo.membrane = h->d_dyn_cloud; lo.n_membrane = dn.n_cloud;
     lo.dim = 2; lo.pbc = a.pbc; lo.radius = dn.radius; lo.radius_thr = local_radius_threshold(dn.radius);
-    lo.halo = 0; lo.rec_stride = dn.n_cloud;
+    lo.halo = 0; lo.rec_stride = dn.n_cloud; lo.cells_max = kLocalMaxCells1D;
     lo.cell_of = h->d_dyn_cell_of; lo.trig = h->d_dyn_rec;
     lo.cell_count = h->d_dyn_count; lo.cell_fill = h->d_dyn_count + h->dyn_slab * (ncell + 1);
     lo.err = h->d_err; lo.aframes = nullptr; lo.write_dist_frame = -1;
@@ -1369,11 +1373,12 @@
         }
         if (lf.method == GORDER_LEAFLETS_LOCAL) {
             const size_t nm = lf.n_membrane, ncell = (size_t)kLocalMaxCells1D * kLocalMaxCells1D;
-            const size_t sl = h->local_slab = local_slab_frames(nm);
+            h->local_halo = t->handle_pbc && !env_flag("GORDER_HIP_LOCAL_ATOMS_ONLY");
+            h->local_fine = h->local_halo && nm > kLocalBuildMax && !env_flag("GORDER_HIP_LOCAL_NO_FINE");
+            const size_t sl = h->local_slab = local_slab_frames(nm, h->local_fine);
             for (const void *fn : {reinterpret_cast<const void *>(k_local_build<2>), reinterpret_cast<const void *>(k_local_build<5>),
                                    reinterpret_cast<const void *>(k_local_build<kLocalBuildTrips>)})
                 HIP_TRY(h, hipFuncSetAttribute(fn, hipFuncAttributeMaxDynamicSharedMemorySize, (int)kLocalBuildLds));
-            h->local_halo = t->handle_pbc && !env_flag("GORDER_HIP_LOCAL_ATOMS_ONLY");
             h->local_rec_stride = (h->local_halo ? 2u : 1u) * nm;
             HIP_TRY(h, hipMalloc((void **)&h->d_lcell_of, sl * nm * sizeof(uint32_t)));
             HIP_TRY(h, hipMalloc((void **)&h->d_ltrig, sl * h->local_rec_stride * sizeof(LocalRec)));
@@ -1390,10 +1395,15 @@
                 HIP_TRY(h, hipHostMalloc((void **)&h->h_lsummary, 2 * sizeof(uint32_t)));
                 h->h_lsummary[0] = h->h_lsummary[1] = 0u;
                 HIP_TRY(h, hipEventCreateWithFlags(&h->lsummary_written, hipEventDisableTiming));
-                HIP_TRY(h, hipFuncSetAttribute(reinterpret_cast<const void *>(k_local_decide), hipFuncAttributeMaxDynamicSharedMemorySize,
+                HIP_TRY(h, hipFuncSetAttribute(reinterpret_cast<const void *>(k_local_decide<false>), hipFuncAttributeMaxDynamicSharedMemorySize,
                                                (int)kDecideLds));
-                HIP_TRY(h, hipFuncSetAttribute(reinterpret_cast<const void *>(k_local_sums), hipFuncAttributeMaxDynamicSharedMemorySize,
-                                               (int)kSumsLds));
+                for (const void *fn : {reinterpret_cast<const void *>(k_local_sums<false>), reinterpret_cast<const void *>(k_local_sums<true>)})
+                    HIP_TRY(h, hipFuncSetAttribute(fn, hipFuncAttributeMaxDynamicSharedMemorySize, (int)kSumsLds));
+                if (h->local_fine) {
+                    HIP_TRY(h, hipMalloc((void **)&h->d_ledge_fine, sl * (size_t)kLocalFineCells1D * (kLocalFineCells1D + 1u) * sizeof(LocalEdge)));
+                    HIP_TRY(h, hipMalloc((void **)&h->d_lgrid_fine, sl * sizeof(uint4)));
+                    HIP_TRY(h, hipMalloc((void **)&h->d_lfinfo_fine, sl * sizeof(float4)));
+                }
                 HIP_TRY(h, hipMalloc((void **)&h->d_ltodo, (1 + sl * (size_t)(p.n_mol_total ? p.n_mol_total : 1)) * sizeof(uint2)));
             }
         }
@@ -1421,6 +1431,7 @@
     (void)hipFree(h->d_map_rec); (void)hipFree(h->d_ua_runs); (void)hipFree(h->d_ua_run_begin);
     (void)hipFree(h->d_runs); (void)hipFree(h->d_run_begin); (void)hipFree(h->d_items_by_slot);
     (void)hipFree(h->d_ua_item_run); (void)hipFree(h->d_item_run); (void)hipFree(h->d_lgrid); (void)hipFree(h->d_lrowpre); (void)hipFree(h->d_ledge);
+    (void)hipFree(h->d_lgrid_fine); (void)hipFree(h->d_ledge_fine); (void)hipFree(h->d_lfinfo_fine);
     (void)hipFree(h->d_own); (void)hipFree(h->d_mom); (void)hipFree(h->d_head_z); (void)hipFree(h->d_own_head_begin); (void)hipFree(h->d_own_heads); (void)hipFree(h->d_spec_center); (void)hipFree(h->d_spec_ok);
     (void)hipFree(h->d_spec_counters); (void)hipFree(h->d_spec_mol_begin); (void)hipFree(h->d_spec_samples);
     if (h->h_spec_counters) (void)hipHostFree(h->h_spec_counters);
@@ -1482,6 +1493,17 @@
     HIP_TRY(h, hipStreamSynchronize(h->stream));
     out[0] = h->decide_submits; out[1] = h->decide_paused_submits;
     out[2] = h->h_lsummary ? h->h_lsummary[0] : 0; out[3] = h->h_lsummary ? h->h_lsummary[1] : 0;
+    return GORDER_OK;
+}
+
+int gorder_hip_debug_local_edges(gorder_hip_handle *h, void *out, uint32_t n_entries) {
+    if (!h || !out) return GORDER_ERR_INVALID_ARGUMENT;
+    const LocalEdge *table = h->local_fine ? h->d_ledge_fine : h->d_ledge;
+    const size_t room = h->local_fine ? (size_t)kLocalFineCells1D * (kLocalFineCells1D + 1u) : (size_t)kLocalMaxCells1D * (kLocalMaxCells1D + 1u);
+    if (!table || n_entries > room) return fail(h, GORDER_ERR_INVALID_ARGUMENT, "no table of cell edges, or more entries than a frame's table holds");
+    HIP_TRY(h, hipSetDevice(h->device));
+    HIP_TRY(h, hipStreamSynchronize(h->stream));
+    HIP_TRY(h, hipMemcpy(out, table, (size_t)n_entries * sizeof(LocalEdge), hipMemcpyDeviceToHost));
     return GORDER_OK;
 }
 
@@ -1727,6 +1749,8 @@
         lo.rec_stride = (uint32_t)h->local_rec_stride;
         lo.rowpre = h->d_lrowpre;
         lo.edge = h->d_ledge;
+        lo.edge_stride = kLocalMaxCells1D * (kLocalMaxCells1D + 1u);
+        lo.cells_max = kLocalMaxCells1D;
         lo.finfo = h->d_lfinfo;
         lo.todo = h->d_ltodo;
         bool decide = lo.halo && lo.prune && lo.n_mol_total && !env_flag("GORDER_HIP_LOCAL_NO_DECIDE");
@@ -1743,8 +1767,12 @@
             else h->decide_submits++;
         }
         lo.need = decide ? h->d_lneed : nullptr;
-        lo.sums = decide && lf.n_membrane <= kLocalBuildMax && !env_flag("GORDER_HIP_LOCAL_THREE_KERNELS") &&
+        const bool fine = h->local_fine && lf.n_membrane > kLocalBuildMax;
+        lo.sums = decide && (lf.n_membrane <= kLocalBuildMax ? !env_flag("GORDER_HIP_LOCAL_THREE_KERNELS") : fine) &&
                   !env_flag("GORDER_HIP_LOCAL_NO_SUMS") ? 1 : 0;
+        const char *band_env = getenv("GORDER_HIP_LOCAL_BAND_CELLS");
+        const bool banded = fine || (band_env && *band_env);
+        lo.band_cells = band_env && *band_env ? (uint32_t)std::min<long>(std::max<long>(atol(band_env), 1), (long)kSumsCells) : kSumsCells;
         const bool report = decide && !h->lsummary_pending;
         lo.summary = report ? h->d_lsummary : nullptr;
         for (size_t done = 0; done < aframes.size(); done += h->local_slab) {
@@ -1757,11 +1785,21 @@
             if (lf.n_membrane > kLocalBuildMax || env_flag("GORDER_HIP_LOCAL_THREE_KERNELS"))
                 HIP_TRY(h, hipMemsetAsync(h->d_lcell_fill, 0, ns * ncell * sizeof(uint32_t), h->stream));
             if (lo.sums) {
+                LocalArgs pre = lo;
+                if (fine) {
+                    pre.cells_max = kLocalFineCells1D;
+                    pre.edge_stride = kLocalFineCells1D * (kLocalFineCells1D + 1u);
+                    pre.edge = h->d_ledge_fine; pre.grid = h->d_lgrid_fine; pre.finfo = h->d_lfinfo_fine;
+                }
+                const uint32_t rows_least = std::max(pre.band_cells / (pre.cells_max - 2u * kLocalFineRows), 1u);
+                pre.bands = (pre.cells_max + rows_least - 1u) / rows_least;
                 HIP_TRY(h, hipMemsetAsync(h->d_lneed, 0, (ns + 1) * sizeof(uint32_t), h->stream));
                 TIMING_MARK(h, "k_local_sums");
-                hipLaunchKernelGGL(k_local_sums, dim3(ns), dim3(1024), kSumsLds, h->stream, lo);
+                if (banded) hipLaunchKernelGGL(k_local_sums<true>, dim3(pre.bands * ((ns + 7u) / 8u * 8u)), dim3(1024), kSumsLds, h->stream, pre);
+                else hipLaunchKernelGGL(k_local_sums<false>, dim3(ns), dim3(1024), kSumsLds, h->stream, pre);
                 TIMING_MARK(h, "k_local_decide");
-                hipLaunchKernelGGL(k_local_decide, dim3(ns), dim3(1024), kDecideLds, h->stream, lo);
+                if (fine) hipLaunchKernelGGL(k_local_decide<true>, dim3((lo.n_mol_total + 1023u) / 1024u, ns), dim3(1024), 0, h->stream, pre);
+                else hipLaunchKernelGGL(k_local_decide<false>, dim3(1, ns), dim3(1024), kDecideLds, h->stream, pre);
             }
             const int cst = launch_cell_list(h, lo, ns, lf.n_membrane, h->d_lcell_count, ns * (ncell + 1) * sizeof(uint32_t));
             if (cst != GORDER_OK) return cst;
@@ -1771,7 +1809,7 @@
                 lo.rows_groups = (lo.n_mol_total + 15u) / 16u;
                 if (lo.need && !lo.sums) {
                     TIMING_MARK(h, "k_local_decide");
-                    hipLaunchKernelGGL(k_local_decide, dim3(ns), dim3(1024), kDecideLds, h->stream, lo);
+                    hipLaunchKernelGGL(k_local_decide<false>, dim3(1, ns), dim3(1024), kDecideLds, h->stream, lo);
                 }
                 TIMING_MARK(h, "k_local_flags_rows");
                 if (lo.need) hipLaunchKernelGGL(k_local_flags_rows_open, dim3(lo.rows_groups * 8u * kRowsSlots), dim3(256), 0, h->stream, lo);
diff --git a/gorder_amd/csrc/kernels_leaflets.h b/gorder_amd/csrc/kernels_leaflets.h
--- a/gorder_amd/csrc/kernels_leaflets.h
+++ b/gorder_amd/csrc/kernels_leaflets.h
@@ -520,9 +520,11 @@
 }
 
 constexpr uint32_t kLocalMaxCells1D = 128;
+constexpr uint32_t kLocalFineCells1D = 512;
 constexpr uint32_t kLocalSlabMax = 2048;
-inline uint32_t local_slab_frames(size_t n_membrane) {
-    const size_t per_frame = n_membrane * (2u * 12u + 4u) + (size_t)(2 * 4u + 16u + 16u) * kLocalMaxCells1D * (kLocalMaxCells1D + 1u) + 32u;
+inline uint32_t local_slab_frames(size_t n_membrane, bool fine = false) {
+    const size_t per_frame = n_membrane * (2u * 12u + 4u) + (size_t)(2 * 4u + 16u + 16u) * kLocalMaxCells1D * (kLocalMaxCells1D + 1u) + 32u +
+                             (fine ? (size_t)16u * kLocalFineCells1D * (kLocalFineCells1D + 1u) + 32u : 0u);
     const size_t n = ((size_t)4096 << 20) / per_frame;
     uint32_t cap = kLocalSlabMax;
     if (const char *ev = getenv("GORDER_HIP_LOCAL_SLAB")) cap = (uint32_t)std::max(4, atoi(ev));
@@ -571,6 +573,10 @@
     uint32_t rows_groups;
     uint32_t rec_stride;
     LocalEdge *edge;
+    uint32_t edge_stride;
+    uint32_t cells_max;
+    uint32_t band_cells;
+    uint32_t bands;
     LocalRowPre *rowpre;
     float4 *finfo;
     uint2 *todo;
@@ -599,8 +605,8 @@
     ka = kb = 0;
     if (a.pbc) {
         const uint32_t k_max = a.halo ? kLocalFineRows : kLocalFine;
-        local_axis(box[da], a.radius, nca, ka, k_max);
-        local_axis(box[db], a.radius, ncb, kb, k_max, a.halo ? kLocalMaxCells1D - 2u * kLocalFineRows : kLocalMaxCells1D);
+        local_axis(box[da], a.radius, nca, ka, k_max, a.cells_max);
+        local_axis(box[db], a.radius, ncb, kb, k_max, a.halo ? a.cells_max - 2u * kLocalFineRows : a.cells_max);
     }
 }
 __device__ __forceinline__ uint32_t local_row_stride(const LocalArgs &a, uint32_t ncb, uint32_t kb) {
@@ -645,6 +651,7 @@
     __shared__ uint32_t hist[kLocalLdsCells];
     const uint32_t i = blockIdx.x * blockDim.x + threadIdx.x;
     const uint32_t s = blockIdx.y;
+    if (a.sums && (a.need[a.n_slab] == 0u || a.need[s] == 0u)) return;
     const uint32_t f = a.aframes ? a.aframes[s] : a.frame0 + s;
     float box[3];
     frame_box(a, f, box);
@@ -677,6 +684,7 @@
 __global__ __launch_bounds__(1024) void k_local_scan(LocalArgs a) {
     __shared__ uint32_t part[1024];
     const uint32_t s = blockIdx.x;
+    if (a.sums && (a.need[a.n_slab] == 0u || a.need[s] == 0u)) return;
     uint32_t *cnt = a.cell_count + (size_t)s * (kLocalMaxCells1D * kLocalMaxCells1D + 1u);
     constexpr uint32_t N = kLocalMaxCells1D * kLocalMaxCells1D, PER = N / 1024u;
     uint32_t local[PER];
@@ -714,6 +722,7 @@
     __shared__ uint32_t hist[kLocalLdsCells];
     const uint32_t i = blockIdx.x * blockDim.x + threadIdx.x;
     const uint32_t s = blockIdx.y;
+    if (a.sums && (a.need[a.n_slab] == 0u || a.need[s] == 0u)) return;
     const uint32_t f = a.aframes ? a.aframes[s] : a.frame0 + s;
     float box[3];
     frame_box(a, f, box);
@@ -1535,11 +1544,19 @@
     w.b = gm_wrap(xb, Lb, w.bad);
     return w;
 }
+template <bool BANDS>
 __global__ __launch_bounds__(1024) void k_local_sums(LocalArgs a) {
     extern __shared__ unsigned long long l_sums[];
     __shared__ float l_zlo[16], l_zhi[16];
     __shared__ uint32_t l_flag[16];
-    const uint32_t s = blockIdx.x, tid = threadIdx.x, lane = tid & 63u, wave = tid >> 6;
+    const uint32_t tid = threadIdx.x, lane = tid & 63u, wave = tid >> 6;
+    uint32_t s = blockIdx.x, band = 0;
+    if (BANDS) {
+        const uint32_t xcd = blockIdx.x & 7u, k = blockIdx.x >> 3;
+        s = (k / a.bands) * 8u + xcd;
+        band = k % a.bands;
+        if (s >= a.n_slab) return;
+    }
     const uint32_t f = a.aframes ? a.aframes[s] : a.frame0 + s;
     float box[3];
     frame_box(a, f, box);
@@ -1548,13 +1565,17 @@
     local_grid(a, box, nca, ncb, da, db, ka, kb);
     const uint32_t ncs = local_row_stride(a, ncb, kb), n_base = nca * ncb;
     const int dn = (int)a.dim;
-    if (tid == 0u) a.grid[s] = make_uint4(nca, ncb, ka, kb);
-    if (!(a.pbc && ka >= 1u && kb >= 1u && n_base <= kSumsCells)) {
-        if (tid == 0u) { local_finfo_init(a, s); a.need[s] = 1u; a.need[a.n_slab] = 1u; }
+    if (tid == 0u && band == 0u) a.grid[s] = make_uint4(nca, ncb, ka, kb);
+    const uint32_t rows_band = BANDS ? max(min(a.band_cells, kSumsCells) / ncb, 1u) : nca;
+    const uint32_t r0 = band * rows_band, n_own = r0 < nca ? min(rows_band, nca - r0) : 0u, n_mine = n_own * ncb;
+    const bool fits = BANDS ? ncb <= kSumsCells && (nca + rows_band - 1u) / rows_band <= a.bands : n_base <= kSumsCells;
+    if (!(a.pbc && ka >= 1u && kb >= 1u && fits)) {
+        if (tid == 0u && band == 0u) { local_finfo_init(a, s); a.need[s] = 1u; a.need[a.n_slab] = 1u; }
         return;
     }
-    unsigned long long *l_a = l_sums, *l_b = l_sums + n_base;
-    for (uint32_t k = tid; k < 2u * n_base; k += 1024u) l_sums[k] = 0ull;
+    if (n_own == 0u) return;
+    unsigned long long *l_a = l_sums, *l_b = l_sums + n_mine;
+    for (uint32_t k = tid; k < 2u * n_mine; k += 1024u) l_sums[k] = 0ull;
     __syncthreads();
     const float *x = a.xyz + (size_t)f * a.n_atoms * 3u;
     const float La = box[da], Lb = box[db], Ln = box[dn];
@@ -1566,15 +1587,34 @@
     for (uint32_t i0 = tid; i0 < a.n_membrane; i0 += U * 1024u) {
         uint32_t at[U];
         float pa[U], pb[U], pn[U];
+        bool want[U];
 #pragma unroll
         for (uint32_t u = 0; u < U; u++) { const uint32_t i = min(i0 + u * 1024u, a.n_membrane - 1u); at[u] = a.membrane ? a.membrane[i] : i; }
+        if (BANDS) {
+#pragma unroll
+            for (uint32_t u = 0; u < U; u++) pa[u] = x[3u * (size_t)at[u] + da];
+#pragma unroll
+            for (uint32_t u = 0; u < U; u++) {
+                float wa = pa[u] > La ? pa[u] - La : pa[u];
+                wa = wa < 0.0f ? wa + La : wa;
+                const uint32_t ca = (uint32_t)fminf(fmaxf(floorf(wa * inv_a), 0.0f), (float)(nca - 1u));
+                want[u] = i0 + u * 1024u < a.n_membrane && (band == 0u || !(wa >= 0.0f && wa <= La) || ca - r0 < n_own);
+            }
+#pragma unroll
+            for (uint32_t u = 0; u < U; u++) {
+                pb[u] = want[u] ? x[3u * (size_t)at[u] + db] : 0.0f;
+                pn[u] = want[u] ? x[3u * (size_t)at[u] + dn] : 0.0f;
+            }
+        } else {
+#pragma unroll
+            for (uint32_t u = 0; u < U; u++) {
+                pa[u] = x[3u * (size_t)at[u] + da]; pb[u] = x[3u * (size_t)at[u] + db]; pn[u] = x[3u * (size_t)at[u] + dn];
+                want[u] = i0 + u * 1024u < a.n_membrane;
+            }
+        }
 #pragma unroll
         for (uint32_t u = 0; u < U; u++) {
-            pa[u] = x[3u * (size_t)at[u] + da]; pb[u] = x[3u * (size_t)at[u] + db]; pn[u] = x[3u * (size_t)at[u] + dn];
-        }
-#pragma unroll
-        for (uint32_t u = 0; u < U; u++) {
-            if (i0 + u * 1024u >= a.n_membrane) continue;
+            if (!want[u]) continue;
             float wa = pa[u] > La ? pa[u] - La : pa[u], wb = pb[u] > Lb ? pb[u] - Lb : pb[u];
             wa = wa < 0.0f ? wa + La : wa;
             wb = wb < 0.0f ? wb + Lb : wb;
@@ -1583,6 +1623,8 @@
                 wa = w.a; wb = w.b; bad |= w.bad;
             }
             const uint32_t ca = (uint32_t)fminf(fmaxf(floorf(wa * inv_a), 0.0f), (float)(nca - 1u));
+            const bool mine = !BANDS || ca - r0 < n_own;
+            if (BANDS && !mine && band != 0u) continue;
             const uint32_t cb = (uint32_t)fminf(fmaxf(floorf(wb * inv_b), 0.0f), (float)(ncb - 1u));
             const float z = pn[u], zm = z - z_mid;
             float sn, cs;
@@ -1592,26 +1634,26 @@
             flag |= (finite ? 0u : 1u) | (room ? 0u : 2u);
             zlo = fminf(zlo, z);
             zhi = fmaxf(zhi, z);
-            if (finite && room) {
+            if (finite && room && mine) {
                 const unsigned long long wa64 = ((unsigned long long)(uint32_t)__builtin_rintf((zm + 8.0f) * 32768.0f) << 32) |
                                                 (unsigned long long)(uint32_t)__builtin_rintf(zm * zm * 8192.0f);
                 const unsigned long long wb64 = (1ull << 42) | ((unsigned long long)(uint32_t)__builtin_rintf((cs + 1.0f) * 256.0f) << 21) |
                                                 (unsigned long long)(uint32_t)__builtin_rintf((sn + 1.0f) * 256.0f);
-                atomicAdd(&l_a[ca * ncb + cb], wa64);
-                atomicAdd(&l_b[ca * ncb + cb], wb64);
-            }
-        }
-    }
-    if (bad) raise_box_range(a.err, f);
+                atomicAdd(&l_a[(ca - r0) * ncb + cb], wa64);
+                atomicAdd(&l_b[(ca - r0) * ncb + cb], wb64);
+            }
+        }
+    }
+    if (bad && band == 0u) raise_box_range(a.err, f);
     __syncthreads();
-    LocalEdge *out = a.edge + (size_t)s * (kLocalMaxCells1D * (kLocalMaxCells1D + 1u));
-    for (uint32_t ra = wave; ra < nca; ra += 16u) {
+    LocalEdge *out = a.edge + (size_t)s * a.edge_stride;
+    for (uint32_t ra = r0 + wave; ra < r0 + n_own; ra += 16u) {
         uint32_t c_n = 0, c_c = 0, c_s = 0;
         double c_z = 0.0, c_q = 0.0;
         for (uint32_t j0 = 0; j0 <= ncs; j0 += 64u) {
             const uint32_t j = j0 + lane, jb = j < ncb ? j : j - ncb;
             unsigned long long va = 0ull, vb = 0ull;
-            if (j < ncs) { va = l_a[ra * ncb + jb]; vb = l_b[ra * ncb + jb]; }
+            if (j < ncs) { va = l_a[(ra - r0) * ncb + jb]; vb = l_b[(ra - r0) * ncb + jb]; }
             const uint32_t n = (uint32_t)(vb >> 42), ci = (uint32_t)(vb >> 21) & 0x1fffffu, si = (uint32_t)vb & 0x1fffffu;
             const double zi = (double)(uint32_t)(va >> 32), qi = (double)(uint32_t)va;
             flag |= n > 4095u ? 2u : 0u;
@@ -1636,6 +1678,10 @@
             c_q += lane_value(i_q, 63);
         }
     }
+    if (BANDS && band != 0u) {
+        if (flag) { a.need[s] = 1u; a.need[a.n_slab] = 1u; }
+        return;
+    }
     block_finfo_record(zlo, zhi, flag, 1u, l_zlo, l_zhi, l_flag, reinterpret_cast<uint4 *>(a.finfo) + s);
     if (tid == 0u && flag) { a.need[s] = 1u; a.need[a.n_slab] = 1u; }
 }
@@ -1647,7 +1693,7 @@
     int da, db, dn;
     float La, Lb, Ln, z_min, z_max;
 };
-template <typename EdgePtr>
+template <bool FINE, typename EdgePtr>
 __device__ __forceinline__ bool local_decide_head(const LocalArgs &a, const DecideFrame &F, uint32_t f, uint32_t m, EdgePtr edge,
                                                   bool &centre_above, int &bad) {
     const uint32_t nca = F.nca, ncb = F.ncb, ka = F.ka, kb = F.kb, ncs = F.ncs, n_rows = F.n_rows;
@@ -1672,6 +1718,7 @@
     const float inv_cb = __builtin_amdgcn_rcpf(cb), t0 = fb * inv_cb + (float)kb, two_kb = (float)(2u * kb);
     uint32_t c_n = 0, r_n = 0;
     float c_z = 0.0f, r_z = 0.0f, r_q = 0.0f, c_c = 0.0f, c_s = 0.0f;
+    float mag_z = 0.0f, mag_q = 0.0f;
     bool spans_ok = true;
     for (uint32_t sub0 = 0; sub0 < n_rows; sub0 += 4u) {
         LocalEdge e_a[4], e_d[4], e_lo[4], e_hi[4];
@@ -1716,13 +1763,19 @@
             c_c += dc;
             c_s += ds;
             spans_ok &= n_c < kEdgeSpanMax;
+            if (FINE) {
+                mag_z += (__builtin_fabsf(e_a[u].zm) + __builtin_fabsf(e_d[u].zm)) + (__builtin_fabsf(e_lo[u].zm) + __builtin_fabsf(e_hi[u].zm));
+                mag_q += (e_a[u].sq + e_d[u].sq) + (e_lo[u].sq + e_hi[u].sq);
+            }
         }
     }
     const float hm = hn_pos - z_mid, fn = (float)c_n, fr = (float)r_n, fi = (float)(c_n - r_n);
     const float T = c_z - fn * hm, A = r_z - fr * hm;
-    const float B = __builtin_fmaxf((r_q - 2.0f * hm * r_z) + fr * hm * hm, 0.0f) * 1.02f + 1e-3f * fr;
+    const float round_b = FINE ? 1.2e-7f * (mag_q + 2.0f * __builtin_fabsf(hm) * mag_z) : 0.0f;
+    const float round_mid = FINE ? 6e-8f * mag_z : 0.0f;
+    const float B = __builtin_fmaxf((r_q - 2.0f * hm * r_z) + fr * hm * hm, 0.0f) * 1.02f + 1e-3f * fr + round_b;
     const float mid = T - 0.5f * A, rad = 0.5005f * __builtin_amdgcn_sqrtf(fr * B);
-    const float slack = 0.1f + fn * (1.05e-3f + 1e-6f * fn * Ln);
+    const float slack = 0.1f + fn * (1.05e-3f + 1e-6f * fn * Ln) + round_mid;
     const float r_c = __builtin_amdgcn_sqrtf(c_c * c_c + c_s * c_s);
     const float est_c = (local_atan2_fast(-c_s, -c_c) + 3.1415927f) * (Ln * 0.15915494f);
     const float shift_c = gm_min_image(hn_pos - est_c, Ln, bad);
@@ -1735,16 +1788,16 @@
     return !redo && spans_ok && c_n > r_n && same_image && head_near && a.prune != 2 &&
            __builtin_fabsf(mid) > rad + slack;
 }
-template <typename EdgePtr>
+template <bool FINE, typename EdgePtr>
 __device__ __forceinline__ void local_decide_frame(const LocalArgs &a, const DecideFrame &F, uint32_t s, uint32_t f, EdgePtr edge) {
     int bad = 0;
     uint32_t n_open = 0;
-    for (uint32_t m0 = threadIdx.x & ~63u; m0 < a.n_mol_total; m0 += 1024u) {
+    for (uint32_t m0 = blockIdx.x * 1024u + (threadIdx.x & ~63u); m0 < a.n_mol_total; m0 += gridDim.x * 1024u) {
         const uint32_t m_raw = m0 + (threadIdx.x & 63u);
         const bool head_ok = m_raw < a.n_mol_total;
         const uint32_t m = head_ok ? m_raw : a.n_mol_total - 1u;
         bool centre_above;
-        const bool decided = local_decide_head(a, F, f, m, edge, centre_above, bad);
+        const bool decided = local_decide_head<FINE>(a, F, f, m, edge, centre_above, bad);
         if (decided && head_ok)
             a.aflags[(size_t)(a.row0 + s) * a.n_mol_total + m] = (uint8_t)((centre_above ? 1 : 0) ^ (a.flip ? 1 : 0));
         n_open += (uint32_t)__popcll(__ballot(!decided && head_ok));
@@ -1752,9 +1805,10 @@
     if (n_open != 0u && (threadIdx.x & 63u) == 0u) { atomicAdd(&a.need[s], n_open); a.need[a.n_slab] = 1u; }
     if (bad) raise_box_range(a.err, f);
 }
+template <bool FINE>
 __global__ __launch_bounds__(1024) void k_local_decide(LocalArgs a) {
     extern __shared__ LocalEdge l_edge[];
-    const uint32_t s = blockIdx.x;
+    const uint32_t s = blockIdx.y;
     const uint32_t f = a.aframes ? a.aframes[s] : a.frame0 + s;
     float box[3];
     frame_box(a, f, box);
@@ -1766,21 +1820,21 @@
     F.La = box[F.da]; F.Lb = box[F.db]; F.Ln = box[F.dn];
     F.z_min = local_key_float(fk.x); F.z_max = local_key_float(fk.y);
     const bool fail = !(F.ka >= 1u && F.kb >= 1u && F.n_rows <= 16u && fk.z == 0u && fk.x <= fk.y);
-    if (a.sums && s == 0u && threadIdx.x == 0u) a.todo[0] = make_uint2(0u, 0u);
+    if (a.sums && s == 0u && blockIdx.x == 0u && threadIdx.x == 0u) a.todo[0] = make_uint2(0u, 0u);
     if (fail || !(F.z_max - F.z_min < 0.75f * F.Ln) || (int)s == a.write_dist_frame || (a.sums && a.need[s] != 0u)) {
         if (threadIdx.x == 0u) { atomicAdd(&a.need[s], 1u); a.need[a.n_slab] = 1u; }
         return;
     }
-    const LocalEdge *edge = a.edge + (size_t)s * (kLocalMaxCells1D * (kLocalMaxCells1D + 1u));
+    const LocalEdge *edge = a.edge + (size_t)s * a.edge_stride;
     const uint32_t n_entries = F.nca * (F.ncs + 1u);
-    if (n_entries <= kDecideEntries) {
+    if (!FINE && n_entries <= kDecideEntries) {
         const uint4 *src = reinterpret_cast<const uint4 *>(edge);
         uint4 *dst = reinterpret_cast<uint4 *>(l_edge);
         for (uint32_t i = threadIdx.x; i < n_entries; i += 1024u) dst[i] = src[i];
         __syncthreads();
-        local_decide_frame<const LocalEdge *>(a, F, s, f, l_edge);
+        local_decide_frame<FINE, const LocalEdge *>(a, F, s, f, l_edge);
     } else {
-        local_decide_frame<const LocalEdge *>(a, F, s, f, edge);
+        local_decide_frame<FINE, const LocalEdge *>(a, F, s, f, edge);
     }
 }
 
diff --git a/include/gorder_hip.h b/include/gorder_hip.h
--- a/include/gorder_hip.h
+++ b/include/gorder_hip.h
@@ -277,6 +277,7 @@
 int gorder_hip_speculation_stats(gorder_hip_handle *h, uint64_t out[4]);
 
 int gorder_hip_local_decide_stats(gorder_hip_handle *h, uint64_t out[4]);
+int gorder_hip_debug_local_edges(gorder_hip_handle *h, void *out, uint32_t n_entries);
 
 int gorder_hip_selftest_arithmetic(int device, uint64_t n, uint64_t seed, uint64_t mismatches[2]);
 int gorder_hip_selftest_trig(int device, int fn, uint32_t first_bits, uint32_t stride, uint32_t n, float *out);
```

After: 20.76 million (median of 5 runs). 1.02x the previous value.
